# bayesml/BayesML

Measured on AMD Instinct MI355X. Metric: GMM-VB E+M samples/sec at K=64,D=128,N=1e7; 1/2/4/8-GPU scaling, higher is better.
Workload: dtype f64; 1 GPU; GMM-VB K=64 D=128 N=10000000 rows/GPU x 1 GPU, x stored f32, one VB iteration per step (c3 of BASELINE.json configs); classes=64, degree=128, rows_per_gpu=10000000, rows_total=10000000, x_storage=f32, parallelism=rows1, row_tiles=1

## Files before the change

### bayesml_amd/csrc/capi.hip

```cpp
#include "capi_internal.h"

namespace {
thread_local std::string g_err;
}

namespace gmmvb {
int fail(int code, const char* what, hipError_t e) {
    g_err = what;
    if (e != hipSuccess) {
        g_err += ": ";
        g_err += hipGetErrorString(e);
    }
    return code;
}
}

namespace {
KernelSizes kernel_sizes(int K, int D) {
    KernelSizes ks;
    ks.max_tiles = kMaxTiles;
    ks.t1_splits = GMMVB_T1_SPLITS;
    ks.sel_rows = kSelRows;
    ks.lse_rows = kLseRows;
    ks.scan_parts = kScanParts;
    ks.rec_slots = kRecSlots;
    ks.generic_rows = generic_rows(D);
    if (D > 32 * kMaxTiles) return ks;
    const int T = feature_tiles(D, kMaxTiles);
    ks.mstep_components_per_wg = mstep_components_per_wg(T, false);
    ks.slab_len = slab_len(T);
    ks.estep_image_doubles = estep_image_doubles(T);
    ks.estep_tri_image_doubles = estep_tri_image_doubles();
    ks.estep_bound_blocks = estep_bound_blocks(T);
    ks.estep_i8_image_bytes = estep_i8_image_bytes(D, 0);
    ks.estep_i8_bound_image_bytes = estep_i8_image_bytes(D, 1);
    ks.estep_i8_digit_row_bytes = estep_i8_digit_row_bytes(D);
    ks.proj_image_len = proj_image_len(K, D);
    ks.proj_const_len = proj_const_len(K);
    return ks;
}

struct Slots {
    void** at[kBufCount];
#define GMMVB_X(name) (void**)&ws->name,
    explicit Slots(gmmvb_workspace* ws) : at{GMMVB_WORKSPACE_BUFFERS(GMMVB_X)} {}
#undef GMMVB_X
};

struct HipAllocator {
    hipError_t err = hipSuccess;
    void* get(int64_t bytes, bool pinned) {
        void* p = nullptr;
        err = pinned ? hipHostMalloc(&p, (size_t)bytes, hipHostMallocDefault) : hipMalloc(&p, (size_t)bytes);
        return err == hipSuccess ? p : nullptr;
    }
    bool zero(void* p, int64_t bytes, bool pinned) {
        if (pinned) std::memset(p, 0, (size_t)bytes);
        else err = hipMemset(p, 0, (size_t)bytes);
        return err == hipSuccess;
    }
    void release(void* p, bool pinned) { (void)(pinned ? hipHostFree(p) : hipFree(p)); }
};

hipError_t init_workspace(gmmvb_workspace* ws) {
    hipError_t e = hipEventCreateWithFlags(&ws->ctr_ev, hipEventDisableTiming);
    if (ws->generic) {
        const int lds = (int)((size_t)ws->D * generic_rows(ws->D) * sizeof(double));
        if (e == hipSuccess) e = hipFuncSetAttribute((const void*)estep_generic_kernel<float>, hipFuncAttributeMaxDynamicSharedMemorySize, lds);
        if (e == hipSuccess) e = hipFuncSetAttribute((const void*)estep_generic_kernel<double>, hipFuncAttributeMaxDynamicSharedMemorySize, lds);
        return e;
    }
    ws->pt.init(ws->T, estep_bound_blocks(ws->T) ? (ws->D + 31) / 32 : 0);
    for (int i = 0; i < 6 && e == hipSuccess && ws->prune != 0; ++i) e = hipEventCreate(&ws->cal_ev[i]);
    return e;
}
}

extern "C" {

int gmmvb_abi_version(void) { return GMMVB_ABI_VERSION; }
const char* gmmvb_last_error(void) { return g_err.c_str(); }

int64_t gmmvb_stats_len(int K, int D) {
    if (K < 1 || D < 1) return -1;
    return (int64_t)K * (2 + (int64_t)D + (int64_t)D * D);
}

static int create_workspace(int K, int D, int x_dtype, int64_t max_rows, gmmvb_workspace* first, gmmvb_workspace** out) {
    if (!out) return fail(GMMVB_EINVAL, "out is null");
    *out = nullptr;
    if (K < 1 || D < 1 || max_rows < 1) return fail(GMMVB_EINVAL, "K, D and max_rows must be positive");
    if (x_dtype != GMMVB_F32 && x_dtype != GMMVB_F64) return fail(GMMVB_EINVAL, "x_dtype must be GMMVB_F32 or GMMVB_F64");
    int dev = 0;
    hipError_t e = hipGetDevice(&dev);
    if (e != hipSuccess) return fail(GMMVB_EHIP, "hipGetDevice", e);
    hipDeviceProp_t prop;
    e = hipGetDeviceProperties(&prop, dev);
    if (e != hipSuccess) return fail(GMMVB_EHIP, "hipGetDeviceProperties", e);

    gmmvb_workspace* ws = new (std::nothrow) gmmvb_workspace();
    gmmvb_scratch* group = first ? first->scratch : new (std::nothrow) gmmvb_scratch();
    if (!ws || !group) {
        delete ws;
        if (!first) delete group;
        return fail(GMMVB_ENOMEM, "host allocation failed");
    }
    ws->scratch = group;
    ++group->refs;
    const KernelSizes ks = kernel_sizes(K, D);
    const WorkspaceShape shape = make_shape(K, D, x_dtype, max_rows, prop.multiProcessorCount > 0 ? prop.multiProcessorCount : 256,
                                            WorkspaceOptions::read(std::getenv), ks);
    static_cast<WorkspaceShape&>(*ws) = shape;
    if (!first) group->npad = shape.npad;
    ws->buffers = buffer_plan(shape, ks, group->npad);
    HipAllocator hip;
    if (const BufferSpec* failed = allocate_all(ws->buffers, Slots(ws).at, group, hip, &ws->bytes)) {
        gmmvb_workspace_destroy(ws);
        return fail(failed->code, failed->what, hip.err);
    }
    e = init_workspace(ws);
    if (e != hipSuccess) {
        gmmvb_workspace_destroy(ws);
        return fail(GMMVB_EHIP, "workspace initialisation", e);
    }
    *out = ws;
    return GMMVB_OK;
}

int gmmvb_workspace_create(int K, int D, int x_dtype, int64_t max_rows, gmmvb_workspace** out) {
    return create_workspace(K, D, x_dtype, max_rows, nullptr, out);
}

int gmmvb_workspace_create_tile(gmmvb_workspace* first, int64_t max_rows, gmmvb_workspace** out) {
    if (!out) return fail(GMMVB_EINVAL, "out is null");
    *out = nullptr;
    if (!first || !first->scratch) return fail(GMMVB_EINVAL, "null argument");
    if (first->generic || first->hmm != nullptr)
        return fail(GMMVB_EUNSUPPORTED, "tile groups: mixture workspaces with c_degree <= 256 only (the HMM's time axis does not tile)");
    if (max_rows < 1 || max_rows > first->max_rows)
        return fail(GMMVB_EINVAL, "a further tile must not be larger than the group's first workspace");
    return create_workspace(first->K, first->D, first->x_dtype, max_rows, first, out);
}

int gmmvb_workspace_destroy(gmmvb_workspace* ws) {
    if (!ws) return GMMVB_OK;
    gmmvb_scratch* group = ws->scratch;
    if (group && group->owner == ws) group->owner = nullptr;
    HipAllocator hip;
    if (free_all(ws->buffers, Slots(ws).at, group, hip)) delete group;
    if (ws->pol_host) (void)hipHostFree(ws->pol_host);
    auto drop = [](hipEvent_t e) {
        if (e) (void)hipEventDestroy(e);
    };
    drop(ws->pol_ev);
    drop(ws->ctr_ev);
    for (hipEvent_t e : ws->ev) drop(e);
    for (hipEvent_t e : ws->span_ev) drop(e);
    for (hipEvent_t e : ws->cal_ev) drop(e);
    if (ws->hmm) hmm_state_destroy(ws->hmm);
    delete ws;
    return GMMVB_OK;
}

int64_t gmmvb_workspace_bytes(const gmmvb_workspace* ws) { return ws ? ws->bytes : -1; }

const char* gmmvb_last_launch_info(const gmmvb_workspace* ws) { return ws ? ws->info : ""; }

int gmmvb_pass_counts(const gmmvb_workspace* ws, int64_t* out ) {
    if (!ws || !out) return fail(GMMVB_EINVAL, "null argument");
    for (int i = 0; i < 8; ++i) out[i] = ws->passes[i];
    return GMMVB_OK;
}

int gmmvb_profile_enable(gmmvb_workspace* ws, int on) {
    if (!ws) return fail(GMMVB_EINVAL, "null argument");
    if (on && !ws->ev[0]) {
        for (auto& e : ws->ev) {
            hipError_t rc = hipEventCreate(&e);
            if (rc != hipSuccess) return fail(GMMVB_EHIP, "hipEventCreate", rc);
        }
        for (auto& e : ws->span_ev) {
            hipError_t rc = hipEventCreate(&e);
            if (rc != hipSuccess) return fail(GMMVB_EHIP, "hipEventCreate", rc);
        }
    }
    ws->prof = on != 0;
    ws->prof_light = on == 2;
    ws->span_open = false;
    ws->ev_e = ws->ev_m = false;
    ws->n_spans = 0;
    return GMMVB_OK;
}

const char* gmmvb_profile_span_name(int slot) { return (slot >= 0 && slot < kSpanSlots) ? kSpanNames[slot] : ""; }

int gmmvb_profile_spans(gmmvb_workspace* ws, float* ms , int* launches ) {
    if (!ws || !ms || !launches) return fail(GMMVB_EINVAL, "null argument");
    for (int i = 0; i < kSpanSlots; ++i) {
        ms[i] = 0.0f;
        launches[i] = 0;
    }
    for (int i = 0; i < ws->n_spans; ++i) {
        float t = 0.0f;
        hipError_t rc = hipEventSynchronize(ws->span_ev[2 * i + 1]);
        if (rc == hipSuccess) rc = hipEventElapsedTime(&t, ws->span_ev[2 * i], ws->span_ev[2 * i + 1]);
        if (rc != hipSuccess) return fail(GMMVB_EHIP, "event timing (span)", rc);
        ms[ws->span_slot[i]] += t;
        ++launches[ws->span_slot[i]];
    }
    return GMMVB_OK;
}

int gmmvb_profile_last_ms(gmmvb_workspace* ws, float* estep_ms, float* mstep_ms) {
    if (!ws || !estep_ms || !mstep_ms) return fail(GMMVB_EINVAL, "null argument");
    *estep_ms = *mstep_ms = -1.0f;
    if (ws->ev_e) {
        hipError_t rc = hipEventSynchronize(ws->ev[1]);
        if (rc == hipSuccess) rc = hipEventElapsedTime(estep_ms, ws->ev[0], ws->ev[1]);
        if (rc != hipSuccess) return fail(GMMVB_EHIP, "event timing (estep)", rc);
    }
    if (ws->ev_m) {
        hipError_t rc = hipEventSynchronize(ws->ev[3]);
        if (rc == hipSuccess) rc = hipEventElapsedTime(mstep_ms, ws->ev[2], ws->ev[3]);
        if (rc != hipSuccess) return fail(GMMVB_EHIP, "event timing (mstep)", rc);
    }
    return GMMVB_OK;
}

int gmmvb_set_pivot(gmmvb_workspace* ws, const double* pivot_dev, void* stream) {
    if (!ws || !pivot_dev) return fail(GMMVB_EINVAL, "null argument");
    hipError_t e = hipMemcpyAsync(ws->pivot, pivot_dev, (size_t)ws->D * sizeof(double), hipMemcpyDeviceToDevice,
                                  (hipStream_t)stream);
    if (e != hipSuccess) return fail(GMMVB_EHIP, "hipMemcpyAsync(pivot)", e);
    ws->xc_src = nullptr;
    ws->xq_src = nullptr;
    ++ws->pivot_gen;
    if (ws->lock_live) {
        ws->lock_live = false;
        ws->lock_reset = true;
    }
    return GMMVB_OK;
}

int gmmvb_wants_drift(const gmmvb_workspace* ws, int64_t n_rows) {
    if (!ws || ws->prune == 0 || ws->estep_variant != kEstepLds8 || ws->hmm != nullptr || !ws->rec_k) return 0;
    if (ws->opt_carry_off) return 0;
    if (ws->sharded) n_rows = ws->shard_rows / ws->shard_ranks;
    return (ws->prune == 2 || n_rows * (int64_t)ws->K >= (int64_t(1) << 23)) ? 1 : 0;
}

namespace {
__global__ void set_drift_kernel(const double* __restrict__ gamma, const double* __restrict__ delta, const double* __restrict__ big_gamma,
                                 const double* __restrict__ cvec, int K, double* __restrict__ drift) {
    const int k = blockIdx.x * blockDim.x + threadIdx.x;
    if (k >= K) return;
    drift[k] = gamma[k];
    drift[K + k] = delta[k];
    drift[2 * K + k] = cvec[k];
    drift[3 * K + k] = big_gamma[k];
}
}

int gmmvb_set_drift(gmmvb_workspace* ws, const double* gamma_dev, const double* delta_dev, const double* big_gamma_dev,
                    double typical_gamma, void* stream) {
    if (!ws || !gamma_dev || !delta_dev || !big_gamma_dev) return fail(GMMVB_EINVAL, "null argument");
    ws->typical_gamma = typical_gamma;
    hipStream_t st = (hipStream_t)stream;
    hipLaunchKernelGGL(set_drift_kernel, dim3((unsigned)((ws->K + 255) / 256)), dim3(256), 0, st, gamma_dev, delta_dev, big_gamma_dev,
                       ws->cvec, ws->K, ws->drift);
    const hipError_t e = hipGetLastError();
    if (e != hipSuccess) return fail(GMMVB_EHIP, "set_drift_kernel", e);
    ws->have_drift = ws->have_params && ws->params_used;
    return GMMVB_OK;
}

int gmmvb_debug_record(gmmvb_workspace* ws, int64_t row, double* out ) {
    if (!ws || !out || !ws->rec_k || row < 0 || row >= ws->npad) return fail(GMMVB_EINVAL, "bad argument");
    hipError_t e = hipDeviceSynchronize();
    auto get = [&e](void* dst, const void* src, size_t n) {
        if (e == hipSuccess) e = hipMemcpy(dst, src, n, hipMemcpyDeviceToHost);
    };
    for (int j = 0; j < kRecSlots; ++j) {
        unsigned short k = 0;
        float d = 0.0f;
        get(&k, ws->rec_k + (int64_t)j * ws->npad + row, sizeof(k));
        get(&d, ws->rec_d + (int64_t)j * ws->npad + row, sizeof(d));
        out[j] = k == kRecEmpty ? -1.0 : (double)k;
        out[8 + j] = d;
    }
    float B = 0.0f;
    unsigned char ex = 0, sel = 0, fl = 0;
    int kh = 0;
    get(&B, ws->rec_B + row, sizeof(B));
    get(&ex, ws->rec_exact + row, 1);
    get(&sel, ws->rec_sel + row, 1);
    get(&fl, ws->rec_flags + row, 1);
    get(&kh, ws->khat + row, sizeof(kh));
    get(out + 21, ws->lse + row, sizeof(double));
    out[16] = B;
    out[17] = ex;
    out[18] = sel;
    out[19] = fl;
    out[20] = kh;
    for (int w = 0; w < 4; ++w) {
        unsigned long long m = 0;
        if (w < (ws->K + 63) / 64) get(&m, ws->masks + (int64_t)w * ws->npad + row, sizeof(m));
        out[22 + w] = (double)m;
    }
    if (e != hipSuccess) return fail(GMMVB_EHIP, "reading a record back", e);
    return GMMVB_OK;
}

int64_t gmmvb_regroup_count(const gmmvb_workspace* ws) { return ws ? ws->sorts : -1; }

namespace {
__global__ void debug_all_rows_kernel(int* __restrict__ list, int* __restrict__ counts, int K, int k, int64_t n_rows) {
    const int64_t i = (int64_t)blockIdx.x * blockDim.x + threadIdx.x;
    if (i < n_rows) list[i] = (int)i;
    if (i < K) counts[i] = (int)(i == k ? n_rows : 0);
}
}

int gmmvb_debug_proof(gmmvb_workspace* ws, int k, int64_t n_rows, float* ub_dev, double* lb_dev, void* stream) {
    if (!ws || !ub_dev || !lb_dev || k < 0 || k >= ws->K) return fail(GMMVB_EINVAL, "bad argument");
    if (!ws->xq || !ws->img_i8b || ws->xq_src == nullptr || ws->xq_rows != n_rows || ws->xq_gen != ws->img_gen || !ws->have_params)
        return fail(GMMVB_ESTATE, "no digit planes for these rows: gmmvb_set_pivot, gmmvb_prepare_rows, gmmvb_set_params first");
    claim_scratch(ws);
    hipStream_t st = (hipStream_t)stream;
    ws->tmeta_valid = false;
    const unsigned grid = (unsigned)((std::max<int64_t>(n_rows, ws->K) + 255) / 256);
    hipLaunchKernelGGL(debug_all_rows_kernel, dim3(grid), dim3(256), 0, st, ws->lists + (int64_t)k * ws->npad, ws->counts, ws->K, k,
                       n_rows);
    hipLaunchKernelGGL(gather_plan_kernel, dim3(1), dim3(64), 0, st, ws->counts, ws->K, estep_i8_pairs_per_chunk(), ws->plan);
    hipError_t e = launch_estep_i8_proof(ws->D, ws->num_cu, st, ws->xq, ws->xqe, ws->img_i8b, ws->cvec, ws->K, ws->lists, ws->npad,
                                         ws->counts, ws->plan, ws->ub32, ws->lnrho, ws->npad);
    if (e == hipSuccess) e = hipMemcpyAsync(ub_dev, ws->ub32 + (int64_t)k * ws->npad, (size_t)n_rows * sizeof(float),
                                            hipMemcpyDeviceToDevice, st);
    if (e == hipSuccess) e = hipMemcpyAsync(lb_dev, ws->lnrho + (int64_t)k * ws->npad, (size_t)n_rows * sizeof(double),
                                            hipMemcpyDeviceToDevice, st);
    if (e != hipSuccess) return fail(GMMVB_EHIP, "proof kernel (diagnostic)", e);
    ws->e_state = 0;
    ws->lost_estep = false;
    ws->bounds_rows = 0;
    ws->rec_valid = ws->dense_valid = ws->rec_live = false;
    ws->active_lists = ws->blk_fresh = false;
    ws->lag.valid = false;
    if (ws->lock_live) {
        ws->lock_live = false;
        ws->lock_reset = true;
    }
    return GMMVB_OK;
}

int gmmvb_forget(gmmvb_workspace* ws) {
    if (!ws) return fail(GMMVB_EINVAL, "null argument");
    ws->forget = true;
    ws->have_drift = false;
    if (ws->lock_live) {
        ws->lock_live = false;
        ws->lock_reset = true;
    }
    return GMMVB_OK;
}

int gmmvb_set_params(gmmvb_workspace* ws, const double* c_dev, const double* m_dev, const double* u_dev,
                     void* stream) {
    if (!ws || !c_dev || !m_dev || !u_dev) return fail(GMMVB_EINVAL, "null argument");
    hipStream_t st = (hipStream_t)stream;
    hipError_t e = hipSuccess;
    if (ws->generic) {
        e = hipMemcpyAsync(ws->cvec, c_dev, (size_t)ws->K * sizeof(double), hipMemcpyDeviceToDevice, st);
        if (e != hipSuccess) return fail(GMMVB_EHIP, "hipMemcpyAsync(c)", e);
        e = hipMemcpyAsync(ws->gen_m, m_dev, (size_t)ws->K * ws->D * sizeof(double), hipMemcpyDeviceToDevice, st);
        if (e == hipSuccess)
            e = hipMemcpyAsync(ws->gen_u, u_dev, (size_t)ws->K * ws->D * ws->D * sizeof(double), hipMemcpyDeviceToDevice, st);
        if (e != hipSuccess) return fail(GMMVB_EHIP, "hipMemcpyAsync(m, u)", e);
        ws->have_params = true;
        ws->params_used = false;
        return GMMVB_OK;
    }
    if (ws->wide) {
        if (ws->pivot_i8) return fail(GMMVB_EUNSUPPORTED, "gmmvb_set_params: int8 images past D = 128");
        hipLaunchKernelGGL(pack_params_kernel, dim3(ws->K), dim3(256), 0, st, u_dev, m_dev, ws->K, ws->D, ws->T, ws->img_len, ws->img,
                           c_dev, ws->cvec, nullptr, nullptr);
        e = hipGetLastError();
        if (e != hipSuccess) return fail(GMMVB_EHIP, "pack_params_kernel", e);
    } else {
        e = launch_pack_images(u_dev, m_dev, c_dev, ws->pivot, ws->K, ws->D, ws->T, ws->img_len, ws->img, ws->cvec, ws->pivot_i8,
                               ws->pivot_i8 ? ws->img_i8 : nullptr, ws->pivot_i8 ? ws->img_i8b : nullptr, st);
        if (e != hipSuccess) return fail(GMMVB_EHIP, "pack_images_kernel", e);
        if (ws->pivot_i8) ws->img_gen = ws->pivot_gen;
    }
    if (ws->tri) {
        e = launch_pack_tri16(u_dev, m_dev, ws->K, ws->D, ws->tri, st);
        if (e != hipSuccess) return fail(GMMVB_EHIP, "pack_tri16_kernel", e);
    }
    ws->proj_table = false;
    if (ws->gimg && ws->opt_project != 0 && ws->sorted && ws->tile_ref_valid && ws->have_drift && ws->xq_gen == ws->pivot_gen &&
        !ws->opt_carry_off) {
        e = launch_proj_table(u_dev, m_dev, c_dev, ws->pivot, ws->K, ws->D, ws->gimg, ws->gconst, st);
        if (e != hipSuccess) return fail(GMMVB_EHIP, "proj_table_kernel", e);
        ws->proj_table = true;
    }
    ws->have_params = true;
    ws->params_used = false;
    return GMMVB_OK;
}

int fetch_counters(gmmvb_workspace* ws) {
    if (ws->ctr_pending) {
        hipError_t e = hipEventSynchronize(ws->ctr_ev);
        if (e != hipSuccess) return fail(GMMVB_EHIP, "waiting for the E-step counters", e);
        ws->lag.act = ws->ctr_host[0];
        if (ws->pend_mode == 0) {
            ws->lag.eval = (double)ws->pend_rows * ws->K;
            ws->lag.over = 0.0;
            ws->lag.settled = 0.0;
            ws->lag.listed = ws->lag.accum = ws->lag.act;
            ws->lag.exits = 0.0;
            ws->lag.cols = -1.0;
            ws->lag.left = -1.0;
            ws->lag.proof = 0.0;
            ws->lag.moved = 0.0;
        } else {
            ws->lag.proof = ws->ctr_host[7];
            ws->lag.exits = (ws->exit_host && ws->gather_exit) ? (double)ws->exit_host[0] : 0.0;
            ws->lag.cols = (ws->exit_host && ws->pend_lazy) ? (double)ws->exit_host[1] : -1.0;
            ws->lag.left = (ws->exit_host && ws->pend_proj) ? (double)ws->exit_host[2] : -1.0;
            ws->lag.settled = ws->ctr_host[4];
            ws->lag.listed = ws->ctr_host[5];
            ws->lag.accum = ws->ctr_host[6];
            ws->lag.eval = ws->ctr_host[1] + ((ws->pend_mode == 1 || ws->pend_mode == 3) ? ws->pend_round0 : 0.0);
            ws->lag.over = ws->ctr_host[2];
            ws->lag.moved = ws->ctr_host[3];
            if (!ws->sharded && ws->sorted && !ws->pend_first_sorted) ws->moved_since_sort += ws->lag.moved;
        }
        ws->lag.rows = (double)ws->pend_rows;
        ws->lag.mode = ws->pend_mode;
        ws->lag.valid = true;
        ws->ctr_pending = false;
    }
    return GMMVB_OK;
}

void poll_counters(gmmvb_workspace* ws) {
    if (ws->ctr_pending && hipEventQuery(ws->ctr_ev) == hipSuccess) (void)fetch_counters(ws);
}

namespace {
__global__ void policy_export_kernel(const double* __restrict__ ctr, const unsigned long long* __restrict__ exits, int mode,
                                     double rows, int K, double round0, int counted, int use_exits, double* __restrict__ out) {
    if (threadIdx.x != 0 || blockIdx.x != 0) return;
    const bool dense = mode == 0;
    const double act = counted ? ctr[0] : 0.0;
    out[0] = act;
    out[1] = dense ? rows * K : ctr[1] + ((mode == 1 || mode == 3) ? round0 : 0.0);
    out[2] = dense ? 0.0 : ctr[2];
    out[3] = dense ? 0.0 : ctr[3];
    out[4] = dense ? 0.0 : ctr[4];
    out[5] = dense ? act : ctr[5];
    out[6] = dense ? act : ctr[6];
    out[7] = dense ? 0.0 : ctr[7];
    out[8] = (dense || !use_exits || !exits) ? 0.0 : (double)*exits;
    out[9] = rows;
    out[10] = 1.0;
    out[11] = counted ? 1.0 : 0.0;
    out[12] = (double)mode;
    for (int i = 13; i < GMMVB_POLICY_LEN; ++i) out[i] = 0.0;
}
}

int gmmvb_set_shard(gmmvb_workspace* ws, int64_t global_rows, int n_ranks) {
    if (!ws || global_rows < 1 || n_ranks < 1) return fail(GMMVB_EINVAL, "bad argument");
    ws->sharded = n_ranks > 1;
    ws->shard_rows = global_rows;
    ws->shard_ranks = n_ranks;
    ws->pol.valid = false;
    if (ws->sharded && !ws->pol_host) {
        hipError_t e = hipHostMalloc((void**)&ws->pol_host, GMMVB_POLICY_LEN * sizeof(double), hipHostMallocDefault);
        if (e == hipSuccess) e = hipEventCreateWithFlags(&ws->pol_ev, hipEventDisableTiming);
        if (e != hipSuccess) return fail(GMMVB_EHIP, "policy buffers", e);
    }
    return GMMVB_OK;
}

int gmmvb_policy_export(gmmvb_workspace* ws, double* out_dev, void* stream) {
    if (!ws || !out_dev) return fail(GMMVB_EINVAL, "null argument");
    if (ws->e_state != 1) return fail(GMMVB_ESTATE, "no E-step output in the workspace");
    hipLaunchKernelGGL(policy_export_kernel, dim3(1), dim3(64), 0, (hipStream_t)stream, ws->ctr, ws->exit_ctr, ws->prev_pass,
                       (double)ws->e_rows, ws->K, ws->pend_round0, ws->exp_counted ? 1 : 0, ws->gather_exit ? 1 : 0, out_dev);
    hipError_t e = hipGetLastError();
    if (e != hipSuccess) return fail(GMMVB_EHIP, "policy export", e);
    return GMMVB_OK;
}

int gmmvb_policy_import(gmmvb_workspace* ws, const double* in_dev, void* stream) {
    if (!ws || !in_dev) return fail(GMMVB_EINVAL, "null argument");
    if (!ws->sharded) return GMMVB_OK;
    hipStream_t st = (hipStream_t)stream;
    hipError_t e = hipMemcpyAsync(ws->pol_host, in_dev, GMMVB_POLICY_LEN * sizeof(double), hipMemcpyDeviceToHost, st);
    if (e == hipSuccess) e = hipEventRecord(ws->pol_ev, st);
    if (e != hipSuccess) return fail(GMMVB_EHIP, "policy import", e);
    ws->pol_pending = true;
    ws->pol_mode = ws->prev_pass;
    ws->pol_first_sorted = ws->pend_first_sorted;
    return GMMVB_OK;
}

int take_policy(gmmvb_workspace* ws) {
    if (!ws->pol_pending) return GMMVB_OK;
    hipError_t e = hipEventSynchronize(ws->pol_ev);
    if (e != hipSuccess) return fail(GMMVB_EHIP, "waiting for the imported counters", e);
    const double* h = ws->pol_host;
    gmmvb_pass_counters& p = ws->pol;
    p.act = h[0];
    p.eval = h[1];
    p.over = h[2];
    p.moved = h[3];
    p.settled = h[4];
    p.listed = h[5];
    p.accum = h[6];
    p.proof = h[7];
    p.exits = h[8];
    p.rows = h[9];
    p.ranks = h[10];
    p.mode = h[10] >= 1.0 ? (int)(h[12] / h[10] + 0.5) : ws->pol_mode;
    p.valid = h[10] >= 1.0 && h[11] == h[10];
    if (p.valid && ws->sorted && !ws->pol_first_sorted) ws->moved_since_sort += p.moved;
    ws->pol_pending = false;
    return GMMVB_OK;
}

int gmmvb_last_sparsity(gmmvb_workspace* ws, void* stream, double* active_pairs, double* evaluated_pairs) {
    (void)stream;
    if (!ws || !active_pairs || !evaluated_pairs) return fail(GMMVB_EINVAL, "null argument");
    if (ws->e_state != 1 && !ws->lost_estep) return fail(GMMVB_ESTATE, "no E-step output in the workspace");
    int rc = fetch_counters(ws);
    if (rc) return rc;
    *evaluated_pairs = ws->lag.mode == 0 ? (double)ws->e_rows * ws->K : ws->lag.eval;
    *active_pairs = (ws->sparse && ws->act_rows == ws->e_rows) ? ws->lag.act : -1.0;
    return GMMVB_OK;
}

int gmmvb_last_work(gmmvb_workspace* ws, double* out) {
    if (!ws || !out) return fail(GMMVB_EINVAL, "null argument");
    if (ws->e_state != 1 && !ws->lost_estep) return fail(GMMVB_ESTATE, "no E-step output in the workspace");
    int rc = fetch_counters(ws);
    if (rc) return rc;
    const bool counted = ws->sparse && ws->act_rows == ws->e_rows;
    out[0] = counted ? ws->lag.act : -1.0;
    out[1] = ws->lag.mode == 0 ? (double)ws->e_rows * ws->K : ws->lag.eval;
    out[2] = counted ? ws->lag.accum : -1.0;
    out[3] = ws->lag.mode == 0 ? 0.0 : ws->lag.settled;
    out[4] = ws->lag.mode == 0 ? 0.0 : ws->lag.exits;
    out[5] = ws->lag.mode == 0 ? 0.0 : ws->lag.proof;
    out[6] = ws->lag.mode == 3 ? ws->lag.cols : -1.0;
    out[7] = ws->lag.mode == 3 ? ws->lag.left : -1.0;
    return GMMVB_OK;
}

int gmmvb_policy_calibrate(gmmvb_workspace* ws, int on) {
    if (!ws) return fail(GMMVB_EINVAL, "null argument");
    ws->opt_calibrate = on != 0;
    if (!on) {
        ws->pt.init(ws->T, estep_bound_blocks(ws->T) ? (ws->D + 31) / 32 : 0);
        for (double& p : ws->cal_pairs) p = 0.0;
    }
    return GMMVB_OK;
}

int gmmvb_policy_table(gmmvb_workspace* ws, double* out ) {
    if (!ws || !out) return fail(GMMVB_EINVAL, "null argument");
    cal_poll(ws);
    const gmmvb::PolicyTable& t = ws->pt;
    const double v[GMMVB_POLICY_TABLE_LEN] = {t.dense_e_ns, t.dense_m_ns, t.bound_ns, t.exact_ns, t.proof_ns, t.list_m_ns,
                                              t.lit_dense_e, t.lit_dense_m, t.lit_bound, t.prune_below(), t.dense_again_above(),
                                              t.list_m_below(), (double)(t.measured & 7), (double)((t.measured >> 3) & 7),
                                              ws->opt_calibrate ? 1.0 : 0.0, 0.0};
    for (int i = 0; i < GMMVB_POLICY_TABLE_LEN; ++i) out[i] = v[i];
    return GMMVB_OK;
}

int check_x(const gmmvb_workspace* ws, const void* x_dev, int64_t ldx, int64_t n_rows, bool* vec) {
    if (!ws || !x_dev) return fail(GMMVB_EINVAL, "null argument");
    if (n_rows < 1 || n_rows > ws->max_rows) return fail(GMMVB_EINVAL, "n_rows must be in [1, max_rows]");
    if (ldx < ws->D) return fail(GMMVB_EINVAL, "ldx must be >= D");
    const int64_t esz = ws->x_dtype == GMMVB_F64 ? 8 : 4;
    const int64_t valign = esz * (ws->T > 4 ? ws->T : 4);
    *vec = (ws->D % 16 == 0) && ((uintptr_t)x_dev % valign == 0) && ((ldx * esz) % valign == 0);
    return GMMVB_OK;
}

int gmmvb_prepare_rows(gmmvb_workspace* ws, const void* x_dev, int64_t ldx, int64_t n_rows, void* stream) {
    bool vec = false;
    int rc = check_x(ws, x_dev, ldx, n_rows, &vec);
    if (rc) return rc;
    claim_scratch(ws);
    ws->bounds_rows = 0;
    if (ws->lock_live) {
        ws->lock_live = false;
        ws->lock_reset = true;
    }
    ws->sorted = false;
    ws->tile_ref_valid = false;
    ws->rec_valid = false;
    ws->dense_valid = false;
    ws->lag.valid = false;
    if (!ws->xc) return GMMVB_OK;
    const int Dp = 16 * ws->T;
    const int64_t pad_rows = round_up(n_rows, 64) + 64;
    const int64_t total = pad_rows * Dp;
    const unsigned grid = (unsigned)((total + 255) / 256);
    hipStream_t st = (hipStream_t)stream;
    if (ws->x_dtype == GMMVB_F64)
        hipLaunchKernelGGL(center_rows_kernel<double>, dim3(grid), dim3(256), 0, st, (const double*)x_dev, ldx, n_rows,
                           pad_rows, ws->D, Dp, ws->pivot, ws->xc);
    else
        hipLaunchKernelGGL(center_rows_kernel<float>, dim3(grid), dim3(256), 0, st, (const float*)x_dev, ldx, n_rows,
                           pad_rows, ws->D, Dp, ws->pivot, ws->xc);
    hipError_t e = hipGetLastError();
    if (e != hipSuccess) return fail(GMMVB_EHIP, "center_rows launch", e);
    ws->xc_src = x_dev;
    ws->xc_rows = n_rows;
    ws->xc_ldx = ldx;
    ws->xc_stale = false;
    if (ws->xq) {
        e = launch_x_digits(x_dev, ws->x_dtype == GMMVB_F64, ldx, n_rows, ws->D, ws->pivot, ws->xq, ws->xqe, st);
        if (e != hipSuccess) return fail(GMMVB_EHIP, "x_digits launch", e);
        ws->xq_src = x_dev;
        ws->xq_rows = n_rows;
        ws->xq_ldx = ldx;
        ws->xq_gen = ws->pivot_gen;
    }
    return GMMVB_OK;
}

hipError_t recenter_rows(gmmvb_workspace* ws, int64_t n_rows, hipStream_t st) {
    const int Dp = 16 * ws->T;
    const int64_t pad_rows = round_up(n_rows, 64) + 64;
    const unsigned cg = (unsigned)((pad_rows * Dp + 255) / 256);
    const void* src = ws->sorted ? ws->xp : ws->xc_src;
    const int64_t ld = ws->sorted ? (int64_t)ws->D : ws->xc_ldx;
    if (ws->x_dtype == GMMVB_F64)
        hipLaunchKernelGGL(center_rows_kernel<double>, dim3(cg), dim3(256), 0, st, (const double*)src, ld, n_rows,
                           pad_rows, ws->D, Dp, ws->pivot, ws->xc);
    else
        hipLaunchKernelGGL(center_rows_kernel<float>, dim3(cg), dim3(256), 0, st, (const float*)src, ld, n_rows,
                           pad_rows, ws->D, Dp, ws->pivot, ws->xc);
    ws->xc_stale = false;
    return hipGetLastError();
}


}
```

### bayesml_amd/csrc/capi_estep.hip

```cpp
#include "capi_internal.h"

namespace {

struct Pass {
    gmmvb_workspace* ws;
    const void* x_dev;
    int64_t ldx, n_rows;
    hipStream_t st;
    int is64;
    bool vec;
    int sel_grid;
    double pairs;
    EstepArgs a{};
    EstepI8Args a8{};
    RecArrays rec{};
    bool i8 = false;
    bool prunable = false;
    bool prev_lists = false, can_project = false, own_known = false, tmeta_was_valid = false;
    int mode = kPassDense;
    bool settle = false, proof_capable = false;
    double skip_margin = -1.0;
    bool counted = false, proof_ran = false, tmeta_kept = false, projected = false, filtered = false, emission_to_hmm = false,
         sorted_now = false;
    bool phase_closed = false;
    const char* name = "";
    int rpw = 0;
    int64_t grid = 0;

    PassFacts facts();
    int apply(const PassFacts& f, const PassPlan& plan);
    int run_generic();
    int run_dense();
    int run_bound();
    int run_sweep();
    int run_sweep_over_lists();
    int run_sweep_from_best();
    int sweep_bounds(bool proof, bool own_round);
    int run_candidates();
    int finish(const char* latch_what);
};

hipError_t regroup_rows(gmmvb_workspace* ws, const void* x_dev, int64_t ldx, int64_t n_rows, hipStream_t st, bool keep_state,
                        bool margin_ok) {
    const int sel_grid = (int)((n_rows + kSelRows - 1) / kSelRows);
    const unsigned cgrid = (unsigned)((n_rows + 255) / 256);
    const int* key = ws->khat;
    const int* perm_in = ws->sorted ? ws->perm : nullptr;
    const bool by_margin = ws->opt_regroup_margin && margin_ok && ws->K >= kMarginBuckets;
    if (by_margin) {
        int* bucket = ws->perm_tmp;
        hipLaunchKernelGGL(margin_bucket_kernel, dim3(cgrid), dim3(256), 0, st, ws->lnrho, ws->npad, n_rows, ws->lse, ws->khat,
                           keep_state ? ws->lock : nullptr, bucket);
        hipLaunchKernelGGL(select_mask_kernel<3>, dim3(sel_grid), dim3(kSelRows), 0, st, ws->lnrho, ws->npad, n_rows,
                           kMarginBuckets, bucket, ws->masks, ws->blk);
        scan_and_fill(ws, st, ws->masks, ws->blk, sel_grid, n_rows, kMarginBuckets);
        int* key1 = reinterpret_cast<int*>(ws->rec_d);
        hipLaunchKernelGGL(perm_compose_kernel, dim3(cgrid, kMarginBuckets), dim3(256), 0, st, ws->lists, ws->npad, ws->counts,
                           ws->khat, key1);
        hipLaunchKernelGGL(perm_compose_kernel, dim3(cgrid, kMarginBuckets), dim3(256), 0, st, ws->lists, ws->npad, ws->counts,
                           perm_in, ws->perm_tmp);
        key = key1;
        perm_in = ws->perm_tmp;
    }
    hipLaunchKernelGGL(select_mask_kernel<3>, dim3(sel_grid), dim3(kSelRows), 0, st, ws->lnrho, ws->npad, n_rows, ws->K,
                       const_cast<int*>(key), ws->masks, ws->blk);
    scan_and_fill(ws, st, ws->masks, ws->blk, sel_grid, n_rows, ws->K);
    ws->tile_ref_valid = false;
    if (ws->tile_ref) {
        if (launch_proj_tile_ref(ws->counts, ws->K, sel_grid, ws->tile_ref, st) == hipSuccess) ws->tile_ref_valid = true;
    }
    if (by_margin) {
        hipLaunchKernelGGL(perm_compose_kernel, dim3(cgrid, ws->K), dim3(256), 0, st, ws->lists, ws->npad, ws->counts, perm_in,
                           ws->khat);
        int* new_perm = ws->khat;
        ws->khat = ws->perm_tmp;
        ws->perm_tmp = ws->perm;
        ws->perm = new_perm;
    } else {
        hipLaunchKernelGGL(perm_compose_kernel, dim3(cgrid, ws->K), dim3(256), 0, st, ws->lists, ws->npad, ws->counts, perm_in,
                           ws->perm_tmp);
        std::swap(ws->perm, ws->perm_tmp);
    }
    if (keep_state) {
        hipLaunchKernelGGL(regroup_state_kernel, dim3((unsigned)((n_rows + 255) / 256)), dim3(256), 0, st, ws->perm,
                           ws->sorted ? ws->iperm : nullptr, n_rows, ws->lock, ws->lcomp, ws->dlock, ws->rec_sel, ws->rec_flags,
                           ws->rthr);
        std::swap(ws->lock, ws->rec_sel);
        std::swap(ws->lcomp, ws->rec_flags);
        std::swap(ws->dlock, ws->rthr);
    }
    hipLaunchKernelGGL(perm_invert_kernel, dim3((unsigned)((n_rows + 255) / 256)), dim3(256), 0, st, ws->perm, n_rows, ws->iperm);
    const int64_t total = n_rows * ws->D;
    const unsigned pg = (unsigned)((total + 255) / 256);
    const int64_t esz = ws->x_dtype == GMMVB_F64 ? 8 : 4;
    if ((ws->D * esz) % 16 == 0 && (ldx * esz) % 16 == 0 && (uintptr_t)x_dev % 16 == 0) {
        const int p16 = (int)(ws->D * esz / 16);
        hipLaunchKernelGGL(permute_rows16_kernel, dim3((unsigned)((n_rows * p16 + 255) / 256)), dim3(256), 0, st,
                           (const uint4*)x_dev, ldx * esz / 16, n_rows, p16, ws->perm, (uint4*)ws->xp);
    } else if (ws->x_dtype == GMMVB_F64)
        hipLaunchKernelGGL(permute_rows_kernel<double>, dim3(pg), dim3(256), 0, st, (const double*)x_dev, ldx, n_rows, ws->D,
                           ws->perm, (double*)ws->xp);
    else
        hipLaunchKernelGGL(permute_rows_kernel<float>, dim3(pg), dim3(256), 0, st, (const float*)x_dev, ldx, n_rows, ws->D,
                           ws->perm, (float*)ws->xp);
    ws->xc_stale = ws->xc != nullptr;
    if (ws->xq && ws->xq_src == x_dev) {
        hipError_t eq = launch_x_digits(ws->xp, ws->x_dtype == GMMVB_F64, ws->D, n_rows, ws->D, ws->pivot, ws->xq, ws->xqe, st);
        if (eq != hipSuccess) return eq;
        ws->xq_gen = ws->pivot_gen;
    }
    ws->sorted = true;
    ++ws->sorts;
    return hipGetLastError();
}

hipError_t launch_bound_pass(gmmvb_workspace* ws, const EstepI8Args& a8, int is64, bool vec, hipStream_t st,
                             const char** name, int* rpw_out, int64_t* grid_out) {
    const int rpw = estep_i8_rows_per_wg();
    int64_t grid = (a8.n_rows + rpw - 1) / rpw;
    if (grid > (1 << 20)) grid = 1 << 20;
    *rpw_out = rpw;
    *grid_out = grid;
    EstepI8Args ab = a8;
    ab.img = ws->img_i8b;
    ab.khat = ws->khat;
    ab.ub = ws->ub32;
    return launch_estep_i8_bound(is64, vec, ws->bound.tb, (int)grid, st, ab, name);
}

hipError_t lists_and_gather(gmmvb_workspace* ws, const EstepArgs& a, int is64, bool vec, int sel_grid, hipStream_t st,
                            const float* thr = nullptr, const double* block_total = nullptr ) {
    if (thr) {
        hipError_t em = hipMemsetAsync(ws->exit_ctr, 0, sizeof(unsigned long long), st);
        if (em != hipSuccess) return em;
    }
    span_begin(ws, kSpanSelect, st);
    scan_and_fill(ws, st, ws->masks, ws->blk, sel_grid, a.n_rows, ws->K, block_total);
    hipLaunchKernelGGL(gather_plan_kernel, dim3(1), dim3(64), 0, st, ws->counts, ws->K,
                       estep_gather_rows_per_wg(ws->T, is64), ws->plan);
    hipError_t e = hipGetLastError();
    span_end(ws, st);
    if (e != hipSuccess) return e;
    span_begin(ws, kSpanGather, st);
    e = launch_estep_gather_dev(ws->T, is64, vec, 2 * ws->num_cu, st, a, ws->lists, ws->npad, ws->counts, ws->plan, thr,
                                thr ? ws->exit_ctr : nullptr, 0.0f);
    span_end(ws, st);
    ++ws->passes[7];
    return e;
}

}

extern "C" {


bool cal_wanted(gmmvb_workspace* ws, int what, double pairs) {
    return ws->opt_calibrate && ws->cal_ev[0] != nullptr && !((ws->pt.measured >> what) & 1) && ws->cal_pairs[what] == 0.0 &&
           pairs >= (double)(int64_t(1) << 23) && ws->hmm == nullptr;
}
void cal_mark(gmmvb_workspace* ws, int what, double pairs, hipStream_t st) {
    note_hip(ws, hipEventRecord(ws->cal_ev[2 * what + 1], st));
    ws->cal_pairs[what] = pairs;
}
void cal_poll(gmmvb_workspace* ws) {
    for (int what = 0; what < 3; ++what) {
        if (ws->cal_pairs[what] <= 0.0 || hipEventQuery(ws->cal_ev[2 * what + 1]) != hipSuccess) continue;
        float ms = 0.0f;
        if (hipEventElapsedTime(&ms, ws->cal_ev[2 * what], ws->cal_ev[2 * what + 1]) == hipSuccess) {
            double ns = (double)ms * 1e6 / ws->cal_pairs[what];
            if (what == 2) ns += 0.010 * tri_pairs(ws->T) / 36.0;
            const bool took = ws->pt.take(what, ns);
            if (ws->opt_debug)
                std::fprintf(stderr, "[gmmvb] policy table: %s %.4f ns per pair %s (prune below %.3f, dense again above %.3f, list M below %.3f)\n",
                             what == 0 ? "dense E" : (what == 1 ? "dense M" : "bound pass"), ns, took ? "taken" : "out of range: literal kept",
                             ws->pt.prune_below(), ws->pt.dense_again_above(), ws->pt.list_m_below());
            if (!took) ws->pt.measured |= 8 << what;
            ws->cal_pairs[what] = (took || ++ws->cal_tries[what] >= 3) ? -1.0 : 0.0;
        } else {
            ws->cal_pairs[what] = -1.0;
        }
    }
}

}

namespace {

hipError_t proof_round(gmmvb_workspace* ws, hipStream_t st, const int* blk_base, int sel_grid, int64_t n_rows, float* ub) {
    if (ws->opt_proof_blocked && ws->slabs &&
        estep_i8_proof_work_bytes(ws->K, n_rows) <= ws->scratch->bytes[kBuf_slabs])
        return launch_estep_i8_proof_blocked(ws->D, ws->num_cu, st, ws->xq, ws->xqe, ws->img_i8b, ws->cvec, ws->K, ws->lists,
                                             ws->npad, ws->counts, blk_base, sel_grid, ws->slabs, ub, ws->lnrho, ws->npad);
    hipLaunchKernelGGL(gather_plan_kernel, dim3(1), dim3(64), 0, st, ws->counts, ws->K, estep_i8_pairs_per_chunk(), ws->plan);
    return launch_estep_i8_proof(ws->D, ws->num_cu, st, ws->xq, ws->xqe, ws->img_i8b, ws->cvec, ws->K, ws->lists, ws->npad,
                                 ws->counts, ws->plan, ub, ws->lnrho, ws->npad);
}

int Pass::run_generic() {
    const int R = generic_rows(ws->D);
    const dim3 g((unsigned)((n_rows + R - 1) / R), (unsigned)ws->K);
    const size_t lds = (size_t)ws->D * R * sizeof(double);
    span_begin(ws, kSpanEstepMain, st);
    if (is64)
        hipLaunchKernelGGL(estep_generic_kernel<double>, g, dim3(64), lds, st, (const double*)x_dev, ldx, n_rows, ws->D,
                           ws->gen_u, ws->gen_m, ws->cvec, R, ws->lnrho, ws->npad);
    else
        hipLaunchKernelGGL(estep_generic_kernel<float>, g, dim3(64), lds, st, (const float*)x_dev, ldx, n_rows, ws->D,
                           ws->gen_u, ws->gen_m, ws->cvec, R, ws->lnrho, ws->npad);
    span_end(ws, st);
    if (phase_events(ws)) {
        note_hip(ws, hipEventRecord(ws->ev[1], st));
        ws->ev_e = true;
    }
    phase_closed = true;
    span_begin(ws, kSpanLse, st);
    hipLaunchKernelGGL(row_lse_kernel, dim3((unsigned)((n_rows + kLseRows - 1) / kLseRows)), dim3(256), 0, st, ws->lnrho,
                       ws->npad, n_rows, ws->K, ws->lse, nullptr, nullptr, 1);
    span_end(ws, st);
    hipError_t eg = hipGetLastError();
    if (eg != hipSuccess) return fail(GMMVB_EHIP, "estep_generic launch", eg);
    ++ws->passes[0];
    ws->rec_live = ws->rec_valid = false;
    ws->evaluated = pairs;
    std::snprintf(ws->info, sizeof(ws->info), "estep_generic_f64<D=%d> grid=%ux%ux64 rows/workgroup=%d", ws->D, g.x, g.y, R);
    name = nullptr;
    return GMMVB_OK;
}

int Pass::run_dense() {
    const bool valu16 = ws->estep_variant == kEstepValu16 && ws->tri != nullptr;
    emission_to_hmm = ws->T == 1 && !ws->wide && !i8 && !ws->sorted && hmm_fused_emission(ws->hmm);
    rpw = ws->wide ? estep_rows_rows_per_wg()
                     : (i8 ? estep_i8_rows_per_wg() : (valu16 ? estep_rows16_rows_per_wg() : estep_rows_per_wg(ws->estep_variant, ws->T, is64)));
    grid = (n_rows + rpw - 1) / rpw;
    if (grid > (1 << 20)) grid = 1 << 20;
    span_begin(ws, kSpanEstepMain, st);
    const bool cal_e = !ws->wide && !i8 && !emission_to_hmm && !valu16 && cal_wanted(ws, 0, pairs);
    if (cal_e) note_hip(ws, hipEventRecord(ws->cal_ev[0], st));
    hipError_t e = ws->wide ? launch_estep_rows(ws->T, is64, (int)grid, st, a, &name)
                            : (i8 ? launch_estep_i8(is64, vec, (int)grid, st, a8, &name)
                                  : (emission_to_hmm ? hmm_launch_emission16(ws->hmm, is64, vec, st, a, &name)
                                     : (valu16 ? launch_estep_rows16(is64, vec, (int)grid, st, a, ws->tri, &name)
                                            : launch_estep(ws->estep_variant, ws->T, is64, vec, (int)grid, st, a, &name))));
    if (cal_e) cal_mark(ws, 0, pairs, st);
    span_end(ws, st);
    if (e != hipSuccess) return fail(GMMVB_EHIP, "estep launch", e);
    ++ws->passes[0];
    const int lse_blocks = (int)((n_rows + kLseRows - 1) / kLseRows);
    const bool count_pairs = ws->sparse && ws->masks && ws->hmm == nullptr && n_rows * (int64_t)ws->K >= (int64_t(1) << 18);
    span_begin(ws, kSpanLse, st);
    if (count_pairs) {
        const int stride = lse_blocks >= 64 ? 16 : 1;
        const int sampled = (lse_blocks + stride - 1) / stride;
        hipLaunchKernelGGL(row_lse_kernel, dim3((unsigned)sampled), dim3(256), 0, st, ws->lnrho, ws->npad, n_rows, ws->K,
                           ws->lse, ws->dpart, nullptr, stride);
        hipLaunchKernelGGL(thr_kernel, dim3((unsigned)ws->K), dim3(256), 0, st, ws->dpart, nullptr, sampled, ws->K, ws->thr,
                           ws->ctr);
        hipLaunchKernelGGL(lse_mask_kernel, dim3((unsigned)sel_grid), dim3(kSelRows), 0, st, ws->lnrho, ws->npad, n_rows,
                           ws->K, ws->thr, ws->lse, ws->masks, ws->blk, ws->apart, ws->khat);
        hipLaunchKernelGGL(sum_parts_kernel, dim3(1), dim3(1024), 0, st, ws->apart, nullptr, nullptr, nullptr, nullptr, nullptr,
                           nullptr, nullptr, sel_grid, ws->ctr);
        if (prunable)
            hipLaunchKernelGGL(rec_build_kernel<false>, dim3((unsigned)((n_rows + 255) / 256)), dim3(256), 0, st, ws->lnrho,
                               ws->npad, n_rows, ws->K, ws->cvec, nullptr, rec, ws->ub32);
        e = hipGetLastError();
        if (e != hipSuccess) return fail(GMMVB_EHIP, "row_lse / lse_mask launch", e);
        counted = true;
        ws->rec_valid = prunable;
    } else if (ws->hmm != nullptr) {
        ws->lse_stale = true;
        ws->rec_valid = false;
    } else {
        hipLaunchKernelGGL(row_lse_kernel, dim3((unsigned)lse_blocks), dim3(256), 0, st, ws->lnrho, ws->npad, n_rows, ws->K,
                           ws->lse, nullptr, nullptr, 1);
        e = hipGetLastError();
        if (e != hipSuccess) return fail(GMMVB_EHIP, "row_lse launch", e);
        ws->rec_valid = false;
    }
    span_end(ws, st);
    ws->rec_live = false;
    ws->evaluated = pairs;
    return GMMVB_OK;
}

int Pass::run_bound() {
    span_begin(ws, kSpanEstepMain, st);
    const bool cal_b = ws->bound.tb == (ws->D + 31) / 32 && cal_wanted(ws, 2, pairs);
    if (cal_b) note_hip(ws, hipEventRecord(ws->cal_ev[4], st));
    hipError_t e = launch_bound_pass(ws, a8, is64, vec, st, &name, &rpw, &grid);
    if (cal_b) cal_mark(ws, 2, pairs, st);
    span_end(ws, st);
    if (e != hipSuccess) return fail(GMMVB_EHIP, "estep_bound launch", e);
    ++ws->passes[1];
    span_begin(ws, kSpanSelect, st);
    hipLaunchKernelGGL(select_mask_kernel<3>, dim3(sel_grid), dim3(kSelRows), 0, st, ws->lnrho, ws->npad, n_rows, ws->K, ws->khat,
                       ws->masks, ws->blk);
    span_end(ws, st);
    e = lists_and_gather(ws, a, is64, vec, sel_grid, st);
    if (e != hipSuccess) return fail(GMMVB_EHIP, "E-step best-component evaluation", e);
    span_begin(ws, kSpanSelect, st);
    hipLaunchKernelGGL(rec_build_kernel<true>, dim3((unsigned)((n_rows + 255) / 256)), dim3(256), 0, st, ws->lnrho, ws->npad,
                       n_rows, ws->K, ws->cvec, ws->khat, rec, ws->ub32);
    hipLaunchKernelGGL(rec_select_kernel, dim3(sel_grid), dim3(kSelRows), 0, st, rec, n_rows, ws->K, ws->cvec, ws->masks,
                       ws->npad, ws->blk, ws->epart, ws->opart, ws->rthr);
    if (proof_capable) {
        scan_and_fill(ws, st, ws->masks, ws->blk, sel_grid, n_rows, ws->K, ws->epart);
        span_end(ws, st);
        span_begin(ws, kSpanProof, st);
        e = proof_round(ws, st, ws->blk, sel_grid, n_rows, ws->ub32);
        span_end(ws, st);
        if (e != hipSuccess) return fail(GMMVB_EHIP, "proof round (bound pass)", e);
        span_begin(ws, kSpanSelect, st);
        hipLaunchKernelGGL(rec_prune_kernel, dim3(sel_grid), dim3(kSelRows), 0, st, rec, ws->masks, ws->npad, n_rows, ws->K,
                           ws->cvec, ws->ub32, ws->rthr, ws->blk, ws->epart, ws->ppart);
        proof_ran = true;
    }
    span_end(ws, st);
    return GMMVB_OK;
}

int Pass::sweep_bounds(bool proof, bool own_round) {
    unsigned char* lock = settle ? ws->lock : nullptr;
    unsigned long long* pmask = proof ? ws->rmask : nullptr;
    const int proof_all = ws->opt_proof_all ? 1 : 0, own_fresh = own_round ? 1 : 0;
    if (can_project && ws->opt_project == 2) {
        note_hip(ws, hipMemsetAsync(ws->exit_ctr + 2, 0, sizeof(unsigned long long), st));
        hipError_t e = launch_rec_project(sel_grid, st, project_args(ws, n_rows, lock, pmask, proof_all, own_fresh));
        if (e != hipSuccess) return fail(GMMVB_EHIP, "rec_project launch", e);
        name = "estep_sweep_projected";
        projected = true;
    } else if (ws->tmeta) {
        note_hip(ws, hipMemsetAsync(ws->exit_ctr + 1, 0, sizeof(unsigned long long), st));
        dispatch_mask_words(ws->K, [&](auto wc) {
            hipLaunchKernelGGL((rec_sweep_kernel<true, true, decltype(wc)::value>), dim3(sel_grid), dim3(kSelRows), 0, st, ws->ub32,
                               ws->lnrho, ws->npad, n_rows, ws->K, ws->drift, ws->cvec, ws->khat, rec, ws->masks, ws->blk,
                               ws->epart, ws->opart, lock, ws->dlock, ws->rthr, ws->lcomp, pmask, ws->rblk, proof_all, own_fresh,
                               ws->tmeta, tmeta_was_valid ? 0 : 1, ws->exit_ctr + 1, ws->ppart);
        });
        tmeta_kept = true;
    } else {
        hipLaunchKernelGGL(rec_sweep_kernel<true>, dim3(sel_grid), dim3(kSelRows), 0, st, ws->ub32, ws->lnrho, ws->npad, n_rows,
                           ws->K, ws->drift, ws->cvec, ws->khat, rec, ws->masks, ws->blk, ws->epart, ws->opart, lock, ws->dlock,
                           ws->rthr, ws->lcomp, pmask, ws->rblk, proof_all, own_fresh, nullptr, 0, nullptr, ws->ppart);
    }
    return GMMVB_OK;
}

int Pass::run_sweep_over_lists() {
    span_begin(ws, kSpanSelect, st);
    if (!ws->active_lists)
        scan_and_fill(ws, st, ws->masks, ws->blk, sel_grid, n_rows, ws->K, ws->prev_pass != 0 ? ws->gpart : nullptr);
    hipLaunchKernelGGL(gather_plan_kernel, dim3(1), dim3(64), 0, st, ws->counts, ws->K, estep_gather_rows_per_wg(ws->T, is64),
                       ws->plan);
    span_end(ws, st);
    span_begin(ws, kSpanGather, st);
    hipError_t e = launch_estep_gather_dev(ws->T, is64, vec, 2 * ws->num_cu, st, a, ws->lists, ws->npad, ws->counts, ws->plan);
    span_end(ws, st);
    ++ws->passes[7];
    if (e != hipSuccess) return fail(GMMVB_EHIP, "E-step active-pair evaluation", e);
    const bool proof = proof_capable && (ws->skip_used || ws->opt_proof_all);
    const bool own_round = proof && ws->skip_used && !(ws->typical_gamma >= ws->pt.own_round_below);
    if (own_round) {
        span_begin(ws, kSpanSelect, st);
        hipLaunchKernelGGL(settled_mask_kernel, dim3(sel_grid), dim3(kSelRows), 0, st, ws->lock, ws->masks, ws->lcomp, ws->npad,
                           n_rows, ws->K, ws->rmask, ws->rblk, ws->drift, ws->spart);
        scan_and_fill(ws, st, ws->rmask, ws->rblk, sel_grid, n_rows, ws->K, ws->spart);
        span_end(ws, st);
        span_begin(ws, kSpanProof, st);
        e = proof_round(ws, st, ws->rblk, sel_grid, n_rows, nullptr);
        span_end(ws, st);
        if (e != hipSuccess) return fail(GMMVB_EHIP, "proof round (settled rows' own pairs)", e);
    }
    span_begin(ws, kSpanSelect, st);
    int rc = sweep_bounds(proof, own_round);
    if (rc) return rc;
    if (proof && can_project && !projected) {
        note_hip(ws, hipMemsetAsync(ws->exit_ctr + 2, 0, sizeof(unsigned long long), st));
        e = launch_proj_filter(sel_grid, st, project_args(ws, n_rows, ws->lock, ws->rmask, 0, 0));
        if (e != hipSuccess) return fail(GMMVB_EHIP, "proj_filter launch", e);
        filtered = true;
    }
    if (proof) {
        scan_and_fill(ws, st, ws->rmask, ws->rblk, sel_grid, n_rows, ws->K, projected ? nullptr : ws->ppart);
        span_end(ws, st);
        span_begin(ws, kSpanProof, st);
        e = proof_round(ws, st, ws->rblk, sel_grid, n_rows, ws->ub32);
        span_end(ws, st);
        if (e != hipSuccess) return fail(GMMVB_EHIP, "proof round", e);
        span_begin(ws, kSpanSelect, st);
        hipLaunchKernelGGL(rec_proof_decide_kernel, dim3(sel_grid), dim3(kSelRows), 0, st, rec, ws->rmask, ws->masks, ws->npad,
                           n_rows, ws->K, ws->cvec, ws->ub32, ws->lnrho, ws->lcomp, ws->dlock, ws->rthr, ws->blk, ws->epart,
                           ws->ppart, own_round ? ws->spart : nullptr);
        proof_ran = true;
    }
    span_end(ws, st);
    return GMMVB_OK;
}

int Pass::run_sweep_from_best() {
    span_begin(ws, kSpanSelect, st);
    hipLaunchKernelGGL(select_mask_kernel<3>, dim3(sel_grid), dim3(kSelRows), 0, st, ws->lnrho, ws->npad, n_rows, ws->K, ws->khat,
                       ws->masks, ws->blk);
    span_end(ws, st);
    hipError_t e = lists_and_gather(ws, a, is64, vec, sel_grid, st);
    if (e != hipSuccess) return fail(GMMVB_EHIP, "E-step best-component evaluation", e);
    span_begin(ws, kSpanSelect, st);
    hipLaunchKernelGGL(rec_sweep_kernel<false>, dim3(sel_grid), dim3(kSelRows), 0, st, ws->ub32, ws->lnrho, ws->npad, n_rows, ws->K,
                       ws->drift, ws->cvec, ws->khat, rec, ws->masks, ws->blk, ws->epart, ws->opart,
                       settle ? ws->lock : nullptr, ws->dlock, ws->rthr, ws->lcomp, nullptr, nullptr, 0, 0, nullptr, 0);
    span_end(ws, st);
    return GMMVB_OK;
}

int Pass::run_sweep() {
    rpw = kSelRows;
    grid = sel_grid;
    name = "estep_sweep_bounds";
    ++ws->passes[4];
    ++ws->sweeps;
    const int rc = prev_lists ? run_sweep_over_lists() : run_sweep_from_best();
    if (rc) return rc;
    ws->sweep_prev = prev_lists;
    return GMMVB_OK;
}

int Pass::run_candidates() {
    hipError_t e = lists_and_gather(ws, a, is64, vec, sel_grid, st, ws->gather_exit ? ws->rthr : nullptr, ws->epart);
    if (e != hipSuccess) return fail(GMMVB_EHIP, "E-step candidate evaluation", e);
    span_begin(ws, kSpanLse, st);
    hipLaunchKernelGGL(rec_finish_kernel, dim3(sel_grid), dim3(kSelRows), 0, st, rec, ws->lnrho, ws->npad, n_rows, ws->K,
                       ws->cvec, ws->lse, ws->khat, ws->masks, ws->blk, ws->apart, ws->mpart, ws->ub32,
                       settle ? ws->lock : nullptr, ws->dlock, skip_margin, settle ? ws->dmask : nullptr,
                       settle ? ws->dblk : nullptr, ws->mmask, ws->mblk, ws->spart, ws->gpart, ws->qpart, ws->rthr, ws->lcomp);
    if (!proof_ran) note_hip(ws, hipMemsetAsync(ws->ctr + 7, 0, sizeof(double), st));
    hipLaunchKernelGGL(sum_parts_kernel, dim3(proof_ran ? 8 : 7), dim3(1024), 0, st, ws->apart, ws->epart, ws->opart, ws->mpart,
                       ws->spart, ws->gpart, ws->qpart, ws->ppart, sel_grid, ws->ctr);
    e = hipGetLastError();
    span_end(ws, st);
    if (e != hipSuccess) return fail(GMMVB_EHIP, "rec_finish launch", e);
    counted = true;
    ws->rec_valid = true;
    ws->rec_live = true;
    ws->evaluated = -1.0;
    if (settle) {
        ws->lock_live = true;
        ws->delta_pending = true;
    }
    return GMMVB_OK;
}

int Pass::finish(const char* latch_what) {
    ws->tmeta_valid = tmeta_kept;
    ws->pend_lazy = tmeta_kept;
    ws->pend_proj = projected || filtered;
    if (!phase_closed && phase_events(ws)) {
        note_hip(ws, hipEventRecord(ws->ev[1], st));
        ws->ev_e = true;
    }
    if (counted) {
        hipError_t e = hipMemcpyAsync(ws->ctr_host, ws->ctr, 8 * sizeof(double), hipMemcpyDeviceToHost, st);
        if (e == hipSuccess && ws->exit_ctr && mode != kPassDense)
            e = hipMemcpyAsync(ws->exit_host, ws->exit_ctr, 3 * sizeof(unsigned long long), hipMemcpyDeviceToHost, st);
        if (e == hipSuccess) e = hipEventRecord(ws->ctr_ev, st);
        if (e != hipSuccess) return fail(GMMVB_EHIP, "E-step counters", e);
        ws->ctr_pending = true;
        ws->pend_mode = mode;
        ws->pend_rows = n_rows;
        ws->pend_first_sorted = sorted_now;
        ws->pend_round0 = (mode == kPassSweep && ws->sweep_prev && own_known) ? ws->lag.listed : (double)n_rows;
        ws->act_rows = n_rows;
    } else {
        ws->ctr_pending = false;
        ws->lag.valid = false;
        ws->act_rows = 0;
    }
    ws->exp_counted = counted;
    ws->pol.valid = false;
    ws->act_host = -1.0;
    ws->active_lists = false;
    ws->mlists_done = ws->mlists_lost = false;
    if (skip_margin >= 0.0) ws->skip_used = true;
    ws->blk_fresh = counted;
    ws->e_state = emission_to_hmm ? 4 : 1;
    ws->hmm_no_lnrho = emission_to_hmm;
    ws->lost_estep = false;
    ws->e_rows = n_rows;
    ws->params_used = true;
    ws->have_drift = false;
    ws->bounds_rows = n_rows;
    ws->bounds_x = x_dev;
    ws->bounds_ldx = ldx;
    ws->prev_pass = mode;
    ws->dense_valid = !projected;
    if (mode == kPassDense || mode == kPassBound) ws->sweeps = 0;
    if (name)
        std::snprintf(ws->info, sizeof(ws->info), "%s grid=%lldx%d rows/workgroup=%d", name, (long long)grid,
                      (i8 || mode != kPassDense) ? 512 : estep_threads(ws->estep_variant), rpw);
    return take_hip(ws, latch_what);
}

PassFacts Pass::facts() {
    PassFacts f;
    f.L = ws->sharded ? ws->pol : ws->lag;
    f.prune = ws->prune;
    f.xc_of_x = xc_is_of(ws, x_dev, ldx, n_rows);
    f.has_xc = ws->xc != nullptr;
    f.can_prune = ws->prune != 0 && ws->estep_variant == kEstepLds8 && ws->hmm == nullptr && ws->rec_k != nullptr && f.has_xc &&
                  f.xc_of_x;
    const int64_t size_rows = ws->sharded ? ws->shard_rows / ws->shard_ranks : n_rows;
    f.big = ws->prune == 2 || size_rows * (int64_t)ws->K >= (int64_t(1) << 23);
    f.same_rows = ws->bounds_rows == n_rows && ws->bounds_x == x_dev && ws->bounds_ldx == ldx;
    f.known = f.L.valid && (ws->sharded || (f.L.rows == (double)n_rows && !ws->ctr_pending));
    own_known = ws->lag.valid && ws->lag.rows == (double)n_rows && !ws->ctr_pending;
    f.after_estep = ws->e_state == 1 || ws->lost_estep;
    f.prev_lists = (ws->active_lists || ws->blk_fresh) && f.after_estep && ws->act_rows == n_rows && f.same_rows;
    f.xq_of_x = xq_is_of(ws, x_dev, ldx, n_rows);
    f.can_project = ws->proj_table && ws->gimg != nullptr && ws->sorted && ws->tile_ref_valid && f.prev_lists && f.xq_of_x &&
                    ws->xq_gen == ws->pivot_gen && ws->lock != nullptr;
    f.forget = ws->forget;
    f.have_drift = ws->have_drift;
    f.opt_carry_off = ws->opt_carry_off;
    f.dense_valid = ws->dense_valid;
    f.opt_project = ws->opt_project;
    f.typical_gamma = ws->typical_gamma;
    f.bound_fail_act = ws->bound_fail_act;
    f.bound_tb = ws->bound.tb;
    f.T = ws->T, f.K = ws->K, f.D = ws->D;
    f.n_rows = n_rows;
    f.sort_rows = ws->sort_rows, f.has_xp = ws->xp != nullptr, f.sorted = ws->sorted;
    f.sorts = ws->sorts;
    f.moved_since_sort = ws->moved_since_sort;
    f.hmm = ws->hmm != nullptr;
    f.has_lock = ws->lock != nullptr, f.lock_reset = ws->lock_reset, f.lock_live = ws->lock_live;
    f.delta_pending = ws->delta_pending, f.cache_on = ws->cache_on, f.sparse = ws->sparse, f.has_masks = ws->masks != nullptr;
    f.opt_proof = ws->opt_proof, f.has_bound_images = ws->img_i8b != nullptr, f.xq_current = ws->xq_gen == ws->img_gen;
    f.settle_margin = ws->settle_margin;
    prunable = f.can_prune && f.big;
    prev_lists = f.prev_lists;
    can_project = f.can_project;
    return f;
}

int Pass::apply(const PassFacts& f, const PassPlan& plan) {
    if (plan.spare_set) ws->spare_last = plan.spare_last;
    if (plan.fell_back) ++ws->passes[3];
    ws->bound_fail_act = plan.bound_fail_act;
    ws->forget = false;
    if (ws->lock) {
        if (plan.reset_cache) {
            hipError_t e = hipMemsetAsync(ws->lock, 0, (size_t)ws->npad, st);
            if (e == hipSuccess) e = hipMemsetAsync(ws->cache, 0, (size_t)gmmvb_stats_len(ws->K, ws->D) * sizeof(double), st);
            if (e != hipSuccess) return fail(GMMVB_EHIP, "resetting the cache of single-component rows", e);
            ws->lock_live = false;
            ws->skip_used = false;
        }
        ws->lock_reset = false;
        ws->delta_pending = false;
    }
    ws->settled_fresh = false;
    mode = plan.mode;
    settle = plan.settle;
    proof_capable = plan.proof_capable;
    skip_margin = plan.skip_margin;
    if (ws->opt_debug) {
        const gmmvb_pass_counters& L = f.L;
        const double rows_l = f.rows_l();
        std::fprintf(stderr, "[gmmvb] estep: mode=%d known=%d lag(mode=%d act=%.3g eval=%.3g over=%.3g settled=%.3g listed=%.3g) gamma=%.3f rec_valid=%d drift=%d settle=%d\n",
                     plan.mode, (int)f.known, L.mode, L.act / rows_l, L.eval / rows_l, L.over / rows_l, L.settled / rows_l,
                     L.listed / rows_l, ws->typical_gamma, (int)ws->rec_valid, (int)ws->have_drift, (int)plan.settle);
    }
    const bool wants_drift = gmmvb_wants_drift(ws, n_rows) != 0;
    ws->bound.choose(plan.mode, ws->img_i8b != nullptr, f.L, f.known, wants_drift && ws->have_drift, wants_drift, ws->pt, ws->T,
                     ws->D, ws->K);
    return GMMVB_OK;
}

}

extern "C" {

int gmmvb_estep(gmmvb_workspace* ws, const void* x_dev, int64_t ldx, int64_t n_rows, void* stream) {
    bool vec = false;
    int rc = check_x(ws, x_dev, ldx, n_rows, &vec);
    if (rc) return rc;
    if (!ws->have_params) return fail(GMMVB_ESTATE, "gmmvb_set_params has not been called");
    claim_scratch(ws);
    hipStream_t st = (hipStream_t)stream;
    Pass p{ws, x_dev, ldx, n_rows, st, ws->x_dtype == GMMVB_F64, vec, (int)((n_rows + kSelRows - 1) / kSelRows),
           (double)n_rows * ws->K};
    if (ws->generic) {
        if (phase_events(ws)) note_hip(ws, hipEventRecord(ws->ev[0], st));
        ws->n_spans = 0;
        rc = p.run_generic();
        return rc ? rc : p.finish("event record inside the E-step");
    }
    p.i8 = ws->estep_variant == kEstepI8;
    p.a = EstepArgs{x_dev, ldx, n_rows, ws->D, ws->img, ws->cvec, ws->K, ws->lnrho, ws->npad};
    p.a8 = EstepI8Args{x_dev, ldx, n_rows, ws->D, ws->img_i8, ws->pivot_i8, ws->cvec, ws->K, ws->lnrho, ws->npad};
    if (ws->sorted && ws->xc_src != x_dev) ws->sorted = false;

    if (ws->sharded) {
        rc = take_policy(ws);
        if (rc) return rc;
    }
    poll_counters(ws);
    cal_poll(ws);
    const PassFacts facts = p.facts();
    const PassPlan plan = choose_pass(ws->pt, facts);
    rc = p.apply(facts, plan);
    if (rc) return rc;

    if (phase_events(ws)) note_hip(ws, hipEventRecord(ws->ev[0], st));
    ws->n_spans = 0;
    if (plan.regroup) {
        span_begin(ws, kSpanSelect, st);
        hipError_t e = regroup_rows(ws, x_dev, ldx, n_rows, st, ws->lock_live, ws->e_state == 1 && !ws->lse_stale);
        span_end(ws, st);
        if (e != hipSuccess) return fail(GMMVB_EHIP, "regrouping the rows", e);
        ws->moved_since_sort = 0.0;
        p.sorted_now = true;
    }
    if (ws->sorted) {
        p.a.x = p.a8.x = ws->xp;
        p.a.ldx = p.a8.ldx = ws->D;
        p.vec = ws->D % 16 == 0;
    }
    p.rec = RecArrays{ws->rec_k, ws->rec_d, ws->rec_B, ws->rec_exact, ws->rec_sel, ws->rec_flags, ws->npad};
    ws->lse_stale = false;
    p.tmeta_was_valid = ws->tmeta_valid;
    ws->tmeta_valid = false;
    if (p.mode == kPassDense) {
        rc = p.run_dense();
    } else {
        rc = p.mode == kPassBound ? p.run_bound() : p.run_sweep();
        if (rc == GMMVB_OK) rc = p.run_candidates();
    }
    return rc ? rc : p.finish("event record / counter reset inside the E-step");
}

}
```

### bayesml_amd/csrc/capi_internal.h

```cpp
#pragma once
#include "workspace.h"

#include <cstdio>
#include <algorithm>
#include <cstdlib>
#include <cstring>
#include <new>
#include <string>
#include <type_traits>

#include "aux_kernels.h"
#include "generic.h"
#include "launch.h"
#include "records.h"

using namespace gmmvb;

#ifndef GMMVB_T1_SPLITS
#define GMMVB_T1_SPLITS 24
#endif

template <int W = 1, typename F>
static inline void dispatch_mask_words(int K, F&& f) {
    if constexpr (W < 4) {
        if ((K + 63) / 64 == W) return f(std::integral_constant<int, W>{});
        return dispatch_mask_words<W + 1>(K, f);
    } else {
        return f(std::integral_constant<int, 4>{});
    }
}

extern "C" {

enum { kSpanEstepMain = 0, kSpanSelect = 1, kSpanGather = 2, kSpanLse = 3, kSpanLists = 4, kSpanMstepMain = 5,
       kSpanReduce = 6, kSpanProof = 7, kSpanSlots = 8 };
static const char* const kSpanNames[kSpanSlots] = {"estep_main", "estep_select", "estep_gather", "estep_lse_mask",
                                                   "mstep_lists", "mstep_main", "mstep_reduce", "estep_proof"};
static inline void note_hip(gmmvb_workspace* ws, hipError_t e) {
    if (e != hipSuccess && ws->hip_err == hipSuccess) ws->hip_err = e;
}
static inline int take_hip(gmmvb_workspace* ws, const char* what) {
    if (ws->hip_err == hipSuccess) return GMMVB_OK;
    const hipError_t e = ws->hip_err;
    ws->hip_err = hipSuccess;
    return fail(GMMVB_EHIP, what, e);
}
static inline bool span_kept(const gmmvb_workspace* ws, int slot) {
    return !ws->prof_light || slot == kSpanEstepMain || slot == kSpanGather || slot == kSpanMstepMain;
}
static inline void span_begin(gmmvb_workspace* ws, int slot, hipStream_t st) {
    ws->span_open = false;
    if (!ws->prof || ws->n_spans >= gmmvb_workspace::kMaxSpans || !span_kept(ws, slot)) return;
    ws->span_slot[ws->n_spans] = slot;
    ws->span_open = true;
    note_hip(ws, hipEventRecord(ws->span_ev[2 * ws->n_spans], st));
}
static inline void span_end(gmmvb_workspace* ws, hipStream_t st) {
    if (!ws->span_open) return;
    ws->span_open = false;
    note_hip(ws, hipEventRecord(ws->span_ev[2 * ws->n_spans + 1], st));
    ++ws->n_spans;
}
static inline bool phase_events(const gmmvb_workspace* ws) { return ws->prof && !ws->prof_light; }

static inline bool xc_is_of(const gmmvb_workspace* ws, const void* x_dev, int64_t ldx, int64_t n_rows) {
    return ws->xc_src == x_dev && ws->xc_rows == n_rows && ws->xc_ldx == ldx;
}
static inline bool xq_is_of(const gmmvb_workspace* ws, const void* x_dev, int64_t ldx, int64_t n_rows) {
    return ws->xq != nullptr && ws->xq_src == x_dev && ws->xq_rows == n_rows && ws->xq_ldx == ldx;
}
static inline void scan_and_fill(gmmvb_workspace* ws, hipStream_t st, const unsigned long long* masks, int* blk, int nblk,
                                 int64_t n_rows, int K, const double* block_total = nullptr, unsigned char* lock = nullptr,
                                 const unsigned char* lcomp = nullptr) {
    launch_scan_counts(st, blk, nblk, K, ws->counts, ws->scan_parts);
    hipLaunchKernelGGL(fill_lists_kernel, dim3(nblk), dim3(kSelRows), 0, st, masks, ws->npad, n_rows, K, blk, ws->lists, ws->npad,
                       lock, lcomp, block_total);
}
static inline ProjectArgs project_args(const gmmvb_workspace* ws, int64_t n_rows, unsigned char* lock, unsigned long long* pmask,
                                       int proof_all, int own_fresh) {
    return ProjectArgs{ws->xq, ws->xqe, ws->gimg, ws->gconst, ws->tile_ref, ws->lnrho, ws->npad, n_rows, ws->K, ws->D, ws->drift,
                       ws->cvec, ws->rec_k, ws->rec_d, ws->rec_B, ws->rec_exact, ws->rec_sel, ws->rec_flags, ws->masks, ws->blk,
                       ws->epart, ws->opart, lock, ws->dlock, ws->rthr, ws->lcomp, pmask, ws->rblk, proof_all, own_fresh,
                       ws->exit_ctr + 2};
}

static inline void yield_scratch(gmmvb_workspace* w) {
    w->lost_estep = w->e_state == 1;
    w->e_state = 0;
    w->active_lists = false;
    if (w->mlists_done) w->mlists_lost = true;
    w->mlists_done = false;
    w->rec_live = false;
    w->settled_fresh = false;
    if (w->xc_src) w->xc_stale = true;
}
static inline void claim_scratch(gmmvb_workspace* ws) {
    gmmvb_scratch* s = ws->scratch;
    if (!s || s->owner == ws) return;
    if (s->owner) yield_scratch(s->owner);
    s->owner = ws;
}
int fetch_counters(gmmvb_workspace* ws);
void poll_counters(gmmvb_workspace* ws);
int take_policy(gmmvb_workspace* ws);
int check_x(const gmmvb_workspace* ws, const void* x_dev, int64_t ldx, int64_t n_rows, bool* vec);
hipError_t recenter_rows(gmmvb_workspace* ws, int64_t n_rows, hipStream_t st);
bool cal_wanted(gmmvb_workspace* ws, int what, double pairs);
void cal_mark(gmmvb_workspace* ws, int what, double pairs, hipStream_t st);
void cal_poll(gmmvb_workspace* ws);

}
```

### bayesml_amd/csrc/capi_mstep.hip

```cpp
#include "capi_internal.h"

extern "C" {

int gmmvb_load_responsibilities(gmmvb_workspace* ws, const double* r_dev, int64_t n_rows, void* stream) {
    if (!ws || !r_dev) return fail(GMMVB_EINVAL, "null argument");
    if (n_rows < 1 || n_rows > ws->max_rows) return fail(GMMVB_EINVAL, "n_rows must be in [1, max_rows]");
    claim_scratch(ws);
    const int tb = 256;
    hipLaunchKernelGGL(load_r_kernel, dim3((unsigned)((n_rows + tb - 1) / tb)), dim3(tb), 0, (hipStream_t)stream,
                       r_dev, n_rows, ws->K, ws->lnrho, ws->npad, ws->lse, ws->sorted ? ws->iperm : nullptr);
    hipError_t e = hipGetLastError();
    if (e != hipSuccess) return fail(GMMVB_EHIP, "load_r launch", e);
    ws->e_state = 2;
    ws->lost_estep = false;
    ws->e_rows = n_rows;
    ws->n_spans = 0;
    ws->bounds_rows = 0;
    if (ws->lock_live) {
        ws->lock_live = false;
        ws->lock_reset = true;
    }

    ws->rec_valid = false;
    ws->dense_valid = false;
    ws->rec_live = false;
    ws->act_rows = 0;
    return GMMVB_OK;
}

int gmmvb_mstep(gmmvb_workspace* ws, const void* x_dev, int64_t ldx, int64_t n_rows, double* stats_dev,
                void* stream) {
    bool vec = false;
    int rc = check_x(ws, x_dev, ldx, n_rows, &vec);
    if (rc) return rc;
    if (!stats_dev) return fail(GMMVB_EINVAL, "stats_dev is null");
    if (ws->e_state == 0 || ws->e_state == 4 || ws->e_rows != n_rows)
        return fail(GMMVB_ESTATE, "no responsibilities for these rows: call gmmvb_estep or gmmvb_load_responsibilities first");
    hipStream_t st = (hipStream_t)stream;
    if (ws->lse_stale && ws->e_state == 1) {
        hipLaunchKernelGGL(row_lse_kernel, dim3((unsigned)((n_rows + kLseRows - 1) / kLseRows)), dim3(256), 0, st, ws->lnrho,
                           ws->npad, n_rows, ws->K, ws->lse, nullptr, nullptr, 1);
        ws->lse_stale = false;
    }
    if (ws->generic) {
        const int direct = ws->e_state == 2 ? 1 : (ws->e_state == 3 ? 2 : 0);
        if (ws->e_state == 3 && hmm_ensure_gamma_cm(ws->hmm, st) != hipSuccess) return fail(GMMVB_EHIP, "gamma transpose launch");
        const double* lr = ws->e_state == 3 ? hmm_gamma_cm(ws->hmm) : ws->lnrho;
        const double* aux = ws->e_state == 3 && !ws->hmm_skip_h ? ws->lnrho : nullptr;
        int S = ws->gen_S;
        const int64_t rps = round_up((n_rows + S - 1) / S, 64);
        S = (int)((n_rows + rps - 1) / rps);
        const int tiles = tri_pairs(ws->T);
        if (phase_events(ws)) note_hip(ws, hipEventRecord(ws->ev[2], st));
        span_begin(ws, kSpanMstepMain, st);
        if (ws->x_dtype == GMMVB_F64) {
            hipLaunchKernelGGL(mstep_generic_first_kernel<double>, dim3(ws->K, S), dim3(256), 0, st, (const double*)x_dev, ldx, n_rows,
                               ws->D, ws->pivot, lr, ws->lse, aux, ws->npad, ws->K, rps, direct, ws->gen_first);
            hipLaunchKernelGGL(mstep_generic_second_kernel<double>, dim3(tiles, ws->K, S), dim3(256), 0, st, (const double*)x_dev, ldx,
                               n_rows, ws->D, ws->pivot, lr, ws->lse, aux, ws->npad, ws->K, rps, direct, ws->T, ws->gen_second);
        } else {
            hipLaunchKernelGGL(mstep_generic_first_kernel<float>, dim3(ws->K, S), dim3(256), 0, st, (const float*)x_dev, ldx, n_rows,
                               ws->D, ws->pivot, lr, ws->lse, aux, ws->npad, ws->K, rps, direct, ws->gen_first);
            hipLaunchKernelGGL(mstep_generic_second_kernel<float>, dim3(tiles, ws->K, S), dim3(256), 0, st, (const float*)x_dev, ldx,
                               n_rows, ws->D, ws->pivot, lr, ws->lse, aux, ws->npad, ws->K, rps, direct, ws->T, ws->gen_second);
        }
        span_end(ws, st);
        if (phase_events(ws)) {
            note_hip(ws, hipEventRecord(ws->ev[3], st));
            ws->ev_m = true;
        }
        span_begin(ws, kSpanReduce, st);
        const int64_t elems = ws->D + 2 + (int64_t)tiles * 256;
        hipLaunchKernelGGL(reduce_generic_kernel, dim3((unsigned)((elems + 255) / 256), ws->K), dim3(256), 0, st, ws->gen_first,
                           ws->gen_second, S, ws->K, ws->D, ws->T, stats_dev);
        span_end(ws, st);
        hipError_t eg = hipGetLastError();
        if (eg != hipSuccess) return fail(GMMVB_EHIP, "mstep_generic launch", eg);
        ++ws->passes[5];
        const size_t used = std::strlen(ws->info);
        std::snprintf(ws->info + used, sizeof(ws->info) - used, " | mstep_generic_f64<D=%d> tiles=%d splits=%d", ws->D, tiles, S);
        return take_hip(ws, "event record inside the M-step");
    }
    int64_t S = ws->S_cap;
    const int64_t groups = (n_rows + 63) / 64;
    if (S > groups) S = groups;
    int64_t rows_per_split = round_up((n_rows + S - 1) / S, 64);
    if (ws->split_rows && rows_per_split > ws->split_rows) rows_per_split = ws->split_rows;
    S = (n_rows + rows_per_split - 1) / rows_per_split;
    bool pre = ws->xc && xc_is_of(ws, x_dev, ldx, n_rows);
    if (ws->wide && !pre && ws->xc) {
        rc = gmmvb_prepare_rows(ws, x_dev, ldx, n_rows, stream);
        if (rc) return rc;
        pre = true;
    }
    const int kpw = mstep_components_per_wg(ws->T, pre);
    const int KG = (ws->K + kpw - 1) / kpw;
    int64_t grid = 8 * ((S + 7) / 8) * KG;
    MstepArgs a{x_dev, ldx, n_rows, ws->D, ws->pivot, ws->lnrho, ws->lse, nullptr, ws->npad, ws->K, KG, (int)S,
                rows_per_split, ws->e_state == 2 ? 1 : 0, ws->slabs};
    const bool hmm_small = ws->e_state == 3 && ws->T == 1 && pre;
    if (ws->e_state == 3) {
        if (!hmm_small && hmm_ensure_gamma_cm(ws->hmm, st) != hipSuccess) return fail(GMMVB_EHIP, "gamma transpose launch");
        a.lnrho = hmm_gamma_cm(ws->hmm);
        a.aux = (ws->hmm_no_lnrho || ws->hmm_skip_h) ? nullptr : ws->lnrho;
        a.direct_r = 2;
    }
    if (pre) {
        a.x = ws->xc;
        a.ldx = 16 * ws->T;
        a.D = 16 * ws->T;
    } else if (ws->sorted) {
        return fail(GMMVB_ESTATE, "the workspace's rows are regrouped for another sample matrix: call gmmvb_prepare_rows first");
    }
    const char* name = "";
    hipError_t e;
    bool sparse = ws->sparse && ws->masks && pre && ws->e_state == 1 && ws->act_rows == n_rows;
    if (sparse) {
        const double pairs = (double)n_rows * ws->K;
        if (ws->rec_live) {
        } else {
            rc = fetch_counters(ws);
            if (rc) return rc;
            sparse = ws->lag.valid && ws->lag.act <= ws->pt.list_m_below() * pairs;
        }
    }
    if (sparse && ws->K > 256) sparse = false;
    if (ws->rec_live && ws->e_state == 1 && !sparse)
        return fail(GMMVB_ESTATE, "a pruned E-step needs the list M-step over the matrix of the E-step (gmmvb_prepare_rows)");
    if (ws->lock_live && !sparse)
        return fail(GMMVB_ESTATE, "settled rows need the list M-step over the matrix of the E-step (gmmvb_prepare_rows)");
    if (sparse) {
        const int nblk = (int)((n_rows + kSelRows - 1) / kSelRows);
        if (phase_events(ws)) note_hip(ws, hipEventRecord(ws->ev[2], st));
        const int cap_chunks0 = (int)std::min<int64_t>((int64_t)ws->S_cap * ws->K, 1 << 30);
#ifndef GMMVB_MLIST_RMIN
#define GMMVB_MLIST_RMIN 1024
#endif
        const int r_min0 = GMMVB_MLIST_RMIN;
        MstepListArgs la0{ws->xc, ws->lnrho, ws->lse, ws->lists, ws->npad, ws->counts, ws->plan_m, cap_chunks0, r_min0,
                          ws->npad, ws->K, ws->slabs};
        static const bool list_xc = dev_env("GMMVB_MLIST_XC") && dev_env("GMMVB_MLIST_XC")[0] == '1';
        if (!list_xc && ws->x_dtype == GMMVB_F32 && ws->D == 16 * ws->T && (ws->T == 2 || ws->T == 4 || ws->T == 8)) {
            if (ws->sorted) {
                la0.x32 = (const float*)ws->xp;
                la0.ldx = ws->D;
            } else if (vec) {
                la0.x32 = (const float*)x_dev;
                la0.ldx = ldx;
            }
            la0.n_rows = n_rows;
            la0.D = ws->D;
            la0.pivot = ws->pivot;
        }
        if (!la0.x32 && ws->xc_stale) {
            e = recenter_rows(ws, n_rows, st);
            if (e != hipSuccess) return fail(GMMVB_EHIP, "center_rows launch", e);
        }
        int64_t lgrid = (cap_chunks0 + kpw - 1) / kpw;
        {
            const int64_t most = (n_rows * (int64_t)ws->K + r_min0 - 1) / r_min0 + ws->K;
            if ((most + kpw - 1) / kpw < lgrid) lgrid = (most + kpw - 1) / kpw;
        }
        const int elems0 = tri_pairs(ws->T) * 256 + 16 * ws->T + 2;
        if (ws->lock_live && ws->delta_pending) {
            span_begin(ws, kSpanLists, st);
            scan_and_fill(ws, st, ws->dmask, ws->dblk, nblk, n_rows, ws->K, ws->e_state == 1 ? ws->qpart : nullptr, ws->lock,
                          ws->lcomp);
            span_end(ws, st);
            MstepListArgs ld = la0;
            ld.direct_r = 3;
            int64_t dgrid = ((n_rows + r_min0 - 1) / r_min0 + ws->K + kpw - 1) / kpw;
            if (dgrid > lgrid) dgrid = lgrid;
            const char* dname = "";
            span_begin(ws, kSpanMstepMain, st);
            e = launch_mstep_list(ws->T, (int)dgrid, st, ld, &dname);
            span_end(ws, st);
            if (e != hipSuccess) return fail(GMMVB_EHIP, "settled-row delta launch", e);
            span_begin(ws, kSpanReduce, st);
            hipLaunchKernelGGL(reduce_chunks_kernel, dim3((elems0 + 255) / 256, ws->K), dim3(256), 0, st, ws->slabs, ws->plan_m,
                               ws->K, ws->D, ws->T, ws->cache, 1, nullptr);
            span_end(ws, st);
            ws->delta_pending = false;
            ws->active_lists = false;
            ws->mlists_done = false;
        }
        if (ws->lock_live) {
            if (!ws->mlists_done) {
                if (ws->mlists_lost)
                    return fail(GMMVB_ESTATE, "the M-step's lists were used by a read-out of settled rows: call gmmvb_estep again");
                span_begin(ws, kSpanLists, st);
                scan_and_fill(ws, st, ws->mmask, ws->mblk, nblk, n_rows, ws->K, ws->e_state == 1 ? ws->qpart : nullptr);
                e = hipGetLastError();
                span_end(ws, st);
                if (e != hipSuccess) return fail(GMMVB_EHIP, "active-sample lists", e);
                ws->mlists_done = true;
                ws->active_lists = false;
            }
        } else if (!ws->active_lists) {
            span_begin(ws, kSpanLists, st);
            scan_and_fill(ws, st, ws->masks, ws->blk, nblk, n_rows, ws->K);
            e = hipGetLastError();
            span_end(ws, st);
            if (e != hipSuccess) return fail(GMMVB_EHIP, "active-sample lists", e);
            ws->active_lists = true;
            ws->blk_fresh = false;
        }
        grid = lgrid;
        S = 0;
        rows_per_split = r_min0;
        const MstepListArgs& la = la0;
        span_begin(ws, kSpanMstepMain, st);
        e = launch_mstep_list(ws->T, (int)grid, st, la, &name);
        span_end(ws, st);
        ++ws->passes[6];
    } else {
        ++ws->passes[5];
        if (phase_events(ws)) note_hip(ws, hipEventRecord(ws->ev[2], st));
        if (pre && ws->xc_stale) {
            e = recenter_rows(ws, n_rows, st);
            if (e != hipSuccess) return fail(GMMVB_EHIP, "center_rows launch", e);
        }
        span_begin(ws, kSpanMstepMain, st);
        if (ws->T == 1 && pre) {
            constexpr int kSmallCw = 8;
            const int per_wg = 4 * kSmallCw;
            const int KGW = (ws->K + per_wg - 1) / per_wg;
            grid = 8 * ((S + 7) / 8) * KGW;
            if (hmm_small)
                e = launch_hmm_mstep_small((int)grid, st, a, KGW, hmm_gamma_tm(ws->hmm), hmm_padded_states(ws->hmm),
                                           !ws->opt_hmm_mstep_dense, &name);
            else
                e = launch_mstep_small((int)grid, st, a, KGW, kSmallCw, &name);
        } else {
            const bool cal = a.direct_r == 0 && cal_wanted(ws, 1, (double)n_rows * ws->K);
            if (cal) note_hip(ws, hipEventRecord(ws->cal_ev[2], st));
            e = launch_mstep(ws->T, ws->x_dtype == GMMVB_F64, vec, pre, (int)grid, st, a, &name);
            if (cal) cal_mark(ws, 1, (double)n_rows * ws->K, st);
        }
        span_end(ws, st);
    }
    if (e != hipSuccess) return fail(GMMVB_EHIP, "mstep launch", e);
    if (phase_events(ws)) {
        note_hip(ws, hipEventRecord(ws->ev[3], st));
        ws->ev_m = true;
    }
    const int elems = tri_pairs(ws->T) * 256 + 16 * ws->T + 2;
    span_begin(ws, kSpanReduce, st);
    if (sparse)
        hipLaunchKernelGGL(reduce_chunks_kernel, dim3((elems + 255) / 256, ws->K), dim3(256), 0, st, ws->slabs, ws->plan_m,
                           ws->K, ws->D, ws->T, stats_dev, 0, ws->lock_live ? ws->cache : nullptr);
    else
        hipLaunchKernelGGL(reduce_stats_kernel, dim3((elems + 255) / 256, ws->K), dim3(256), 0, st, ws->slabs, (int)S,
                           ws->K, ws->D, ws->T, stats_dev);
    span_end(ws, st);
    e = hipGetLastError();
    if (e != hipSuccess) return fail(GMMVB_EHIP, "reduce_stats launch", e);
    const size_t used = std::strlen(ws->info);
    std::snprintf(ws->info + used, sizeof(ws->info) - used, " | %s grid=%lldx%d splits=%lld rows/split=%lld", name,
                  (long long)grid, mstep_threads(ws->T, pre), (long long)S, (long long)rows_per_split);
    return take_hip(ws, "event record inside the M-step");
}

int gmmvb_estep_mstep(gmmvb_workspace* ws, const void* x_dev, int64_t ldx, int64_t n_rows, double* stats_dev,
                      void* stream) {
    int rc = gmmvb_estep(ws, x_dev, ldx, n_rows, stream);
    if (rc) return rc;
    return gmmvb_mstep(ws, x_dev, ldx, n_rows, stats_dev, stream);
}

}
```

### bayesml_amd/csrc/records.h

```cpp
#pragma once
#include <type_traits>
#include "aux_kernels.h"

namespace gmmvb {

__device__ __forceinline__ void rec_insert(float (&ds)[kRecSlots], unsigned short (&ks)[kRecSlots], float (&vs)[kRecSlots],
                                           float& rest, float cd, unsigned short ck, float cv) {
    if (!(cd < ds[kRecSlots - 1])) {
        if (ck != kRecEmpty && !(ck & kRecListed)) rest = (cv > rest || cv != cv) ? cv : rest;
        return;
    }
#pragma unroll
    for (int j = 0; j < kRecSlots; ++j) {
        const bool lt = cd < ds[j];
        const float td = lt ? ds[j] : cd, tv = lt ? vs[j] : cv;
        const unsigned short tk = lt ? ks[j] : ck;
        ds[j] = lt ? cd : ds[j];
        vs[j] = lt ? cv : vs[j];
        ks[j] = lt ? ck : ks[j];
        cd = td;
        cv = tv;
        ck = tk;
    }
    if (ck != kRecEmpty && !(ck & kRecListed)) rest = (cv > rest || cv != cv) ? cv : rest;
}

template <bool GIVEN>
__global__ __launch_bounds__(256) void rec_build_kernel(const double* __restrict__ lnrho, int64_t npad, int64_t n_rows,
                                                        int K, const double* __restrict__ cvec,
                                                        const int* __restrict__ khat, RecArrays rec,
                                                        float* __restrict__ ub32 ) {
    const int64_t n = (int64_t)blockIdx.x * 256 + threadIdx.x;
    if (n >= n_rows) return;
    float ds[kRecSlots], vs[kRecSlots];
    unsigned short ks[kRecSlots];
#pragma unroll
    for (int j = 0; j < kRecSlots; ++j) {
        ds[j] = __builtin_huge_valf();
        vs[j] = -__builtin_huge_valf();
        ks[j] = kRecEmpty;
    }
    float rest = -__builtin_huge_valf();
    const int kb = GIVEN ? khat[n] : -1;
    for (int k0 = 0; k0 < K; k0 += 8) {
        double pre[8];
#pragma unroll
        for (int q = 0; q < 8; ++q) {
            if (k0 + q >= K) pre[q] = 0.0;
            else if (GIVEN) pre[q] = (double)ub32[(int64_t)(k0 + q) * npad + n];
            else pre[q] = lnrho[(int64_t)(k0 + q) * npad + n];
        }
#pragma unroll
        for (int q = 0; q < 8; ++q) {
            const int k = k0 + q;
            if (k >= K) break;
            const double v = pre[q];
            if (!GIVEN) ub32[(int64_t)k * npad + n] = f32_up(v);
            if (GIVEN && k == kb) continue;
            rec_insert(ds, ks, vs, rest, f32_down(dist_of(cvec[k], v)), (unsigned short)k, f32_up(v));
        }
    }
    unsigned ex = 0;
    if (GIVEN) {
        const int at = kRecSlots - 1;
        if (ks[at] != kRecEmpty) rest = (vs[at] > rest || vs[at] != vs[at]) ? vs[at] : rest;
        ks[at] = (unsigned short)kb;
        const double vb = lnrho[(int64_t)kb * npad + n];
        ds[at] = f32_down(dist_of(cvec[kb], vb));
        ub32[(int64_t)kb * npad + n] = f32_up(vb);
        ex = 1u << at;
    } else {
#pragma unroll
        for (int j = 0; j < kRecSlots; ++j) ex |= (ks[j] != kRecEmpty) ? (1u << j) : 0u;
    }
#pragma unroll
    for (int j = 0; j < kRecSlots; ++j) {
        rec.k[(int64_t)j * rec.npad + n] = ks[j];
        rec.d[(int64_t)j * rec.npad + n] = ds[j];
    }
    rec.B[n] = rest;
    rec.exact[n] = (unsigned char)ex;
    rec.sel[n] = 0;
    rec.flags[n] = 0;
}

static __global__ __launch_bounds__(kSelRows) void rec_select_kernel(RecArrays rec, int64_t n_rows, int K,
                                                              const double* __restrict__ cvec,
                                                              unsigned long long* __restrict__ masks, int64_t npad,
                                                              int* __restrict__ blk_cnt, double* __restrict__ epart,
                                                              double* __restrict__ opart,
                                                              float* __restrict__ rthr ) {
    __shared__ int wcnt[4][256];
    __shared__ double sc[256];
    __shared__ int wsum[2][4];
    const int tid = threadIdx.x, wave = tid >> 6;
    const int W = (K + 63) / 64;
    for (int k = tid & 63; k < K; k += 64) wcnt[wave][k] = 0;
    for (int k = tid; k < K; k += kSelRows) sc[k] = cvec[k];
    __syncthreads();
    const int64_t n = (int64_t)blockIdx.x * kSelRows + tid;
    const bool valid = n < n_rows;
    unsigned long long mk[4] = {0ull, 0ull, 0ull, 0ull};
    int listed = 0, over_i = 0;
    if (valid) {
        const unsigned ex = rec.exact[n];
        const double ninf = -__builtin_huge_val();
        double lb = ninf;
        double ub[kRecSlots];
        unsigned short kk[kRecSlots];
#pragma unroll
        for (int j = 0; j < kRecSlots; ++j) {
            const unsigned short k = rec.k[(int64_t)j * rec.npad + n];
            kk[j] = k;
            ub[j] = ninf;
            if (k == kRecEmpty) continue;
            const double d = (double)rec.d[(int64_t)j * rec.npad + n];
            const float yf = f32_down(d * (1.0 - 1e-12));
            const double c = sc[k];
            ub[j] = c - 0.5 * (double)yf * (double)yf * (1.0 - 1e-12) + 1e-12 * fabs(c);
            if ((ex >> j) & 1u) {
                const double du = d * (1.0 + 2.4e-7) * (1.0 + 1e-12);
                const double l = c - 0.5 * du * du * (1.0 + 1e-12) - 1e-12 * fabs(c);
                lb = l > lb ? l : lb;
            }
        }
        const double thr = lb - kRelNats;
        unsigned sel = 0;
#pragma unroll
        for (int j = 0; j < kRecSlots; ++j) {
            if (kk[j] == kRecEmpty || ((ex >> j) & 1u)) continue;
            if (!(ub[j] < thr)) {
                sel |= 1u << j;
                mk[kk[j] >> 6] |= 1ull << (kk[j] & 63);
                ++listed;
            }
        }
        const double B = (double)rec.B[n];
        bool over = !(lb > ninf);
        int extra = 0;
        if (!over && (B > ninf || B != B) && !(B < thr)) {
            unsigned long long inslot[4] = {0ull, 0ull, 0ull, 0ull};
#pragma unroll
            for (int j = 0; j < kRecSlots; ++j)
                if (kk[j] != kRecEmpty) inslot[kk[j] >> 6] |= 1ull << (kk[j] & 63);
            for (int k = 0; k < K; ++k) {
                if ((inslot[k >> 6] >> (k & 63)) & 1ull) continue;
                mk[k >> 6] |= 1ull << (k & 63);
                ++extra;
            }
            rec.B[n] = -__builtin_huge_valf();
            over = extra > 24;
        }
        listed += extra;
        if (over) {
            for (int w = 0; w < W; ++w) mk[w] = (K - 64 * w >= 64) ? ~0ull : ((1ull << (K - 64 * w)) - 1ull);
            listed = K;
            over_i = 1;
            sel = 0;
        }
        rec.sel[n] = (unsigned char)sel;
        rec.flags[n] = (unsigned char)(over ? 1 : (extra > 0 ? 2 : 0));
        rthr[n] = (over || !(thr > ninf)) ? -__builtin_huge_valf() : f32_down(thr);
        for (int w = 0; w < W; ++w) masks[(int64_t)w * npad + n] = mk[w];
    }
    for (int w = 0; w < W; ++w) count_word(mk[w], w, wave, wcnt);
#pragma unroll
    for (int o = 32; o > 0; o >>= 1) {
        listed += __shfl_xor(listed, o);
        over_i += __shfl_xor(over_i, o);
    }
    if ((tid & 63) == 0) {
        wsum[0][wave] = listed;
        wsum[1][wave] = over_i;
    }
    __syncthreads();
    for (int k = tid; k < K; k += kSelRows)
        blk_cnt[blk_at(k, blockIdx.x, K)] = wcnt[0][k] + wcnt[1][k] + wcnt[2][k] + wcnt[3][k];
    if (tid == 0) {
        epart[blockIdx.x] = (double)(wsum[0][0] + wsum[0][1] + wsum[0][2] + wsum[0][3]);
        opart[blockIdx.x] = (double)(wsum[1][0] + wsum[1][1] + wsum[1][2] + wsum[1][3]);
    }
}


__device__ __forceinline__ float sweep_carry(float old, float4 p) {
    const float qd = p.w - old;
    const float sq = __builtin_amdgcn_sqrtf(qd + qd);
    const float t = fmaxf(fmaf(p.x, sq, -p.y), 0.0f);
    const float w = fminf(t * t * 0.4999995f, 3.0e38f);
    const float r = p.z - w;
    return fmaf(fabsf(r), 2.4e-7f, r);
}

__device__ __forceinline__ float max_f32_raw(float a, float b) {
    float r;
    asm("v_max_f32 %0, %1, %2" : "=v"(r) : "v"(a), "v"(b));
    return r;
}

__device__ __forceinline__ float wave_max_f32(float v) {
    asm volatile(
        "s_nop 1\n\t"
        "v_max_f32_dpp %0, %0, %0 quad_perm:[1,0,3,2] row_mask:0xf bank_mask:0xf\n\t"
        "s_nop 1\n\t"
        "v_max_f32_dpp %0, %0, %0 quad_perm:[2,3,0,1] row_mask:0xf bank_mask:0xf\n\t"
        "s_nop 1\n\t"
        "v_max_f32_dpp %0, %0, %0 row_half_mirror row_mask:0xf bank_mask:0xf\n\t"
        "s_nop 1\n\t"
        "v_max_f32_dpp %0, %0, %0 row_mirror row_mask:0xf bank_mask:0xf\n\t"
        "s_nop 1"
        : "+v"(v));
    const float a = __builtin_bit_cast(float, __builtin_amdgcn_readlane(__builtin_bit_cast(int, v), 0));
    const float b = __builtin_bit_cast(float, __builtin_amdgcn_readlane(__builtin_bit_cast(int, v), 16));
    const float c = __builtin_bit_cast(float, __builtin_amdgcn_readlane(__builtin_bit_cast(int, v), 32));
    const float d = __builtin_bit_cast(float, __builtin_amdgcn_readlane(__builtin_bit_cast(int, v), 48));
    return max_f32_raw(max_f32_raw(a, b), max_f32_raw(c, d));
}

template <bool PREV, bool LAZY = false, int WC = 0>
__global__ __launch_bounds__(kSelRows, (LAZY && WC >= 3 ? 5 : 1)) void rec_sweep_kernel(float* __restrict__ ub, const double* __restrict__ u, int64_t npad,
                                                             int64_t n_rows, int K,
                                                             const double* __restrict__ drift,
                                                             const double* __restrict__ c_new,
                                                             const int* __restrict__ khat, RecArrays rec,
                                                             unsigned long long* __restrict__ masks,
                                                             int* __restrict__ blk_cnt, double* __restrict__ epart,
                                                             double* __restrict__ opart,
                                                             unsigned char* __restrict__ lock ,
                                                             float* __restrict__ dlock,
                                                             float* __restrict__ rthr ,
                                                             const unsigned char* __restrict__ lcomp ,
                                                             unsigned long long* __restrict__ pmask ,
                                                             int* __restrict__ pblk,
                                                             int proof_all ,
                                                             int own_fresh ,
                                                             float4* __restrict__ tmeta = nullptr ,
                                                             int tmeta_reset = 0 ,
                                                             unsigned long long* __restrict__ col_ctr = nullptr ,
                                                             double* __restrict__ ppre = nullptr ) {
    static_assert(!LAZY || PREV, "the lazy sweep is a form of the PREV sweep");
    __shared__ int wcnt[4][256];
    __shared__ int pcnt[4][256];
    __shared__ float4 sp[256];
    __shared__ float2 sq[256];
    __shared__ double sc[256];
    __shared__ unsigned char sfirst[256];
    __shared__ float s_delta[256];
    __shared__ int wsum[3][4];
    __shared__ unsigned char s_force[LAZY ? 256 : 1];
    __shared__ float s_thr[LAZY ? 4 : 1];
    __shared__ unsigned long long s_open[LAZY ? 4 : 1];
    __shared__ unsigned long long s_redo[LAZY ? 4 : 1];
    __shared__ unsigned long long s_keep[LAZY ? 4 : 1];
    __shared__ unsigned long long s_any[LAZY ? 4 : 1][4];
    __shared__ float s_red[LAZY ? 4 : 1][LAZY ? 256 : 1];
    __shared__ float s_skip[LAZY ? 4 : 1];
    const int tid = threadIdx.x, wave = tid >> 6, lane = tid & 63;
    const int W = WC > 0 ? WC : (K + 63) / 64;
    const int64_t n = (int64_t)blockIdx.x * kSelRows + tid;
    const bool valid = n < n_rows;
    unsigned long long fresh[4] = {0ull, 0ull, 0ull, 0ull};
    unsigned lk_pre = 0u;
    int kset_pre = 0;
    float dl_pre = 0.0f;
    double lb_pre = 0.0;
    float4 meta_pre = make_float4(0.0f, 0.0f, 0.0f, 0.0f);
    if (valid && PREV) {
        for (int w = 0; w < W; ++w) fresh[w] = masks[(int64_t)w * npad + n];
        if (lock != nullptr) {
            lk_pre = lock[n];
            kset_pre = lcomp[n];
            dl_pre = dlock[n];
            if (own_fresh && lk_pre == 1u) lb_pre = u[(int64_t)kset_pre * npad + n];
        }
    }
    if constexpr (LAZY)
        if (tid < K && !tmeta_reset) meta_pre = tmeta[(int64_t)blockIdx.x * K + tid];
    for (int k = lane; k < K; k += 64) wcnt[wave][k] = pcnt[wave][k] = 0;
    float4 step = make_float4(0.0f, 0.0f, 0.0f, 0.0f);
    for (int k = tid; k < K; k += kSelRows) {
        sfirst[k] = (own_fresh && own_first(drift[3 * K + k], drift[K + k])) ? 1 : 0;
        const double g = drift[k] * (1.0 - 1e-6);
        step = make_float4(g > 0.0 ? f32_down(g) : 0.0f, f32_up(drift[K + k]), f32_up(c_new[k]), f32_down(drift[2 * K + k]));
        if constexpr (!LAZY) sp[k] = step;
        s_delta[k] = step.y;
        sq[k] = make_float2(f32_up(drift[3 * K + k] * (1.0 + 1e-6)), f32_down(c_new[k]));
        sc[k] = c_new[k];
        if constexpr (LAZY) s_force[k] = 0;
    }
    const double ninf = -__builtin_huge_val();
    double vb = ninf;
    if (valid && PREV) {
        for (int w = 0; w < W; ++w) {
            unsigned long long m = fresh[w];
            while (m) {
                const int b = __builtin_ctzll(m);
                m &= m - 1;
                const double v = u[(int64_t)(64 * w + b) * npad + n];
                vb = (v > vb || v != v) ? v : vb;
            }
        }
    }
    __syncthreads();
    unsigned long long mk[4] = {0ull, 0ull, 0ull, 0ull};
    unsigned long long pm[4] = {0ull, 0ull, 0ull, 0ull};
    int listed = 0, over_i = 0;
    unsigned long long nocand[4] = {0ull, 0ull, 0ull, 0ull};
    bool by_bound = false, over = false;
    int kset = -1;
    float d_set = 0.0f, thr_f = __builtin_huge_valf();
    if (valid) {
        const int kb = PREV ? -1 : khat[n];
        if constexpr (!PREV) {
            fresh[kb >> 6] = 1ull << (kb & 63);
            vb = u[(int64_t)kb * npad + n];
        }
        const double thr = vb - kRelNats;
        by_bound = PREV && lock != nullptr && lk_pre == 1u && (fresh[0] | fresh[1] | fresh[2] | fresh[3]) == 0ull;
        float thr_set = 0.0f;
        if (by_bound) {
            kset = kset_pre;
            float dn;
            if (sfirst[kset]) {
                const double lbn = lb_pre;
                dn = f32_up(dist_of(sc[kset], lbn) * (1.0 + 1e-9));
            } else {
                dn = fmaf(sq[kset].x, dl_pre, s_delta[kset]) * (1.0f + 2.4e-7f);
            }
            const float lb = sq[kset].y - dn * dn * 0.5000005f;
            d_set = dn;
            thr_set = (lb - fabsf(lb) * 2.4e-7f) - ((float)kRelevanceNats + 0.2f);
        }
        over = !by_bound && !(thr > ninf);
        thr_f = by_bound ? thr_set : (over ? -__builtin_huge_valf() : f32_down(thr));
        if (over) fresh[0] = fresh[1] = fresh[2] = fresh[3] = 0ull;
        rthr[n] = thr_f;
#pragma unroll
        for (int w = 0; w < 4; ++w) nocand[w] = fresh[w];
        if (by_bound) nocand[kset >> 6] |= 1ull << (kset & 63);
    }
    float4 meta = make_float4(0.0f, 0.0f, 0.0f, 0.0f), comp = meta;
    bool col_open = false, col_forced = false, col_redo = false, col_keep = false;
    float col_bound = 0.0f;
    if constexpr (LAZY) {
        if (valid) {
            for (int w = 0; w < W; ++w) {
                unsigned long long m = nocand[w];
                while (m) {
                    const int b = __builtin_ctzll(m);
                    m &= m - 1;
                    s_force[64 * w + b] = 1;
                }
            }
        }
        float tmin = thr_f == thr_f ? thr_f : -__builtin_huge_valf();
#pragma unroll
        for (int o = 32; o > 0; o >>= 1) tmin = fminf(tmin, __shfl_xor(tmin, o));
        if (lane == 0) s_thr[wave] = tmin;
        __syncthreads();
        const float tile_thr = fminf(fminf(s_thr[0], s_thr[1]), fminf(s_thr[2], s_thr[3]));
        float skip = -__builtin_huge_valf();
        if (tid < K) {
            const int k = tid;
            meta = tmeta_reset ? make_float4(__builtin_huge_valf(), 1.0f, 0.0f, step.w) : meta_pre;
            comp = make_float4(f32_down((double)meta.y * (double)step.x),
                               f32_up(((double)step.x * (double)meta.z + (double)step.y) * (1.0 + 1e-15)), step.z, meta.w);
            col_bound = sweep_carry(meta.x, comp);
            col_forced = s_force[k] != 0;
            const bool unknown = !(meta.x < __builtin_huge_valf());
            col_open = col_forced || unknown || !(col_bound < tile_thr);
            col_redo = col_open && unknown && !col_forced;
            col_keep = col_open && !unknown && !col_forced;
            sp[k] = comp;
            if (!col_open) {
                tmeta[(int64_t)blockIdx.x * K + k] = make_float4(meta.x, comp.x, comp.y, meta.w);
                skip = col_bound;
            }
        }
        const unsigned long long ob = __builtin_amdgcn_ballot_w64(col_open), rb = __builtin_amdgcn_ballot_w64(col_redo);
        const unsigned long long kb2 = __builtin_amdgcn_ballot_w64(col_keep);
#pragma unroll
        for (int o = 32; o > 0; o >>= 1) skip = fmaxf(skip, __shfl_xor(skip, o));
        if (lane == 0) {
            s_open[wave] = ob;
            s_redo[wave] = rb;
            s_keep[wave] = kb2;
            s_skip[wave] = skip;
            if (col_ctr && ob) atomicAdd(col_ctr, (unsigned long long)__builtin_popcountll(ob));
        }
        __syncthreads();
    }
    unsigned long long anyw[4] = {0ull, 0ull, 0ull, 0ull};
    float mine[4] = {-__builtin_huge_valf(), -__builtin_huge_valf(), -__builtin_huge_valf(), -__builtin_huge_valf()};
    bool stays = false;
    {
        unsigned s[kRecSlots + 1];
#pragma unroll
        for (int j = 0; j <= kRecSlots; ++j) s[j] = 0xFFFFFFFFu;
        float restmax = -__builtin_huge_valf();
        const bool near = npad < (int64_t(1) << 29);
        const unsigned off = (unsigned)(near ? (valid ? n : 0) : 0) * 4u;
        const int64_t nn = valid ? n : 0;
        unsigned long long red_w = 0ull, keep_w = 0ull;
        float mine_w = -__builtin_huge_valf();
        const bool need_chain = !LAZY || __builtin_amdgcn_ballot_w64(valid && !by_bound) != 0ull;
        auto pair = [&](auto ch, int k, int bit, float old, unsigned long long fw, unsigned long long nw, unsigned long long& mw,
                        unsigned long long& aw) {
            constexpr bool CH = decltype(ch)::value;
            const float ubn = sweep_carry(old, sp[k]);
            char* base = (char*)(ub + (int64_t)k * npad + (near ? 0 : nn));
            const unsigned long long b1 = 1ull << bit;
            if (valid && !(LAZY && (keep_w & b1) != 0ull)) *(float*)(base + off) = ubn;
            const bool isf = (fw & b1) != 0ull;
            const bool cand = valid && !(ubn < thr_f) && (nw & b1) == 0ull;
            mw |= cand ? b1 : 0ull;
            restmax = max_f32_raw(restmax, (cand || isf) ? -__builtin_huge_valf() : ubn);
            if constexpr (CH) sweep_chain(s, (isf || !valid) ? 0xFFFFFFFFu : sweep_key(ubn, (unsigned)k));
            if constexpr (LAZY) {
                aw |= __builtin_amdgcn_ballot_w64(cand) != 0ull ? b1 : 0ull;
                if (red_w & b1) {
                    const float m = wave_max_f32(valid ? ubn : -__builtin_huge_valf());
                    mine_w = lane == bit ? m : mine_w;
                }
            }
        };
        auto old_of = [&](int k) {
            const char* base = (const char*)(ub + (int64_t)k * npad + (near ? 0 : nn));
            return *(const float*)(base + off);
        };
        for (int w = 0; w < W; ++w) {
            const unsigned long long fw = w == 0 ? fresh[0] : (w == 1 ? fresh[1] : (w == 2 ? fresh[2] : fresh[3]));
            const unsigned long long nw = w == 0 ? nocand[0] : (w == 1 ? nocand[1] : (w == 2 ? nocand[2] : nocand[3]));
            unsigned long long mw = 0ull, aw = 0ull;
            if constexpr (LAZY) {
                const unsigned long long o0 = s_open[w];
                unsigned long long ow = ((unsigned long long)(unsigned)__builtin_amdgcn_readfirstlane((int)(o0 >> 32)) << 32) |
                                        (unsigned)__builtin_amdgcn_readfirstlane((int)o0);
                const unsigned long long r0 = s_redo[w];
                red_w = ((unsigned long long)(unsigned)__builtin_amdgcn_readfirstlane((int)(r0 >> 32)) << 32) |
                        (unsigned)__builtin_amdgcn_readfirstlane((int)r0);
                const unsigned long long q0 = s_keep[w];
                keep_w = ((unsigned long long)(unsigned)__builtin_amdgcn_readfirstlane((int)(q0 >> 32)) << 32) |
                         (unsigned)__builtin_amdgcn_readfirstlane((int)q0);
                mine_w = -__builtin_huge_valf();
                auto columns = [&](auto ch) {
                    while (ow) {
                        int kq[8];
#pragma unroll
                        for (int q = 0; q < 8; ++q) {
                            kq[q] = ow ? __builtin_ctzll(ow) : -1;
                            ow &= ow - 1;
                        }
                        float pre[8];
#pragma unroll
                        for (int q = 0; q < 8; ++q)
                            if (kq[q] >= 0) pre[q] = old_of(64 * w + kq[q]);
#pragma unroll
                        for (int q = 0; q < 8; ++q)
                            if (kq[q] >= 0) pair(ch, 64 * w + kq[q], kq[q], pre[q], fw, nw, mw, aw);
                    }
                };
                if (need_chain) columns(std::true_type{});
                else columns(std::false_type{});
                if (w == 0) mine[0] = mine_w;
                else if (w == 1) mine[1] = mine_w;
                else if (w == 2) mine[2] = mine_w;
                else mine[3] = mine_w;
            } else {
                if (valid) {
                    const int kend = K < 64 * w + 64 ? K : 64 * w + 64;
                    int k0 = 64 * w;
                    for (; k0 + 8 <= kend; k0 += 8) {
                        float pre[8];
#pragma unroll
                        for (int q = 0; q < 8; ++q) pre[q] = old_of(k0 + q);
#pragma unroll
                        for (int q = 0; q < 8; ++q) pair(std::true_type{}, k0 + q, k0 + q - 64 * w, pre[q], fw, nw, mw, aw);
                    }
                    for (; k0 < kend; ++k0) pair(std::true_type{}, k0, k0 - 64 * w, old_of(k0), fw, nw, mw, aw);
                }
            }
            if (w == 0) { mk[0] = mw; anyw[0] = aw; }
            else if (w == 1) { mk[1] = mw; anyw[1] = aw; }
            else if (w == 2) { mk[2] = mw; anyw[2] = aw; }
            else { mk[3] = mw; anyw[3] = aw; }
        }
        if (valid) {
        bool proof_row = false, proof_cand = false;
        if (pmask != nullptr && proof_all && !by_bound && !over && (mk[0] | mk[1] | mk[2] | mk[3]) != 0ull) {
#pragma unroll
            for (int w = 0; w < 4; ++w) {
                pm[w] = mk[w];
                mk[w] = 0ull;
            }
            proof_cand = true;
        }
        if (by_bound) {
            stays = (mk[0] | mk[1] | mk[2] | mk[3]) == 0ull;
            if (stays) {
                dlock[n] = d_set;
            } else if (pmask != nullptr) {
#pragma unroll
                for (int w = 0; w < 4; ++w) {
                    pm[w] = mk[w];
                    mk[w] = 0ull;
                }
                if (!sfirst[kset]) pm[kset >> 6] |= 1ull << (kset & 63);
                proof_row = true;
                dlock[n] = d_set;
            } else {
                mk[kset >> 6] |= 1ull << (kset & 63);
                rthr[n] = -__builtin_huge_valf();
            }
        }
        unsigned sel = 0, ex = 0;
        int in_slots = 0;
        if (!(LAZY && stays)) {
        if (LAZY && by_bound) {
#pragma unroll
            for (int j = 0; j <= kRecSlots; ++j) s[j] = 0xFFFFFFFFu;
        }
        for (int w = 0; w < W; ++w) {
            unsigned long long m = fresh[w];
            while (m) {
                const int b = __builtin_ctzll(m);
                m &= m - 1;
                const int k = 64 * w + b;
                const float fu = f32_up(u[(int64_t)k * npad + n]);
                ub[(int64_t)k * npad + n] = fu;
                sweep_chain(s, PREV ? sweep_key(fu, (unsigned)k) : (unsigned)k);
            }
        }
        float ds[kRecSlots];
        unsigned short ks[kRecSlots];
        unsigned long long in_slot[4] = {0ull, 0ull, 0ull, 0ull};
#pragma unroll
        for (int j = 0; j < kRecSlots; ++j) {
            ks[j] = kRecEmpty;
            ds[j] = __builtin_huge_valf();
            if (s[j] == 0xFFFFFFFFu) continue;
            const int k = (int)(s[j] & 0xFFu);
            ks[j] = (unsigned short)k;
            const unsigned long long bit = 1ull << (k & 63);
            const int kw = WC == 1 ? 0 : (k >> 6);
            if (fresh[kw] & bit) {
                in_slot[kw] |= bit;
                ex |= 1u << j;
                ds[j] = f32_down(dist_of(sc[k], PREV ? u[(int64_t)k * npad + n] : vb));
            } else {
                ds[j] = dist_lower_f32(sc[k], (double)sweep_key_bound(s[j]));
                if (mk[kw] & bit) {
                    sel |= 1u << j;
                    ++in_slots;
                }
            }
        }
        for (int w = 0; w < W; ++w) {
            mk[w] |= fresh[w] & ~in_slot[w];
            listed += __builtin_popcountll(mk[w]);
        }
        float rest = -__builtin_huge_valf();
        if (s[kRecSlots] != 0xFFFFFFFFu) {
            const int k9 = (int)(s[kRecSlots] & 0xFFu);
            rest = ((mk[k9 >> 6] >> (k9 & 63)) & 1ull) ? restmax : sweep_key_bound(s[kRecSlots]);
        }
        if constexpr (LAZY) {
            if (by_bound) rest = restmax;
            rest = fmaxf(rest, fmaxf(fmaxf(s_skip[0], s_skip[1]), fmaxf(s_skip[2], s_skip[3])));
        }
        {
#pragma unroll
            for (int j = 0; j < kRecSlots; ++j) {
                rec.k[(int64_t)j * rec.npad + n] = ks[j];
                rec.d[(int64_t)j * rec.npad + n] = ds[j];
            }
            rec.B[n] = rest;
            rec.exact[n] = (unsigned char)(over ? 0 : ex);
            rec.sel[n] = (unsigned char)(over ? 0 : sel);
        }
        }
        rec.flags[n] = (unsigned char)(stays ? 4 : (proof_row ? 8 : (over ? 1 : ((listed > in_slots ? 2 : 0) | (proof_cand ? 16 : 0)))));
        over_i = over ? 1 : 0;
        for (int w = 0; w < W; ++w) {
            masks[(int64_t)w * npad + n] = mk[w];
            if (pmask) pmask[(int64_t)w * npad + n] = pm[w];
        }
        }
    }
    int plisted = 0;
    for (int w = 0; w < W; ++w) {
        count_word(mk[w], w, wave, wcnt);
        if (pmask) count_word(pm[w], w, wave, pcnt);
        plisted += __builtin_popcountll(pm[w]);
    }
#pragma unroll
    for (int o = 32; o > 0; o >>= 1) {
        listed += __shfl_xor(listed, o);
        over_i += __shfl_xor(over_i, o);
        plisted += __shfl_xor(plisted, o);
    }
    if (lane == 0) {
        wsum[0][wave] = listed;
        wsum[1][wave] = over_i;
        wsum[2][wave] = plisted;
    }
    if constexpr (LAZY) {
        if (lane == 0)
            for (int w = 0; w < 4; ++w) s_any[wave][w] = anyw[w];
        for (int w = 0; w < W; ++w) s_red[wave][64 * w + lane] = w == 0 ? mine[0] : (w == 1 ? mine[1] : (w == 2 ? mine[2] : mine[3]));
    }
    __syncthreads();
    if constexpr (LAZY) {
        for (int w = 0; w < W; ++w) {
            unsigned long long fix = s_keep[w] & (s_any[0][w] | s_any[1][w] | s_any[2][w] | s_any[3][w]);
            while (fix) {
                const int b = __builtin_ctzll(fix);
                fix &= fix - 1;
                const int k = 64 * w + b;
                if (valid) {
                    float* e = ub + (int64_t)k * npad + n;
                    *e = sweep_carry(*e, sp[k]);
                }
            }
        }
        if (tid < K && col_open) {
            const int k = tid, w = k >> 6;
            const bool any = (((s_any[0][w] | s_any[1][w] | s_any[2][w] | s_any[3][w]) >> (k & 63)) & 1ull) != 0ull;
            if (col_keep && !any) {
                tmeta[(int64_t)blockIdx.x * K + k] = make_float4(meta.x, comp.x, comp.y, meta.w);
            } else {
                float tub = col_bound;
                if (col_redo) tub = fmaxf(fmaxf(s_red[0][k], s_red[1][k]), fmaxf(s_red[2][k], s_red[3][k]));
                if (col_forced || any) tub = __builtin_huge_valf();
                tmeta[(int64_t)blockIdx.x * K + k] = make_float4(tub, 1.0f, 0.0f, sq[k].y);
            }
        }
    }
    for (int k = tid; k < K; k += kSelRows) {
        blk_cnt[blk_at(k, blockIdx.x, K)] = wcnt[0][k] + wcnt[1][k] + wcnt[2][k] + wcnt[3][k];
        if (pmask) pblk[blk_at(k, blockIdx.x, K)] = pcnt[0][k] + pcnt[1][k] + pcnt[2][k] + pcnt[3][k];
    }
    if (tid == 0) {
        epart[blockIdx.x] = (double)(wsum[0][0] + wsum[0][1] + wsum[0][2] + wsum[0][3]);
        opart[blockIdx.x] = (double)(wsum[1][0] + wsum[1][1] + wsum[1][2] + wsum[1][3]);
        if (ppre) ppre[blockIdx.x] = (double)(wsum[2][0] + wsum[2][1] + wsum[2][2] + wsum[2][3]);
    }
}

static __global__ __launch_bounds__(kSelRows) void rec_proof_decide_kernel(RecArrays rec, const unsigned long long* __restrict__ pmask,
                                                                    unsigned long long* __restrict__ masks, int64_t npad,
                                                                    int64_t n_rows, int K, const double* __restrict__ cvec,
                                                                    const float* __restrict__ ub32, const double* __restrict__ lb,
                                                                    const unsigned char* __restrict__ lcomp,
                                                                    float* __restrict__ dlock, float* __restrict__ rthr,
                                                                    int* __restrict__ blk_cnt, double* __restrict__ epart,
                                                                    double* __restrict__ ppart,
                                                                    const double* __restrict__ own_part ) {
    __shared__ int wcnt[4][256];
    __shared__ int wsum[2][4];
    const int tid = threadIdx.x, wave = tid >> 6;
    const int W = (K + 63) / 64;
    for (int k = tid & 63; k < K; k += 64) wcnt[wave][k] = 0;
    const int64_t n = (int64_t)blockIdx.x * kSelRows + tid;
    const bool valid = n < n_rows;
    unsigned long long mk[4] = {0ull, 0ull, 0ull, 0ull}, old[4] = {0ull, 0ull, 0ull, 0ull};
    int listed = 0, proved = 0;
    const unsigned fl0 = valid ? rec.flags[n] : 0u;
    if (valid && ((fl0 & 16u) || fl0 == 8u)) {
        for (int w = 0; w < W; ++w) old[w] = mk[w] = masks[(int64_t)w * npad + n];
        if (fl0 & 16u) {
            const double thr = (double)rthr[n];
            unsigned sel = rec.sel[n];
            int in_slots = __builtin_popcount(sel), total = 0;
            unsigned long long kept[4] = {0ull, 0ull, 0ull, 0ull};
            for (int w = 0; w < W; ++w) {
                unsigned long long m = pmask[(int64_t)w * npad + n];
                proved += __builtin_popcountll(m);
                while (m) {
                    int b[4];
                    float uf[4];
#pragma unroll
                    for (int q = 0; q < 4; ++q) {
                        b[q] = m ? __builtin_ctzll(m) : -1;
                        m &= m - 1;
                    }
#pragma unroll
                    for (int q = 0; q < 4; ++q) uf[q] = b[q] >= 0 ? ub32[(int64_t)(64 * w + b[q]) * npad + n] : 0.0f;
#pragma unroll
                    for (int q = 0; q < 4; ++q)
                        if (b[q] >= 0 && !((double)uf[q] < thr)) kept[w] |= 1ull << b[q];
                }
            }
            unsigned long long done[4] = {0ull, 0ull, 0ull, 0ull};
            for (int w = 0; w < W; ++w) done[w] = pmask[(int64_t)w * npad + n] & ~kept[w];
#pragma unroll
            for (int j = 0; j < kRecSlots; ++j) {
                const unsigned short k = rec.k[(int64_t)j * rec.npad + n];
                if (k == kRecEmpty) continue;
                if (((kept[k >> 6] >> (k & 63)) & 1ull) && !((sel >> j) & 1u)) {
                    sel |= 1u << j;
                    ++in_slots;
                } else if ((done[k >> 6] >> (k & 63)) & 1ull) {
                    rec.d[(int64_t)j * rec.npad + n] = dist_lower_f32(cvec[k], (double)ub32[(int64_t)k * npad + n]);
                    done[k >> 6] &= ~(1ull << (k & 63));
                }
            }
            float done_max = -__builtin_huge_valf();
            for (int w = 0; w < W; ++w) {
                unsigned long long m = done[w];
                while (m) {
                    const int b = __builtin_ctzll(m);
                    m &= m - 1;
                    done_max = fmaxf(done_max, ub32[(int64_t)(64 * w + b) * npad + n]);
                }
            }
            if (done_max > rec.B[n]) rec.B[n] = done_max;
            for (int w = 0; w < W; ++w) {
                mk[w] |= kept[w];
                total += __builtin_popcountll(mk[w]);
                masks[(int64_t)w * npad + n] = mk[w];
            }
            rec.sel[n] = (unsigned char)sel;
            rec.flags[n] = (unsigned char)(total > in_slots ? 2 : 0);
        }
        if (fl0 == 8u) {
            const int kset = lcomp[n];
            const double l = lb[(int64_t)kset * npad + n];
            const double thr = l - kRelNats;
            unsigned long long kept[4] = {0ull, 0ull, 0ull, 0ull};
            bool any = false;
            float done_max = -__builtin_huge_valf();
            for (int w = 0; w < W; ++w) {
                unsigned long long m = pmask[(int64_t)w * npad + n];
                proved += __builtin_popcountll(m);
                if ((kset >> 6) == w) m &= ~(1ull << (kset & 63));
                while (m) {
                    int b[4];
                    float uf[4];
#pragma unroll
                    for (int q = 0; q < 4; ++q) {
                        b[q] = m ? __builtin_ctzll(m) : -1;
                        m &= m - 1;
                    }
#pragma unroll
                    for (int q = 0; q < 4; ++q) uf[q] = b[q] >= 0 ? ub32[(int64_t)(64 * w + b[q]) * npad + n] : 0.0f;
#pragma unroll
                    for (int q = 0; q < 4; ++q) {
                        if (b[q] < 0) continue;
                        if (!((double)uf[q] < thr)) {
                            kept[w] |= 1ull << b[q];
                            any = true;
                        } else {
                            done_max = fmaxf(done_max, uf[q]);
                        }
                    }
                }
            }
            if (!any && l > -__builtin_huge_val()) {
                rec.flags[n] = 4;
                dlock[n] = f32_up(dist_of(cvec[kset], l) * (1.0 + 1e-9));
            } else {
                kept[kset >> 6] |= 1ull << (kset & 63);
                unsigned sel = 0;
                int in_slots = 0, total = 0;
#pragma unroll
                for (int j = 0; j < kRecSlots; ++j) {
                    const unsigned short k = rec.k[(int64_t)j * rec.npad + n];
                    if (k != kRecEmpty && ((kept[k >> 6] >> (k & 63)) & 1ull)) {
                        sel |= 1u << j;
                        ++in_slots;
                    }
                }
                for (int w = 0; w < W; ++w) {
                    mk[w] = kept[w];
                    total += __builtin_popcountll(kept[w]);
                    masks[(int64_t)w * npad + n] = kept[w];
                }
                rec.sel[n] = (unsigned char)sel;
                rec.exact[n] = 0;
                rec.flags[n] = (unsigned char)(total > in_slots ? 2 : 0);
                const float Bn = rec.B[n];
                if (done_max > Bn) rec.B[n] = done_max;
                rthr[n] = -__builtin_huge_valf();
            }
        }
        for (int w = 0; w < W; ++w) {
            mk[w] &= ~old[w];
            listed += __builtin_popcountll(mk[w]);
        }
    }
    for (int w = 0; w < W; ++w) count_word(mk[w], w, wave, wcnt);
#pragma unroll
    for (int o = 32; o > 0; o >>= 1) {
        listed += __shfl_xor(listed, o);
        proved += __shfl_xor(proved, o);
    }
    if ((tid & 63) == 0) {
        wsum[0][wave] = listed;
        wsum[1][wave] = proved;
    }
    __syncthreads();
    const int joined = wsum[0][0] + wsum[0][1] + wsum[0][2] + wsum[0][3];
    if (joined != 0)
        for (int k = tid; k < K; k += kSelRows) {
            const int c = wcnt[0][k] + wcnt[1][k] + wcnt[2][k] + wcnt[3][k];
            if (c != 0) blk_cnt[blk_at(k, blockIdx.x, K)] += c;
        }
    if (tid == 0) {
        if (joined != 0) epart[blockIdx.x] += (double)joined;
        ppart[blockIdx.x] = (double)(wsum[1][0] + wsum[1][1] + wsum[1][2] + wsum[1][3]) + (own_part ? own_part[blockIdx.x] : 0.0);
    }
}

static __global__ __launch_bounds__(kSelRows) void rec_prune_kernel(RecArrays rec, unsigned long long* __restrict__ masks, int64_t npad,
                                                             int64_t n_rows, int K, const double* __restrict__ cvec,
                                                             const float* __restrict__ ub32, const float* __restrict__ rthr,
                                                             int* __restrict__ blk_cnt, double* __restrict__ epart,
                                                             double* __restrict__ ppart) {
    __shared__ int wcnt[4][256];
    __shared__ int wsum[2][4];
    const int tid = threadIdx.x, wave = tid >> 6;
    const int W = (K + 63) / 64;
    for (int k = tid & 63; k < K; k += 64) wcnt[wave][k] = 0;
    const int64_t n = (int64_t)blockIdx.x * kSelRows + tid;
    const bool valid = n < n_rows;
    unsigned long long mk[4] = {0ull, 0ull, 0ull, 0ull};
    int listed = 0, proved = 0;
    if (valid) {
        for (int w = 0; w < W; ++w) mk[w] = masks[(int64_t)w * npad + n];
        const unsigned fl = rec.flags[n];
        if (fl != 1u && (mk[0] | mk[1] | mk[2] | mk[3]) != 0ull) {
            const double thr = (double)rthr[n];
            unsigned long long inslot[4] = {0ull, 0ull, 0ull, 0ull};
            unsigned sel = rec.sel[n];
            float rest = rec.B[n];
            bool changed = false;
#pragma unroll
            for (int j = 0; j < kRecSlots; ++j) {
                const unsigned short k = rec.k[(int64_t)j * rec.npad + n];
                if (k == kRecEmpty) continue;
                inslot[k >> 6] |= 1ull << (k & 63);
                if (!((sel >> j) & 1u)) continue;
                const float u = ub32[(int64_t)k * npad + n];
                if ((double)u < thr) {
                    sel &= ~(1u << j);
                    mk[k >> 6] &= ~(1ull << (k & 63));
                    rec.d[(int64_t)j * rec.npad + n] = dist_lower_f32(cvec[k], (double)u);
                    changed = true;
                }
                ++proved;
            }
            int extra = 0;
            for (int w = 0; w < W; ++w) {
                unsigned long long m = mk[w] & ~inslot[w];
                while (m) {
                    const int b = __builtin_ctzll(m);
                    m &= m - 1;
                    const float u = ub32[(int64_t)(64 * w + b) * npad + n];
                    ++proved;
                    if ((double)u < thr) {
                        mk[w] &= ~(1ull << b);
                        rest = (u > rest) ? u : rest;
                        changed = true;
                    } else {
                        ++extra;
                    }
                }
            }
            if (changed) {
                for (int w = 0; w < W; ++w) masks[(int64_t)w * npad + n] = mk[w];
                rec.sel[n] = (unsigned char)sel;
                rec.B[n] = rest;
                rec.flags[n] = (unsigned char)(extra > 0 ? 2 : 0);
            }
        }
        for (int w = 0; w < W; ++w) listed += __builtin_popcountll(mk[w]);
    }
    for (int w = 0; w < W; ++w) count_word(mk[w], w, wave, wcnt);
#pragma unroll
    for (int o = 32; o > 0; o >>= 1) {
        listed += __shfl_xor(listed, o);
        proved += __shfl_xor(proved, o);
    }
    if ((tid & 63) == 0) {
        wsum[0][wave] = listed;
        wsum[1][wave] = proved;
    }
    __syncthreads();
    for (int k = tid; k < K; k += kSelRows)
        blk_cnt[blk_at(k, blockIdx.x, K)] = wcnt[0][k] + wcnt[1][k] + wcnt[2][k] + wcnt[3][k];
    if (tid == 0) {
        epart[blockIdx.x] = (double)(wsum[0][0] + wsum[0][1] + wsum[0][2] + wsum[0][3]);
        ppart[blockIdx.x] = (double)(wsum[1][0] + wsum[1][1] + wsum[1][2] + wsum[1][3]);
    }
}

static __global__ void gather_plan_kernel(const int* __restrict__ counts, int K, int per_wg, int* __restrict__ first) {
    __shared__ int sc[1025];
    if (blockIdx.x != 0) return;
    if (K > 1024) {
        if (threadIdx.x != 0) return;
        int total = 0;
        for (int k = 0; k < K; ++k) {
            first[k] = total;
            total += (counts[k] + per_wg - 1) / per_wg;
        }
        first[K] = total;
        return;
    }
    for (int k = threadIdx.x; k < K; k += blockDim.x) sc[k] = (counts[k] + per_wg - 1) / per_wg;
    __syncthreads();
    if (threadIdx.x == 0) {
        int total = 0;
        for (int k = 0; k < K; ++k) {
            const int c = sc[k];
            sc[k] = total;
            total += c;
        }
        sc[K] = total;
    }
    __syncthreads();
    for (int k = threadIdx.x; k <= K; k += blockDim.x) first[k] = sc[k];
}

static __global__ __launch_bounds__(kSelRows) void rec_finish_kernel(RecArrays rec, const double* __restrict__ lnrho, int64_t npad,
                                                              int64_t n_rows, int K, const double* __restrict__ cvec,
                                                              double* __restrict__ lse, int* __restrict__ khat,
                                                              unsigned long long* __restrict__ masks,
                                                              int* __restrict__ blk_cnt, double* __restrict__ apart,
                                                              double* __restrict__ mpart ,
                                                              float* __restrict__ ub32 ,
                                                              unsigned char* __restrict__ lock ,
                                                              float* __restrict__ dlock, double settle_margin ,
                                                              unsigned long long* __restrict__ dmask, int* __restrict__ dblk,
                                                              unsigned long long* __restrict__ mmask, int* __restrict__ mblk,
                                                              double* __restrict__ spart, double* __restrict__ gpart,
                                                              double* __restrict__ qpart ,
                                                              const float* __restrict__ rthr ,
                                                              unsigned char* __restrict__ lcomp ) {
    __shared__ int wcnt[4][256];
    __shared__ int dcnt[4][256];
    __shared__ int mcnt[4][256];
    __shared__ int wact[4], wmov[4], wset[4], wlist[4], wacc[4];
    const int tid = threadIdx.x, wave = tid >> 6;
    const int W = (K + 63) / 64;
    for (int k = tid & 63; k < K; k += 64) wcnt[wave][k] = dcnt[wave][k] = mcnt[wave][k] = 0;
    const int64_t n = (int64_t)blockIdx.x * kSelRows + tid;
    const bool valid = n < n_rows;
    unsigned long long mk[4] = {0ull, 0ull, 0ull, 0ull};
    unsigned long long dm[4] = {0ull, 0ull, 0ull, 0ull};
    int active = 0, settled_i = 0;
    const int khat_before = valid ? khat[n] : 0;
    const unsigned fl = valid ? rec.flags[n] : 0u;
    double row_l = 0.0, row_best = 0.0, row_second = __builtin_huge_val();
    int row_arg = -1;
    const double thr_row = valid ? (double)rthr[n] : 0.0;
    if (valid && fl == 4u) {
        active = 1;
        settled_i = 1;
    } else if (valid && fl == 2u) {
        const unsigned live = (unsigned)rec.sel[n] | (unsigned)rec.exact[n];
        float ds[kRecSlots], vs[kRecSlots];
        unsigned short ks[kRecSlots];
#pragma unroll
        for (int j = 0; j < kRecSlots; ++j) {
            ds[j] = __builtin_huge_valf();
            vs[j] = -__builtin_huge_valf();
            ks[j] = kRecEmpty;
        }
        float rest = rec.B[n];
        unsigned long long cand[4] = {0ull, 0ull, 0ull, 0ull}, ev[4] = {0ull, 0ull, 0ull, 0ull};
        for (int w = 0; w < W; ++w) cand[w] = masks[(int64_t)w * npad + n];
        double mx = -__builtin_huge_val(), ssum = 0.0;
        int arg = 0x7fffffff;
        bool nan = false;
        auto take_exact = [&](int k) {
            const double x = lnrho[(int64_t)k * npad + n];
            ub32[(int64_t)k * npad + n] = f32_up(x);
            ev[k >> 6] |= 1ull << (k & 63);
            nan = nan || x != x;
            if (x > mx) {
                ssum = fma(ssum, exp(mx - x), 1.0);
                arg = k;
                mx = x;
            } else {
                if (x == mx && k < arg) arg = k;
                ssum += exp(x - mx);
            }
            rec_insert(ds, ks, vs, rest, f32_down(dist_of(cvec[k], x)),
                       (unsigned short)(k | (x < thr_row ? 0 : kRecExactBit)), f32_up(x));
        };
#pragma unroll
        for (int j = 0; j < kRecSlots; ++j) {
            const unsigned short k = rec.k[(int64_t)j * rec.npad + n];
            if (k == kRecEmpty) continue;
            cand[k >> 6] &= ~(1ull << (k & 63));
            if ((live >> j) & 1u) {
                take_exact(k);
            } else {
                const float d = rec.d[(int64_t)j * rec.npad + n];
                rec_insert(ds, ks, vs, rest, d, k, f32_up(cvec[k] - 0.5 * (double)d * (double)d));
            }
        }
        for (int w = 0; w < W; ++w) {
            unsigned long long m = cand[w];
            while (m) {
                const int b = __builtin_ctzll(m);
                m &= m - 1;
                take_exact(64 * w + b);
            }
        }
        double l = mx + log(ssum);
        if (nan) l = __builtin_nan("");
        lse[n] = l;
        khat[n] = arg == 0x7fffffff ? 0 : arg;
        unsigned ex = 0;
#pragma unroll
        for (int j = 0; j < kRecSlots; ++j) {
            const bool e1 = ks[j] != kRecEmpty && (ks[j] & kRecExactBit);
            rec.k[(int64_t)j * rec.npad + n] = ks[j] == kRecEmpty ? kRecEmpty : (unsigned short)(ks[j] & kRecCompMask);
            rec.d[(int64_t)j * rec.npad + n] = ds[j];
            ex |= e1 ? (1u << j) : 0u;
        }
        rec.B[n] = rest;
        rec.exact[n] = (unsigned char)ex;
        for (int w = 0; w < W; ++w) {
            unsigned long long m = ev[w];
            while (m) {
                const int b = __builtin_ctzll(m);
                m &= m - 1;
                const double t = lnrho[(int64_t)(64 * w + b) * npad + n] - l;
                if (!(t < -kRelNats)) {
                    mk[w] |= 1ull << b;
                    ++active;
                }
            }
        }
        if (!nan) {
            float sec = rest;
#pragma unroll
            for (int j = 0; j < kRecSlots; ++j)
                if (ks[j] != kRecEmpty && (int)(ks[j] & kRecCompMask) != arg) sec = (vs[j] > sec || vs[j] != vs[j]) ? vs[j] : sec;
            row_l = l;
            row_best = mx;
            row_arg = arg == 0x7fffffff ? -1 : arg;
            row_second = (double)sec;
        }
    } else if (valid && fl == 0u) {
        unsigned live = (unsigned)rec.sel[n] | (unsigned)rec.exact[n];
        unsigned bounds_only = 0;
        double v[kRecSlots];
        unsigned short kk[kRecSlots];
        double mx = -__builtin_huge_val();
        int arg = 0x7fffffff;
        bool nan = false;
#pragma unroll
        for (int j = 0; j < kRecSlots; ++j) kk[j] = rec.k[(int64_t)j * rec.npad + n];
#pragma unroll
        for (int j = 0; j < kRecSlots; ++j)
            v[j] = ((live >> j) & 1u) ? lnrho[(int64_t)kk[j] * npad + n] : 0.0;
#pragma unroll
        for (int j = 0; j < kRecSlots; ++j) {
            if (!((live >> j) & 1u)) continue;
            const double x = v[j];
            ub32[(int64_t)kk[j] * npad + n] = f32_up(x);
            rec.d[(int64_t)j * rec.npad + n] = f32_down(dist_of(cvec[kk[j]], x));
            if (x < thr_row) bounds_only |= 1u << j;
            nan = nan || x != x;
            if (x > mx || (x == mx && (int)kk[j] < arg)) {
                mx = x;
                arg = kk[j];
            }
        }
        double s = 0.0;
#pragma unroll
        for (int j = 0; j < kRecSlots; ++j)
            if ((live >> j) & 1u) s += exp(v[j] - mx);
        double l = mx + log(s);
        if (nan) {
            l = __builtin_nan("");
            arg = arg == 0x7fffffff ? 0 : arg;
        }
        lse[n] = l;
        khat[n] = arg == 0x7fffffff ? 0 : arg;
        rec.exact[n] = (unsigned char)(live & ~bounds_only);
#pragma unroll
        for (int j = 0; j < kRecSlots; ++j) {
            if (!((live >> j) & 1u)) continue;
            if (!(v[j] - l < -kRelNats)) {
                mk[kk[j] >> 6] |= 1ull << (kk[j] & 63);
                ++active;
            }
        }
        if (!nan) {
            row_l = l;
            row_best = mx;
            row_arg = arg == 0x7fffffff ? -1 : arg;
        }
        if (!nan && active == 1 && settle_margin >= 0.0 && lock != nullptr) {
            double sec = (double)rec.B[n];
#pragma unroll
            for (int j = 0; j < kRecSlots; ++j) {
                if (kk[j] == kRecEmpty || (int)kk[j] == arg) continue;
                double o = v[j];
                if (!((live >> j) & 1u)) {
                    const double d = (double)rec.d[(int64_t)j * rec.npad + n];
                    o = cvec[kk[j]] - 0.5 * d * d * (1.0 - 1e-6);
                }
                sec = (o > sec || o != o) ? o : sec;
            }
            row_second = sec;
        }
    } else if (valid) {
        float ds[kRecSlots], vs[kRecSlots];
        unsigned short ks[kRecSlots];
#pragma unroll
        for (int j = 0; j < kRecSlots; ++j) {
            ds[j] = __builtin_huge_valf();
            vs[j] = -__builtin_huge_valf();
            ks[j] = kRecEmpty;
        }
        float rest = -__builtin_huge_valf();
        double mx = lnrho[n], s = 1.0;
        int arg = 0;
        ub32[n] = f32_up(mx);
        rec_insert(ds, ks, vs, rest, f32_down(dist_of(cvec[0], mx)), 0, f32_up(mx));
        for (int k = 1; k < K; ++k) {
            const double x = lnrho[(int64_t)k * npad + n];
            ub32[(int64_t)k * npad + n] = f32_up(x);
            rec_insert(ds, ks, vs, rest, f32_down(dist_of(cvec[k], x)), (unsigned short)k, f32_up(x));
            if (x > mx) {
                s = fma(s, exp(mx - x), 1.0);
                mx = x;
                arg = k;
            } else {
                s += exp(x - mx);
            }
        }
        const double l = mx + log(s);
        lse[n] = l;
        khat[n] = arg;
        row_l = l;
        row_best = mx;
        row_arg = (l == l) ? arg : -1;
        unsigned ex = 0;
#pragma unroll
        for (int j = 0; j < kRecSlots; ++j) {
            rec.k[(int64_t)j * rec.npad + n] = ks[j];
            rec.d[(int64_t)j * rec.npad + n] = ds[j];
            ex |= (ks[j] != kRecEmpty) ? (1u << j) : 0u;
        }
        rec.B[n] = rest;
        rec.exact[n] = (unsigned char)ex;
        rec.sel[n] = (unsigned char)ex;
        for (int k = 0; k < K; ++k) {
            const double t = lnrho[(int64_t)k * npad + n] - l;
            if (!(t < -kRelNats)) {
                mk[k >> 6] |= 1ull << (k & 63);
                ++active;
            }
        }
    }
    unsigned long long mm[4] = {mk[0], mk[1], mk[2], mk[3]};
    int in_lists = 0, m_pairs = 0;
    if (valid && lock != nullptr && fl != 4u) {
        const unsigned lk = lock[n];
        const bool single = row_arg >= 0 && active == 1;
        if (lk == 1u) {
            const int was = lcomp[n];
            if (!(single && row_arg == was)) {
                dm[was >> 6] |= 1ull << (was & 63);
                if (single) dm[row_arg >> 6] |= 1ull << (row_arg & 63);
                lock[n] = single ? 4 : 2;
            }
        } else if (single) {
            dm[row_arg >> 6] |= 1ull << (row_arg & 63);
            lock[n] = 3;
        }
        if (single) {
            lcomp[n] = (unsigned char)row_arg;
            mm[row_arg >> 6] &= ~(1ull << (row_arg & 63));
            if (settle_margin >= 1e300 || (settle_margin >= 0.0 && row_second < row_l - kRelNats - settle_margin)) {
                dlock[n] = f32_up(dist_of(cvec[row_arg], row_best) * (1.0 + 1e-9));
                mk[row_arg >> 6] &= ~(1ull << (row_arg & 63));
            }
        }
    }
    if (valid) {
        for (int w = 0; w < W; ++w) {
            masks[(int64_t)w * npad + n] = mk[w];
            in_lists += __builtin_popcountll(mk[w]);
            m_pairs += __builtin_popcountll(mm[w]) + __builtin_popcountll(dm[w]);
            if (dmask) {
                dmask[(int64_t)w * npad + n] = dm[w];
                mmask[(int64_t)w * npad + n] = mm[w];
            }
        }
    }
    for (int w = 0; w < W; ++w) {
        count_word<false>(mk[w], w, wave, wcnt);
        if (dmask) {
            count_word<false>(dm[w], w, wave, dcnt);
            count_word<false>(mm[w], w, wave, mcnt);
        }
    }
    int moved = (valid && khat[n] != khat_before) ? 1 : 0;
#pragma unroll
    for (int o = 32; o > 0; o >>= 1) {
        active += __shfl_xor(active, o);
        moved += __shfl_xor(moved, o);
        settled_i += __shfl_xor(settled_i, o);
        in_lists += __shfl_xor(in_lists, o);
        m_pairs += __shfl_xor(m_pairs, o);
    }
    if ((tid & 63) == 0) {
        wact[wave] = active;
        wmov[wave] = moved;
        wset[wave] = settled_i;
        wlist[wave] = in_lists;
        wacc[wave] = m_pairs;
    }
    __syncthreads();
    for (int k = tid; k < K; k += kSelRows) {
        blk_cnt[blk_at(k, blockIdx.x, K)] = wcnt[0][k] + wcnt[1][k] + wcnt[2][k] + wcnt[3][k];
        if (dblk) {
            dblk[blk_at(k, blockIdx.x, K)] = dcnt[0][k] + dcnt[1][k] + dcnt[2][k] + dcnt[3][k];
            mblk[blk_at(k, blockIdx.x, K)] = mcnt[0][k] + mcnt[1][k] + mcnt[2][k] + mcnt[3][k];
        }
    }
    if (tid == 0) {
        apart[blockIdx.x] = (double)(wact[0] + wact[1] + wact[2] + wact[3]);
        mpart[blockIdx.x] = (double)(wmov[0] + wmov[1] + wmov[2] + wmov[3]);
        spart[blockIdx.x] = (double)(wset[0] + wset[1] + wset[2] + wset[3]);
        gpart[blockIdx.x] = (double)(wlist[0] + wlist[1] + wlist[2] + wlist[3]);
        qpart[blockIdx.x] = (double)(wacc[0] + wacc[1] + wacc[2] + wacc[3]);
    }
}

static __global__ __launch_bounds__(1024) void sum_parts_kernel(const double* __restrict__ apart, const double* __restrict__ epart,
                                                         const double* __restrict__ opart, const double* __restrict__ mpart,
                                                         const double* __restrict__ spart, const double* __restrict__ gpart,
                                                         const double* __restrict__ qpart, const double* __restrict__ ppart,
                                                         int blocks, double* __restrict__ ctr) {
    __shared__ double part[16];
    const double* src = blockIdx.x == 0 ? apart : (blockIdx.x == 1 ? epart : (blockIdx.x == 2 ? opart :
                        (blockIdx.x == 3 ? mpart : (blockIdx.x == 4 ? spart : (blockIdx.x == 5 ? gpart :
                        (blockIdx.x == 6 ? qpart : ppart))))));
    if (!src) return;
    double a = 0.0;
    for (int b = threadIdx.x; b < blocks; b += 1024) a += src[b];
#pragma unroll
    for (int o = 32; o > 0; o >>= 1) a += __shfl_xor(a, o);
    if ((threadIdx.x & 63) == 0) part[threadIdx.x >> 6] = a;
    __syncthreads();
    if (threadIdx.x == 0) {
        double t = 0.0;
        for (int i = 0; i < 16; ++i) t += part[i];
        ctr[blockIdx.x] = t;
    }
}

__device__ __forceinline__ bool row_settled(const unsigned char* __restrict__ lock,
                                            const unsigned long long* __restrict__ emask, int64_t npad, int W, int64_t n) {
    if (lock[n] != 1) return false;
    unsigned long long any = 0ull;
    for (int w = 0; w < W; ++w) any |= emask[(int64_t)w * npad + n];
    return any == 0ull;
}

static __global__ __launch_bounds__(kSelRows) void settled_mask_kernel(const unsigned char* __restrict__ lock,
                                                                const unsigned long long* __restrict__ emask,
                                                                const unsigned char* __restrict__ lcomp, int64_t npad, int64_t n_rows,
                                                                int K, unsigned long long* __restrict__ masks,
                                                                int* __restrict__ blk_cnt,
                                                                const double* __restrict__ drift = nullptr ,
                                                                double* __restrict__ listed_part = nullptr ) {
    __shared__ int wcnt[4][256];
    const int64_t n = (int64_t)blockIdx.x * kSelRows + threadIdx.x;
    const bool valid = n < n_rows;
    const int W = (K + 63) / 64;
    const int wave = threadIdx.x >> 6;
    for (int k = threadIdx.x & 63; k < K; k += 64) wcnt[wave][k] = 0;
    const int64_t nn = valid ? n : 0;
    const unsigned lk = lock[nn];
    const int lc = (int)lcomp[nn];
    unsigned long long any = 0ull;
    for (int w = 0; w < W; ++w) any |= emask[(int64_t)w * npad + nn];
    int kh = (valid && lk == 1u && any == 0ull) ? lc : -1;
    if (kh >= 0 && drift != nullptr && !own_first(drift[3 * K + kh], drift[K + kh])) kh = -1;
    for (int w = 0; w < W; ++w) {
        const unsigned long long mk = (kh >= 0 && (kh >> 6) == w) ? 1ull << (kh & 63) : 0ull;
        if (valid) masks[(int64_t)w * npad + n] = mk;
        count_word(mk, w, wave, wcnt);
    }
    __syncthreads();
    int tot = 0;
    for (int k = threadIdx.x; k < K; k += kSelRows) {
        const int c = wcnt[0][k] + wcnt[1][k] + wcnt[2][k] + wcnt[3][k];
        blk_cnt[blk_at(k, blockIdx.x, K)] = c;
        tot += c;
    }
    if (listed_part) {
        __shared__ int wtot[4];
#pragma unroll
        for (int o = 32; o > 0; o >>= 1) tot += __shfl_xor(tot, o);
        if ((threadIdx.x & 63) == 0) wtot[wave] = tot;
        __syncthreads();
        if (threadIdx.x == 0) listed_part[blockIdx.x] = (double)(wtot[0] + wtot[1] + wtot[2] + wtot[3]);
    }
}

static __global__ void settled_lse_kernel(const unsigned char* __restrict__ lock, const unsigned long long* __restrict__ emask,
                                   const unsigned char* __restrict__ lcomp, const double* __restrict__ lnrho, int64_t npad,
                                   int64_t n_rows, int K, double* __restrict__ lse) {
    const int64_t n = (int64_t)blockIdx.x * blockDim.x + threadIdx.x;
    if (n < n_rows && row_settled(lock, emask, npad, (K + 63) / 64, n)) lse[n] = lnrho[(int64_t)lcomp[n] * npad + n];
}

static __global__ void rec_readout_kernel(RecArrays rec, const unsigned long long* __restrict__ masks,
                                   const double* __restrict__ lnrho, const double* __restrict__ lse,
                                   const double* __restrict__ cvec, int64_t npad, int64_t row0, int64_t n_rows, int K,
                                   int mode, double* __restrict__ out, const int* __restrict__ iperm,
                                   const unsigned char* __restrict__ lock, const unsigned char* __restrict__ lcomp) {
    const int64_t e = (int64_t)blockIdx.x * blockDim.x + threadIdx.x;
    if (e >= n_rows * K) return;
    const int64_t n = iperm ? iperm[row0 + e / K] : row0 + e / K;
    const int k = (int)(e % K);
    bool exact = ((masks[(int64_t)(k >> 6) * npad + n] >> (k & 63)) & 1ull) != 0 || (rec.flags[n] & 1) != 0;
    if (lock && (lock[n] == 1 || lock[n] >= 3) && (int)lcomp[n] == k) exact = true;
    if (mode == 1) {
        out[e] = exact ? exp(lnrho[(int64_t)k * npad + n] - lse[n]) : 0.0;
        return;
    }
    const bool no_record = rec.flags[n] == 4;
    double ub = no_record ? __builtin_huge_val() : (double)rec.B[n];
    if (!exact && !no_record) {
        const unsigned live = rec.exact[n];
#pragma unroll
        for (int j = 0; j < kRecSlots; ++j) {
            if (rec.k[(int64_t)j * rec.npad + n] == k) {
                exact = (live >> j) & 1u;
                const double d = (double)rec.d[(int64_t)j * rec.npad + n];
                ub = cvec[k] - 0.5 * d * d;
            }
        }
    }
    if (!exact) {
        const double cap = lse[n] - kRelNats;
        ub = cap < ub ? cap : ub;
    }
    out[e] = exact ? lnrho[(int64_t)k * npad + n] : ub;
}

}
```

### bayesml_amd/csrc/workspace.h

```cpp
#pragma once
#include "../../include/gmmvb.h"

#include <hip/hip_runtime.h>
#include <stdint.h>

#include <cstdlib>

#include "pass_plan.h"
#include "workspace_plan.h"

struct gmmvb_hmm_state;
struct gmmvb_workspace;

struct gmmvb_scratch : gmmvb::Scratch {
    gmmvb_workspace* owner = nullptr;
};

struct gmmvb_workspace : gmmvb::WorkspaceShape {
    gmmvb_scratch* scratch = nullptr;
    bool lost_estep = false;
    double* lnrho = nullptr;
    double* lse = nullptr;
    double* img = nullptr;
    double* tri = nullptr;
    unsigned char* img_i8 = nullptr;
    double* pivot_i8 = nullptr;
    unsigned char* img_i8b = nullptr;
    gmmvb::BoundLevel bound;
    double* drift = nullptr;
    bool have_drift = false;
    double typical_gamma = -1.0;
    bool params_used = false;
    int64_t bounds_rows = 0;
    const void* bounds_x = nullptr;
    int64_t bounds_ldx = 0;
    int prev_pass = 0;
    unsigned short* rec_k = nullptr;
    float* rec_d = nullptr;
    float* rec_B = nullptr;
    unsigned char* rec_exact = nullptr, *rec_sel = nullptr, *rec_flags = nullptr;
    bool rec_valid = false;
    bool rec_live = false;
    float* ub32 = nullptr;
    bool dense_valid = false;
    int sweeps = 0;
    int* plan = nullptr;
    int* plan_m = nullptr;
    double* epart = nullptr;
    double* opart = nullptr;
    double* mpart = nullptr;
    double moved_since_sort = 0.0;
    bool pend_first_sorted = false;
    double* ctr = nullptr;
    double* ctr_host = nullptr;
    hipEvent_t ctr_ev = nullptr;
    bool ctr_pending = false;
    int pend_mode = 0;
    int64_t pend_rows = 0;
    double pend_round0 = 0.0;
    bool sweep_prev = false;
    gmmvb_pass_counters lag, pol;
    gmmvb::PolicyTable pt;
    hipEvent_t cal_ev[6] = {nullptr, nullptr, nullptr, nullptr, nullptr, nullptr};
    double cal_pairs[3] = {0.0, 0.0, 0.0};
    int cal_tries[3] = {0, 0, 0};
    bool sharded = false;
    int64_t shard_rows = 0;
    int shard_ranks = 1;
    double* pol_host = nullptr;
    hipEvent_t pol_ev = nullptr;
    bool pol_pending = false;
    int pol_mode = 0;
    bool pol_first_sorted = false;
    bool exp_counted = false;
    bool forget = false;
    double spare_last = -1.0;
    double bound_fail_act = -1.0;
    double* cvec = nullptr;
    double* pivot = nullptr;
    double* dpart = nullptr;
    double* thr = nullptr;
    double* apart = nullptr;
    int64_t act_rows = 0;
    double act_host = -1.0;
    double evaluated = 0.0;
    int* lists = nullptr;
    bool active_lists = false;
    bool blk_fresh = false;
    int* khat = nullptr;
    int* counts = nullptr;
    int* blk = nullptr;
    int* scan_parts = nullptr;
    unsigned long long* masks = nullptr;
    double* slabs = nullptr;
    unsigned char* lock = nullptr;
    unsigned char* lcomp = nullptr;
    float* dlock = nullptr;
    float* rthr = nullptr;
    unsigned long long* exit_ctr = nullptr;
    unsigned long long* exit_host = nullptr;
    bool pend_lazy = false;
    unsigned long long* dmask = nullptr;
    int* dblk = nullptr;
    unsigned long long* mmask = nullptr;
    int* mblk = nullptr;
    double* cache = nullptr;
    double* spart = nullptr, *gpart = nullptr, *qpart = nullptr;
    unsigned long long* rmask = nullptr;
    int* rblk = nullptr;
    bool lock_live = false;
    bool delta_pending = false;
    bool mlists_done = false;
    bool mlists_lost = false;
    bool skip_used = false;
    bool lock_reset = false;
    bool settled_fresh = false;
    unsigned char* xq = nullptr;
    signed char* xqe = nullptr;
    const void* xq_src = nullptr;
    int64_t xq_rows = 0, xq_ldx = 0;
    int pivot_gen = 0, xq_gen = -1, img_gen = -2;
    unsigned char* gimg = nullptr;
    void* gconst = nullptr;
    int* tile_ref = nullptr;
    bool proj_table = false;
    bool tile_ref_valid = false;
    bool pend_proj = false;
    float4* tmeta = nullptr;
    bool tmeta_valid = false;
    double* ppart = nullptr;
    void* xp = nullptr;
    int* perm = nullptr, *iperm = nullptr, *perm_tmp = nullptr;
    bool sorted = false;
    int64_t sorts = 0;
    double* xc = nullptr;
    const void* xc_src = nullptr;
    int64_t xc_rows = 0, xc_ldx = 0;
    bool xc_stale = false;
    double* gen_u = nullptr;
    double* gen_m = nullptr;
    double* gen_first = nullptr;
    double* gen_second = nullptr;
    gmmvb::BufferPlan buffers;
    int64_t bytes = 0;
    bool have_params = false;
    int e_state = 0;
    int64_t e_rows = 0;
    char info[512] = {0};
    hipError_t hip_err = hipSuccess;
    int64_t passes[8] = {0, 0, 0, 0, 0, 0, 0, 0};
    bool prof = false;
    bool prof_light = false;
    bool span_open = false;
    hipEvent_t ev[4] = {nullptr, nullptr, nullptr, nullptr};
    bool ev_e = false, ev_m = false;
    static constexpr int kMaxSpans = 24;
    int n_spans = 0;
    int span_slot[kMaxSpans] = {0};
    hipEvent_t span_ev[2 * kMaxSpans] = {nullptr};
    gmmvb_hmm_state* hmm = nullptr;
    bool hmm_skip_h = false;
    bool hmm_no_lnrho = false;
    bool lse_stale = false;
};

namespace gmmvb {
inline const char* dev_env(const char* name) { return dev_switch(std::getenv, name); }
int fail(int code, const char* what, hipError_t e = hipSuccess);
void hmm_state_destroy(gmmvb_hmm_state* h);
const double* hmm_gamma_cm(const gmmvb_hmm_state* h);
const double* hmm_gamma_tm(const gmmvb_hmm_state* h);
int hmm_padded_states(const gmmvb_hmm_state* h);
bool hmm_fused_emission(const gmmvb_hmm_state* h);
hipError_t hmm_ensure_gamma_cm(gmmvb_hmm_state* h, hipStream_t st);
}
```

### bayesml_amd/csrc/workspace_plan.h

```cpp
#pragma once
#include <stdint.h>

#include <algorithm>
#include <cstdlib>
#include <cstring>
#include <vector>

#include "../../include/gmmvb.h"

namespace gmmvb {

enum EstepVariant { kEstepLds = 0, kEstepDirect = 1, kEstepLds8 = 2, kEstepI8 = 3, kEstepValu16 = 4 };
inline int64_t round_up(int64_t v, int64_t m) { return (v + m - 1) / m * m; }

inline bool not_zero(const char* v) { return !(v && std::strcmp(v, "0") == 0); }
inline bool is(const char* v, const char* word) { return v && std::strcmp(v, word) == 0; }
template <typename Lookup>
inline const char* dev_switch(Lookup&& lookup, const char* name) {
    const char* on = lookup("GMMVB_DEBUG");
    return (on && on[0] != '\0' && on[0] != '0') ? lookup(name) : nullptr;
}

struct WorkspaceOptions {
    bool sparse = true;
    int prune = 1;
    int variant_asked = -1;
    bool sort_rows = true;
    double settle_margin = 1e300;
    bool opt_proof = true;
    bool opt_proof_all = true;
    bool opt_proof_blocked = true;
    bool opt_lazy = true;
    int opt_project = 0;
    bool opt_regroup_margin = true;
    bool gather_exit = true;
    bool cache_on = true;
    bool opt_carry_off = false;
    bool opt_hmm_mstep_dense = false;
    bool opt_calibrate = true;
    bool opt_debug = false;

    template <typename Lookup>
    static WorkspaceOptions read(Lookup&& lookup) {
        auto dev = [&lookup](const char* name) { return dev_switch(lookup, name); };
        WorkspaceOptions o;
        o.sparse = not_zero(lookup("GMMVB_MSTEP_SPARSE"));
        o.prune = is(lookup("GMMVB_ESTEP_PRUNE"), "0") ? 0 : (is(lookup("GMMVB_ESTEP_PRUNE"), "force") ? 2 : 1);
        const char* variant = dev("GMMVB_ESTEP_VARIANT");
        o.variant_asked = is(variant, "lds8") ? kEstepLds8 : is(variant, "direct") ? kEstepDirect : is(variant, "lds4") ? kEstepLds
                          : is(variant, "i8") ? kEstepI8 : -1;
        o.sort_rows = not_zero(dev("GMMVB_SORT_ROWS"));
        if (const char* v = dev("GMMVB_SETTLE_MARGIN")) o.settle_margin = std::atof(v);
        o.opt_proof = not_zero(dev("GMMVB_PROOF"));
        o.opt_proof_all = !is(dev("GMMVB_PROOF"), "settled");
        o.opt_proof_blocked = not_zero(dev("GMMVB_PROOF_BLOCKED"));
        o.opt_lazy = not_zero(dev("GMMVB_SWEEP_LAZY"));
        o.opt_project = is(dev("GMMVB_PROJECT"), "filter") ? 1 : (is(dev("GMMVB_PROJECT"), "only") ? 2 : 0);
        o.opt_regroup_margin = not_zero(dev("GMMVB_REGROUP_MARGIN"));
        o.gather_exit = not_zero(dev("GMMVB_GATHER_EXIT"));
        o.cache_on = not_zero(dev("GMMVB_MSTEP_CACHE"));
        o.opt_carry_off = dev("GMMVB_ESTEP_CARRY_OFF") != nullptr;
        o.opt_hmm_mstep_dense = dev("GMMVB_HMM_MSTEP_DENSE") != nullptr;
        o.opt_calibrate = not_zero(dev("GMMVB_POLICY_CALIBRATE"));
        o.opt_debug = lookup("GMMVB_DEBUG") && lookup("GMMVB_DEBUG")[0] == '2';
        return o;
    }
};

struct KernelSizes {
    int max_tiles = 0, t1_splits = 0, sel_rows = 0, lse_rows = 0, scan_parts = 0, rec_slots = 0;
    int mstep_components_per_wg = 0;
    int slab_len = 0, estep_image_doubles = 0, estep_tri_image_doubles = 0, estep_bound_blocks = 0;
    int estep_i8_image_bytes = 0, estep_i8_bound_image_bytes = 0;
    int64_t estep_i8_digit_row_bytes = 0, proj_image_len = 0, proj_const_len = 0;
    int generic_rows = 0;
};

inline bool wide_features(int D, int max_tiles) { return D > 16 * max_tiles && D <= 32 * max_tiles; }
inline int feature_tiles(int D, int max_tiles) {
    const int T = (D + 15) / 16;
    return wide_features(D, max_tiles) ? 2 * ((T + 1) / 2) : T;
}

struct WorkspaceShape : WorkspaceOptions {
    int K = 0, D = 0, x_dtype = 0, num_cu = 0, T = 0;
    int64_t max_rows = 0, npad = 0;
    bool wide = false;
    bool generic = false;
    int KG = 0, S_cap = 0, img_len = 0, estep_variant = 0, gen_S = 1, img_i8_len = 0, img_i8b_len = 0;
    int64_t split_rows = 0, xc_len = 0;
    bool has_lists = false;
};

inline WorkspaceShape make_shape(int K, int D, int x_dtype, int64_t max_rows, int num_cu, const WorkspaceOptions& opt,
                                 const KernelSizes& ks) {
    WorkspaceShape s;
    s.K = K;
    s.D = D;
    s.x_dtype = x_dtype;
    s.max_rows = max_rows;
    s.num_cu = num_cu;
    s.T = feature_tiles(D, ks.max_tiles);
    s.wide = wide_features(D, ks.max_tiles);
    s.generic = D > 32 * ks.max_tiles;
    s.npad = round_up(max_rows, 64);
    if (s.generic) {
        s.sparse = s.sort_rows = s.cache_on = false;
        s.prune = 0;
        s.gen_S = (int)std::min<int64_t>(64, std::max<int64_t>(1, max_rows / 16384));
        return s;
    }
    static_cast<WorkspaceOptions&>(s) = opt;
    s.KG = (K + ks.mstep_components_per_wg - 1) / ks.mstep_components_per_wg;
    s.S_cap = std::max(8, (int)round_up(((int64_t)(s.T == 1 ? ks.t1_splits : 4) * num_cu + s.KG - 1) / s.KG, 8));
    s.split_rows = round_up(std::max<int64_t>(64, (16 << 20) / (16 * s.T * 8)), 64);
    s.S_cap = (int)std::max<int64_t>(s.S_cap, round_up((max_rows + s.split_rows - 1) / s.split_rows, 8));
    s.img_len = ks.estep_image_doubles;
    s.estep_variant = s.T == 1 ? kEstepValu16 : kEstepLds8;
    if (!s.wide && opt.variant_asked >= 0) s.estep_variant = opt.variant_asked;
    if (max_rows > 2000000000 || s.wide || K == 1) s.sparse = false;
    if (max_rows > 2000000000) s.sort_rows = false;
    if (!s.sparse || ks.estep_bound_blocks == 0 || K > 256) s.prune = 0;
    s.xc_len = (K == 1 && !s.wide) ? 0 : (s.npad + 64) * 16 * (int64_t)s.T;
    s.has_lists = s.sparse && K <= 256;
    if (s.estep_variant == kEstepI8) s.img_i8_len = ks.estep_i8_image_bytes;
    if (s.prune != 0) s.img_i8b_len = ks.estep_i8_bound_image_bytes;
    return s;
}

#define GMMVB_WORKSPACE_BUFFERS(X)                                                                                             \
    X(tri) X(img_i8) X(img_i8b) X(pivot_i8) X(lnrho) X(lse) X(img) X(cvec) X(pivot) X(slabs) X(xc) X(dpart) X(thr) X(apart)     \
    X(ctr) X(drift) X(lists) X(khat) X(counts) X(plan) X(plan_m) X(blk) X(scan_parts) X(masks) X(lock) X(lcomp) X(dlock)       \
    X(rthr) X(exit_ctr) X(exit_host) X(dmask) X(dblk) X(mmask) X(rmask) X(rblk) X(mblk) X(cache) X(spart) X(gpart) X(qpart)    \
    X(epart) X(opart) X(mpart) X(ppart) X(xq) X(xqe) X(gimg) X(gconst) X(tile_ref) X(rec_k) X(rec_d) X(rec_B) X(rec_exact)    \
    X(rec_sel) X(rec_flags) X(ub32) X(tmeta) X(xp) X(perm) X(iperm) X(perm_tmp) X(gen_u) X(gen_m) X(gen_first) X(gen_second)  \
    X(ctr_host)
#define GMMVB_X(name) kBuf_##name,
enum BufferId { GMMVB_WORKSPACE_BUFFERS(GMMVB_X) kBufCount };
#undef GMMVB_X
#define GMMVB_X(name) #name,
inline const char* buffer_name(int id) {
    static const char* const names[kBufCount] = {GMMVB_WORKSPACE_BUFFERS(GMMVB_X)};
    return names[id];
}
#undef GMMVB_X

enum : unsigned {
    kZeroed = 1,
    kZeroedLast = 8,
    kPinned = 2,
    kScratch = 4,
};
struct BufferSpec {
    int id;
    int64_t bytes;
    unsigned flags;
    int code;
    const char* what;
    bool counted() const { return (flags & kPinned) == 0; }
};

struct BufferPlan : std::vector<BufferSpec> {
    int code = GMMVB_ENOMEM;
    const char* what = "";
    void group(int c, const char* w) { code = c, what = w; }
    void add(int id, int64_t bytes, unsigned flags = 0) {
        if (bytes > 0) push_back(BufferSpec{id, bytes, flags, code, what});
    }
    int64_t counted_bytes() const {
        int64_t sum = 0;
        for (const BufferSpec& b : *this) sum += b.counted() ? b.bytes : 0;
        return sum;
    }
};

inline BufferPlan buffer_plan(const WorkspaceShape& s, const KernelSizes& ks, int64_t group_npad = 0) {
    const int64_t K = s.K, D = s.D, np = s.npad, f64 = 8, i32 = 4;
    BufferPlan p;
    if (s.generic) {
        p.group(GMMVB_ENOMEM, "hipMalloc (workspace)");
        p.add(kBuf_lnrho, K * np * f64, kScratch);
        p.add(kBuf_lse, np * f64);
        p.add(kBuf_cvec, K * f64);
        p.add(kBuf_pivot, D * f64, kZeroedLast);
        p.add(kBuf_gen_u, K * D * D * f64);
        p.add(kBuf_gen_m, K * D * f64);
        p.add(kBuf_gen_first, s.gen_S * K * (D + 2) * f64);
        p.add(kBuf_gen_second, s.gen_S * K * (s.T * (s.T + 1) / 2) * 256 * f64);
        p.add(kBuf_ctr, 8 * f64, kZeroedLast);
        p.group(GMMVB_EHIP, "workspace initialisation");
        p.add(kBuf_ctr_host, 8 * f64, kPinned);
        return p;
    }
    const int64_t blocks = (np + ks.sel_rows - 1) / ks.sel_rows, words = (K + 63) / 64;
    p.group(GMMVB_ENOMEM, "hipMalloc (packed triangular images)");
    if (s.estep_variant == kEstepValu16) p.add(kBuf_tri, K * ks.estep_tri_image_doubles * f64);
    p.group(GMMVB_ENOMEM, "hipMalloc (int8 images)");
    p.add(kBuf_img_i8, K * s.img_i8_len);
    p.add(kBuf_img_i8b, K * s.img_i8b_len);
    if (s.img_i8_len || s.img_i8b_len) p.add(kBuf_pivot_i8, D * f64);
    p.group(GMMVB_ENOMEM, "hipMalloc (workspace)");
    p.add(kBuf_lnrho, K * np * f64, kScratch);
    p.add(kBuf_lse, np * f64);
    p.add(kBuf_img, K * s.img_len * f64);
    p.add(kBuf_cvec, K * f64);
    p.add(kBuf_pivot, D * f64, kZeroedLast);
    p.add(kBuf_slabs, s.S_cap * K * ks.slab_len * f64, kScratch);
    p.add(kBuf_xc, s.xc_len * f64, kScratch);
    p.add(kBuf_dpart, (np + ks.lse_rows - 1) / ks.lse_rows * K * f64);
    p.add(kBuf_thr, K * f64);
    p.add(kBuf_apart, blocks * f64);
    p.add(kBuf_ctr, 8 * f64, kZeroedLast);
    p.add(kBuf_drift, 4 * K * f64);
    if (s.has_lists) {
        p.group(GMMVB_ENOMEM, "hipMalloc (sample lists / records)");
        p.add(kBuf_lists, K * (group_npad ? group_npad : np) * i32, kScratch);
        p.add(kBuf_khat, np * i32);
        p.add(kBuf_counts, K * i32);
        p.add(kBuf_plan, (K + 1) * i32);
        p.add(kBuf_plan_m, (K + 2) * i32);
        p.add(kBuf_blk, blocks * K * i32);
        p.add(kBuf_scan_parts, K * ks.scan_parts * i32);
        p.add(kBuf_masks, words * np * 8);
        p.add(kBuf_lock, np, kZeroed);
        p.add(kBuf_lcomp, np);
        p.add(kBuf_dlock, np * 4);
        p.add(kBuf_rthr, np * 4);
        p.add(kBuf_exit_ctr, 4 * 8, kZeroed);
        p.add(kBuf_exit_host, 4 * 8, kPinned | kZeroed);
        p.add(kBuf_dmask, words * np * 8);
        p.add(kBuf_dblk, blocks * K * i32);
        p.add(kBuf_mmask, words * np * 8);
        p.add(kBuf_rmask, words * np * 8);
        p.add(kBuf_rblk, blocks * K * i32);
        p.add(kBuf_mblk, blocks * K * i32);
        p.add(kBuf_cache, K * (2 + D + D * D) * f64, kZeroed);
        for (int id : {kBuf_spart, kBuf_gpart, kBuf_qpart, kBuf_epart, kBuf_opart, kBuf_mpart}) p.add(id, blocks * f64);
        p.add(kBuf_ppart, blocks * f64, kZeroed);
        if (s.prune != 0 && s.opt_proof && s.cache_on) {
            p.add(kBuf_xq, np * ks.estep_i8_digit_row_bytes);
            p.add(kBuf_xqe, np);
            if (s.opt_project != 0 && s.sort_rows && K <= ks.sel_rows && D > 32 && D <= 128) {
                p.add(kBuf_gimg, ks.proj_image_len, kZeroed);
                p.add(kBuf_gconst, ks.proj_const_len * 16);
                p.add(kBuf_tile_ref, blocks * i32);
            }
        }
        p.add(kBuf_rec_k, ks.rec_slots * np * 2);
        p.add(kBuf_rec_d, ks.rec_slots * np * 4);
        p.add(kBuf_rec_B, np * 4);
        for (int id : {kBuf_rec_exact, kBuf_rec_sel, kBuf_rec_flags}) p.add(id, np);
        p.add(kBuf_ub32, K * np * 4);
        if (s.opt_lazy && K <= ks.sel_rows) p.add(kBuf_tmeta, blocks * K * 16);
        if (s.sort_rows) {
            p.add(kBuf_xp, s.max_rows * D * (s.x_dtype == GMMVB_F64 ? 8 : 4));
            for (int id : {kBuf_perm, kBuf_iperm, kBuf_perm_tmp}) p.add(id, np * i32);
        }
    }
    p.group(GMMVB_EHIP, "workspace initialisation");
    p.add(kBuf_ctr_host, 8 * f64, kPinned);
    return p;
}

struct Scratch {
    void* buf[kBufCount] = {};
    int64_t bytes[kBufCount] = {};
    int64_t npad = 0;
    int refs = 0;
};
using BufferSlots = void** const*;

template <typename Allocator>
const BufferSpec* allocate_all(const BufferPlan& plan, BufferSlots slots, Scratch* group, Allocator& a, int64_t* counted) {
    static const BufferSpec too_large{-1, 0, 0, GMMVB_EINVAL, "a further tile must not be larger than the group's first workspace"};
    for (const BufferSpec& b : plan)
        if ((b.flags & kScratch) && group->buf[b.id] && b.bytes > group->bytes[b.id]) return &too_large;
    for (const BufferSpec& b : plan) {
        void*& p = *slots[b.id];
        if ((b.flags & kScratch) && group->buf[b.id]) {
            p = group->buf[b.id];
            continue;
        }
        p = a.get(b.bytes, (b.flags & kPinned) != 0);
        if (!p) return &b;
        if (b.flags & kScratch) {
            group->buf[b.id] = p;
            group->bytes[b.id] = b.bytes;
        }
        if (b.counted()) *counted += b.bytes;
        if ((b.flags & kZeroed) && !a.zero(p, b.bytes, (b.flags & kPinned) != 0)) return &b;
    }
    static const BufferSpec initialisation{-1, 0, 0, GMMVB_EHIP, "workspace initialisation"};
    for (const BufferSpec& b : plan)
        if ((b.flags & kZeroedLast) && !a.zero(*slots[b.id], b.bytes, false)) return &initialisation;
    return nullptr;
}

template <typename Allocator>
bool free_all(const BufferPlan& plan, BufferSlots slots, Scratch* group, Allocator& a) {
    for (const BufferSpec& b : plan) {
        void*& p = *slots[b.id];
        if (p && !(b.flags & kScratch)) a.release(p, (b.flags & kPinned) != 0);
        p = nullptr;
    }
    if (!group || --group->refs > 0) return false;
    for (void*& p : group->buf) {
        if (p) a.release(p, false);
        p = nullptr;
    }
    return true;
}

}
```

Baseline: 5.255 billion samples/s.

## Skip finish and settle-mask work for row tiles that stayed quiet two passes

The sweep kernel now counts, per 256-row tile, the rows that did not stay settled, and the proof kernel subtracts rows it returned to the settled state. A tile with zero loose rows that was also quiet on the previous pass exits early in rec_finish_kernel, writing only zeroed counts and partial sums, and settled_mask_kernel skips loading its lock and mask words. The goal is to avoid per-row finish work and memory reads for fully settled tiles. In exchange it adds cross-pass state that many code paths must invalidate, plus reuse of perm_tmp as scratch, which creates correctness risk if any invalidation is missed.

```diff
diff --git a/bayesml_amd/csrc/capi.hip b/bayesml_amd/csrc/capi.hip
--- a/bayesml_amd/csrc/capi.hip
+++ b/bayesml_amd/csrc/capi.hip
@@ -235,6 +235,7 @@
     ws->xc_src = nullptr;
     ws->xq_src = nullptr;
     ++ws->pivot_gen;
+    ws->quiet_valid = false;
     if (ws->lock_live) {
         ws->lock_live = false;
         ws->lock_reset = true;
@@ -328,6 +329,7 @@
     claim_scratch(ws);
     hipStream_t st = (hipStream_t)stream;
     ws->tmeta_valid = false;
+    ws->quiet_valid = false;
     const unsigned grid = (unsigned)((std::max<int64_t>(n_rows, ws->K) + 255) / 256);
     hipLaunchKernelGGL(debug_all_rows_kernel, dim3(grid), dim3(256), 0, st, ws->lists + (int64_t)k * ws->npad, ws->counts, ws->K, k,
                        n_rows);
@@ -356,6 +358,7 @@
     if (!ws) return fail(GMMVB_EINVAL, "null argument");
     ws->forget = true;
     ws->have_drift = false;
+    ws->quiet_valid = false;
     if (ws->lock_live) {
         ws->lock_live = false;
         ws->lock_reset = true;
@@ -420,6 +423,7 @@
             ws->lag.exits = 0.0;
             ws->lag.cols = -1.0;
             ws->lag.left = -1.0;
+            ws->lag_quiet = ws->lag_skipped = -1.0;
             ws->lag.proof = 0.0;
             ws->lag.moved = 0.0;
         } else {
@@ -427,6 +431,8 @@
             ws->lag.exits = (ws->exit_host && ws->gather_exit) ? (double)ws->exit_host[0] : 0.0;
             ws->lag.cols = (ws->exit_host && ws->pend_lazy) ? (double)ws->exit_host[1] : -1.0;
             ws->lag.left = (ws->exit_host && ws->pend_proj) ? (double)ws->exit_host[2] : -1.0;
+            ws->lag_quiet = (ws->exit_host && ws->pend_quiet) ? (double)(ws->exit_host[3] & 0xFFFFFFFFull) : -1.0;
+            ws->lag_skipped = (ws->exit_host && ws->pend_quiet) ? (double)(ws->exit_host[3] >> 32) : -1.0;
             ws->lag.settled = ws->ctr_host[4];
             ws->lag.listed = ws->ctr_host[5];
             ws->lag.accum = ws->ctr_host[6];
@@ -597,6 +603,7 @@
     if (rc) return rc;
     claim_scratch(ws);
     ws->bounds_rows = 0;
+    ws->quiet_valid = false;
     if (ws->lock_live) {
         ws->lock_live = false;
         ws->lock_reset = true;
diff --git a/bayesml_amd/csrc/capi_estep.hip b/bayesml_amd/csrc/capi_estep.hip
--- a/bayesml_amd/csrc/capi_estep.hip
+++ b/bayesml_amd/csrc/capi_estep.hip
@@ -17,11 +17,13 @@
     bool i8 = false;
     bool prunable = false;
     bool prev_lists = false, can_project = false, own_known = false, tmeta_was_valid = false;
+    bool quiet_was_valid = false;
     int mode = kPassDense;
     bool settle = false, proof_capable = false;
     double skip_margin = -1.0;
     bool counted = false, proof_ran = false, tmeta_kept = false, projected = false, filtered = false, emission_to_hmm = false,
          sorted_now = false;
+    bool quiet_swept = false;
     bool phase_closed = false;
     const char* name = "";
     int rpw = 0;
@@ -323,6 +325,9 @@
     unsigned char* lock = settle ? ws->lock : nullptr;
     unsigned long long* pmask = proof ? ws->rmask : nullptr;
     const int proof_all = ws->opt_proof_all ? 1 : 0, own_fresh = own_round ? 1 : 0;
+    int* tile_loose = can_project ? nullptr : ws->tile_loose();
+    unsigned long long* quiet_ctr = (tile_loose && ws->opt_debug) ? ws->exit_ctr + 3 : nullptr;
+    if (quiet_ctr) note_hip(ws, hipMemsetAsync(quiet_ctr, 0, sizeof(unsigned long long), st));
     if (can_project && ws->opt_project == 2) {
         note_hip(ws, hipMemsetAsync(ws->exit_ctr + 2, 0, sizeof(unsigned long long), st));
         hipError_t e = launch_rec_project(sel_grid, st, project_args(ws, n_rows, lock, pmask, proof_all, own_fresh));
@@ -335,13 +340,16 @@
             hipLaunchKernelGGL((rec_sweep_kernel<true, true, decltype(wc)::value>), dim3(sel_grid), dim3(kSelRows), 0, st, ws->ub32,
                                ws->lnrho, ws->npad, n_rows, ws->K, ws->drift, ws->cvec, ws->khat, rec, ws->masks, ws->blk,
                                ws->epart, ws->opart, lock, ws->dlock, ws->rthr, ws->lcomp, pmask, ws->rblk, proof_all, own_fresh,
-                               ws->tmeta, tmeta_was_valid ? 0 : 1, ws->exit_ctr + 1, ws->ppart);
+                               ws->tmeta, tmeta_was_valid ? 0 : 1, ws->exit_ctr + 1, ws->ppart, tile_loose, quiet_ctr);
         });
         tmeta_kept = true;
+        quiet_swept = tile_loose != nullptr;
     } else {
         hipLaunchKernelGGL(rec_sweep_kernel<true>, dim3(sel_grid), dim3(kSelRows), 0, st, ws->ub32, ws->lnrho, ws->npad, n_rows,
                            ws->K, ws->drift, ws->cvec, ws->khat, rec, ws->masks, ws->blk, ws->epart, ws->opart, lock, ws->dlock,
-                           ws->rthr, ws->lcomp, pmask, ws->rblk, proof_all, own_fresh, nullptr, 0, nullptr, ws->ppart);
+                           ws->rthr, ws->lcomp, pmask, ws->rblk, proof_all, own_fresh, nullptr, 0, nullptr, ws->ppart, tile_loose,
+                           quiet_ctr);
+        quiet_swept = tile_loose != nullptr;
     }
     return GMMVB_OK;
 }
@@ -363,7 +371,7 @@
     if (own_round) {
         span_begin(ws, kSpanSelect, st);
         hipLaunchKernelGGL(settled_mask_kernel, dim3(sel_grid), dim3(kSelRows), 0, st, ws->lock, ws->masks, ws->lcomp, ws->npad,
-                           n_rows, ws->K, ws->rmask, ws->rblk, ws->drift, ws->spart);
+                           n_rows, ws->K, ws->rmask, ws->rblk, ws->drift, ws->spart, quiet_was_valid ? ws->tile_quiet() : nullptr);
         scan_and_fill(ws, st, ws->rmask, ws->rblk, sel_grid, n_rows, ws->K, ws->spart);
         span_end(ws, st);
         span_begin(ws, kSpanProof, st);
@@ -390,7 +398,7 @@
         span_begin(ws, kSpanSelect, st);
         hipLaunchKernelGGL(rec_proof_decide_kernel, dim3(sel_grid), dim3(kSelRows), 0, st, rec, ws->rmask, ws->masks, ws->npad,
                            n_rows, ws->K, ws->cvec, ws->ub32, ws->lnrho, ws->lcomp, ws->dlock, ws->rthr, ws->blk, ws->epart,
-                           ws->ppart, own_round ? ws->spart : nullptr);
+                           ws->ppart, own_round ? ws->spart : nullptr, quiet_swept ? ws->tile_loose() : nullptr);
         proof_ran = true;
     }
     span_end(ws, st);
@@ -431,7 +439,9 @@
     hipLaunchKernelGGL(rec_finish_kernel, dim3(sel_grid), dim3(kSelRows), 0, st, rec, ws->lnrho, ws->npad, n_rows, ws->K,
                        ws->cvec, ws->lse, ws->khat, ws->masks, ws->blk, ws->apart, ws->mpart, ws->ub32,
                        settle ? ws->lock : nullptr, ws->dlock, skip_margin, settle ? ws->dmask : nullptr,
-                       settle ? ws->dblk : nullptr, ws->mmask, ws->mblk, ws->spart, ws->gpart, ws->qpart, ws->rthr, ws->lcomp);
+                       settle ? ws->dblk : nullptr, ws->mmask, ws->mblk, ws->spart, ws->gpart, ws->qpart, ws->rthr, ws->lcomp,
+                       quiet_swept ? ws->tile_loose() : nullptr, quiet_swept ? ws->tile_quiet() : nullptr, quiet_was_valid ? 1 : 0,
+                       (quiet_swept && ws->opt_debug) ? ws->exit_ctr + 3 : nullptr);
     if (!proof_ran) note_hip(ws, hipMemsetAsync(ws->ctr + 7, 0, sizeof(double), st));
     hipLaunchKernelGGL(sum_parts_kernel, dim3(proof_ran ? 8 : 7), dim3(1024), 0, st, ws->apart, ws->epart, ws->opart, ws->mpart,
                        ws->spart, ws->gpart, ws->qpart, ws->ppart, sel_grid, ws->ctr);
@@ -442,6 +452,7 @@
     ws->rec_valid = true;
     ws->rec_live = true;
     ws->evaluated = -1.0;
+    ws->quiet_valid = quiet_swept;
     if (settle) {
         ws->lock_live = true;
         ws->delta_pending = true;
@@ -453,6 +464,7 @@
     ws->tmeta_valid = tmeta_kept;
     ws->pend_lazy = tmeta_kept;
     ws->pend_proj = projected || filtered;
+    ws->pend_quiet = quiet_swept && ws->opt_debug;
     if (!phase_closed && phase_events(ws)) {
         note_hip(ws, hipEventRecord(ws->ev[1], st));
         ws->ev_e = true;
@@ -460,7 +472,7 @@
     if (counted) {
         hipError_t e = hipMemcpyAsync(ws->ctr_host, ws->ctr, 8 * sizeof(double), hipMemcpyDeviceToHost, st);
         if (e == hipSuccess && ws->exit_ctr && mode != kPassDense)
-            e = hipMemcpyAsync(ws->exit_host, ws->exit_ctr, 3 * sizeof(unsigned long long), hipMemcpyDeviceToHost, st);
+            e = hipMemcpyAsync(ws->exit_host, ws->exit_ctr, 4 * sizeof(unsigned long long), hipMemcpyDeviceToHost, st);
         if (e == hipSuccess) e = hipEventRecord(ws->ctr_ev, st);
         if (e != hipSuccess) return fail(GMMVB_EHIP, "E-step counters", e);
         ws->ctr_pending = true;
@@ -553,6 +565,7 @@
             if (e != hipSuccess) return fail(GMMVB_EHIP, "resetting the cache of single-component rows", e);
             ws->lock_live = false;
             ws->skip_used = false;
+            ws->quiet_valid = false;
         }
         ws->lock_reset = false;
         ws->delta_pending = false;
@@ -565,9 +578,11 @@
     if (ws->opt_debug) {
         const gmmvb_pass_counters& L = f.L;
         const double rows_l = f.rows_l();
-        std::fprintf(stderr, "[gmmvb] estep: mode=%d known=%d lag(mode=%d act=%.3g eval=%.3g over=%.3g settled=%.3g listed=%.3g) gamma=%.3f rec_valid=%d drift=%d settle=%d\n",
+        std::fprintf(stderr, "[gmmvb] estep: mode=%d known=%d lag(mode=%d act=%.3g eval=%.3g over=%.3g settled=%.3g listed=%.3g) gamma=%.3f rec_valid=%d drift=%d settle=%d quiet=%.0f/%lld skipped=%.0f\n",
                      plan.mode, (int)f.known, L.mode, L.act / rows_l, L.eval / rows_l, L.over / rows_l, L.settled / rows_l,
-                     L.listed / rows_l, ws->typical_gamma, (int)ws->rec_valid, (int)ws->have_drift, (int)plan.settle);
+                     L.listed / rows_l, ws->typical_gamma, (int)ws->rec_valid, (int)ws->have_drift, (int)plan.settle,
+                     ws->lag.valid ? ws->lag_quiet : -1.0, (long long)((n_rows + kSelRows - 1) / kSelRows),
+                     ws->lag.valid ? ws->lag_skipped : -1.0);
     }
     const bool wants_drift = gmmvb_wants_drift(ws, n_rows) != 0;
     ws->bound.choose(plan.mode, ws->img_i8b != nullptr, f.L, f.known, wants_drift && ws->have_drift, wants_drift, ws->pt, ws->T,
@@ -629,6 +644,8 @@
     ws->lse_stale = false;
     p.tmeta_was_valid = ws->tmeta_valid;
     ws->tmeta_valid = false;
+    p.quiet_was_valid = ws->quiet_valid && !plan.regroup && ws->tile_quiet() != nullptr;
+    ws->quiet_valid = false;
     if (p.mode == kPassDense) {
         rc = p.run_dense();
     } else {
diff --git a/bayesml_amd/csrc/capi_internal.h b/bayesml_amd/csrc/capi_internal.h
--- a/bayesml_amd/csrc/capi_internal.h
+++ b/bayesml_amd/csrc/capi_internal.h
@@ -85,6 +85,7 @@
 }
 
 static inline void yield_scratch(gmmvb_workspace* w) {
+    w->quiet_valid = false;
     w->lost_estep = w->e_state == 1;
     w->e_state = 0;
     w->active_lists = false;
diff --git a/bayesml_amd/csrc/capi_mstep.hip b/bayesml_amd/csrc/capi_mstep.hip
--- a/bayesml_amd/csrc/capi_mstep.hip
+++ b/bayesml_amd/csrc/capi_mstep.hip
@@ -16,6 +16,7 @@
     ws->e_rows = n_rows;
     ws->n_spans = 0;
     ws->bounds_rows = 0;
+    ws->quiet_valid = false;
     if (ws->lock_live) {
         ws->lock_live = false;
         ws->lock_reset = true;
diff --git a/bayesml_amd/csrc/records.h b/bayesml_amd/csrc/records.h
--- a/bayesml_amd/csrc/records.h
+++ b/bayesml_amd/csrc/records.h
@@ -237,7 +237,9 @@
                                                              float4* __restrict__ tmeta = nullptr ,
                                                              int tmeta_reset = 0 ,
                                                              unsigned long long* __restrict__ col_ctr = nullptr ,
-                                                             double* __restrict__ ppre = nullptr ) {
+                                                             double* __restrict__ ppre = nullptr ,
+                                                             int* __restrict__ tile_loose = nullptr ,
+                                                             unsigned long long* __restrict__ quiet_ctr = nullptr ) {
     static_assert(!LAZY || PREV, "the lazy sweep is a form of the PREV sweep");
     __shared__ int wcnt[4][256];
     __shared__ int pcnt[4][256];
@@ -246,7 +248,7 @@
     __shared__ double sc[256];
     __shared__ unsigned char sfirst[256];
     __shared__ float s_delta[256];
-    __shared__ int wsum[3][4];
+    __shared__ int wsum[4][4];
     __shared__ unsigned char s_force[LAZY ? 256 : 1];
     __shared__ float s_thr[LAZY ? 4 : 1];
     __shared__ unsigned long long s_open[LAZY ? 4 : 1];
@@ -593,6 +595,7 @@
         if (pmask) count_word(pm[w], w, wave, pcnt);
         plisted += __builtin_popcountll(pm[w]);
     }
+    const int loose_w = __builtin_popcountll(__builtin_amdgcn_ballot_w64(valid && !stays));
 #pragma unroll
     for (int o = 32; o > 0; o >>= 1) {
         listed += __shfl_xor(listed, o);
@@ -603,6 +606,7 @@
         wsum[0][wave] = listed;
         wsum[1][wave] = over_i;
         wsum[2][wave] = plisted;
+        wsum[3][wave] = loose_w;
     }
     if constexpr (LAZY) {
         if (lane == 0)
@@ -644,6 +648,11 @@
         epart[blockIdx.x] = (double)(wsum[0][0] + wsum[0][1] + wsum[0][2] + wsum[0][3]);
         opart[blockIdx.x] = (double)(wsum[1][0] + wsum[1][1] + wsum[1][2] + wsum[1][3]);
         if (ppre) ppre[blockIdx.x] = (double)(wsum[2][0] + wsum[2][1] + wsum[2][2] + wsum[2][3]);
+        if (tile_loose) {
+            const int loose = wsum[3][0] + wsum[3][1] + wsum[3][2] + wsum[3][3];
+            tile_loose[blockIdx.x] = loose;
+            if (quiet_ctr && loose == 0) atomicAdd(quiet_ctr, 1ull);
+        }
     }
 }
 
@@ -655,9 +664,10 @@
                                                                     float* __restrict__ dlock, float* __restrict__ rthr,
                                                                     int* __restrict__ blk_cnt, double* __restrict__ epart,
                                                                     double* __restrict__ ppart,
-                                                                    const double* __restrict__ own_part ) {
+                                                                    const double* __restrict__ own_part ,
+                                                                    int* __restrict__ tile_loose = nullptr ) {
     __shared__ int wcnt[4][256];
-    __shared__ int wsum[2][4];
+    __shared__ int wsum[3][4];
     const int tid = threadIdx.x, wave = tid >> 6;
     const int W = (K + 63) / 64;
     for (int k = tid & 63; k < K; k += 64) wcnt[wave][k] = 0;
@@ -665,6 +675,7 @@
     const bool valid = n < n_rows;
     unsigned long long mk[4] = {0ull, 0ull, 0ull, 0ull}, old[4] = {0ull, 0ull, 0ull, 0ull};
     int listed = 0, proved = 0;
+    bool back = false;
     const unsigned fl0 = valid ? rec.flags[n] : 0u;
     if (valid && ((fl0 & 16u) || fl0 == 8u)) {
         for (int w = 0; w < W; ++w) old[w] = mk[w] = masks[(int64_t)w * npad + n];
@@ -758,6 +769,7 @@
             }
             if (!any && l > -__builtin_huge_val()) {
                 rec.flags[n] = 4;
+                back = true;
                 dlock[n] = f32_up(dist_of(cvec[kset], l) * (1.0 + 1e-9));
             } else {
                 kept[kset >> 6] |= 1ull << (kset & 63);
@@ -790,6 +802,7 @@
         }
     }
     for (int w = 0; w < W; ++w) count_word(mk[w], w, wave, wcnt);
+    const int back_w = __builtin_popcountll(__builtin_amdgcn_ballot_w64(back));
 #pragma unroll
     for (int o = 32; o > 0; o >>= 1) {
         listed += __shfl_xor(listed, o);
@@ -798,6 +811,7 @@
     if ((tid & 63) == 0) {
         wsum[0][wave] = listed;
         wsum[1][wave] = proved;
+        wsum[2][wave] = back_w;
     }
     __syncthreads();
     const int joined = wsum[0][0] + wsum[0][1] + wsum[0][2] + wsum[0][3];
@@ -809,6 +823,8 @@
     if (tid == 0) {
         if (joined != 0) epart[blockIdx.x] += (double)joined;
         ppart[blockIdx.x] = (double)(wsum[1][0] + wsum[1][1] + wsum[1][2] + wsum[1][3]) + (own_part ? own_part[blockIdx.x] : 0.0);
+        const int returned = wsum[2][0] + wsum[2][1] + wsum[2][2] + wsum[2][3];
+        if (tile_loose && returned != 0) tile_loose[blockIdx.x] -= returned;
     }
 }
 
@@ -937,12 +953,31 @@
                                                               double* __restrict__ spart, double* __restrict__ gpart,
                                                               double* __restrict__ qpart ,
                                                               const float* __restrict__ rthr ,
-                                                              unsigned char* __restrict__ lcomp ) {
+                                                              unsigned char* __restrict__ lcomp ,
+                                                              const int* __restrict__ tile_loose = nullptr ,
+                                                              int* __restrict__ tile_quiet = nullptr ,
+                                                              int quiet_valid = 0 ,
+                                                              unsigned long long* __restrict__ quiet_ctr = nullptr ) {
     __shared__ int wcnt[4][256];
     __shared__ int dcnt[4][256];
     __shared__ int mcnt[4][256];
     __shared__ int wact[4], wmov[4], wset[4], wlist[4], wacc[4];
     const int tid = threadIdx.x, wave = tid >> 6;
+    const int loose = tile_loose ? tile_loose[blockIdx.x] : -1;
+    if (quiet_valid && loose == 0 && tile_quiet[blockIdx.x] == 1) {
+        for (int k = tid; k < K; k += kSelRows) {
+            blk_cnt[blk_at(k, blockIdx.x, K)] = 0;
+            if (dblk) dblk[blk_at(k, blockIdx.x, K)] = mblk[blk_at(k, blockIdx.x, K)] = 0;
+        }
+        if (tid == 0) {
+            const int64_t left = n_rows - (int64_t)blockIdx.x * kSelRows;
+            const double rows = (double)(left < kSelRows ? left : (int64_t)kSelRows);
+            apart[blockIdx.x] = spart[blockIdx.x] = rows;
+            mpart[blockIdx.x] = gpart[blockIdx.x] = qpart[blockIdx.x] = 0.0;
+            if (quiet_ctr) atomicAdd(quiet_ctr, 1ull << 32);
+        }
+        return;
+    }
     const int W = (K + 63) / 64;
     for (int k = tid & 63; k < K; k += 64) wcnt[wave][k] = dcnt[wave][k] = mcnt[wave][k] = 0;
     const int64_t n = (int64_t)blockIdx.x * kSelRows + tid;
@@ -1234,6 +1269,7 @@
         spart[blockIdx.x] = (double)(wset[0] + wset[1] + wset[2] + wset[3]);
         gpart[blockIdx.x] = (double)(wlist[0] + wlist[1] + wlist[2] + wlist[3]);
         qpart[blockIdx.x] = (double)(wacc[0] + wacc[1] + wacc[2] + wacc[3]);
+        if (tile_quiet) tile_quiet[blockIdx.x] = loose == 0 ? 1 : 0;
     }
 }
 
@@ -1274,7 +1310,8 @@
                                                                 int K, unsigned long long* __restrict__ masks,
                                                                 int* __restrict__ blk_cnt,
                                                                 const double* __restrict__ drift = nullptr ,
-                                                                double* __restrict__ listed_part = nullptr ) {
+                                                                double* __restrict__ listed_part = nullptr ,
+                                                                const int* __restrict__ tile_quiet = nullptr ) {
     __shared__ int wcnt[4][256];
     const int64_t n = (int64_t)blockIdx.x * kSelRows + threadIdx.x;
     const bool valid = n < n_rows;
@@ -1282,10 +1319,13 @@
     const int wave = threadIdx.x >> 6;
     for (int k = threadIdx.x & 63; k < K; k += 64) wcnt[wave][k] = 0;
     const int64_t nn = valid ? n : 0;
-    const unsigned lk = lock[nn];
     const int lc = (int)lcomp[nn];
+    unsigned lk = 1u;
     unsigned long long any = 0ull;
-    for (int w = 0; w < W; ++w) any |= emask[(int64_t)w * npad + nn];
+    if (!(tile_quiet && tile_quiet[blockIdx.x] == 1)) {
+        lk = lock[nn];
+        for (int w = 0; w < W; ++w) any |= emask[(int64_t)w * npad + nn];
+    }
     int kh = (valid && lk == 1u && any == 0ull) ? lc : -1;
     if (kh >= 0 && drift != nullptr && !own_first(drift[3 * K + kh], drift[K + kh])) kh = -1;
     for (int w = 0; w < W; ++w) {
diff --git a/bayesml_amd/csrc/workspace.h b/bayesml_amd/csrc/workspace.h
--- a/bayesml_amd/csrc/workspace.h
+++ b/bayesml_amd/csrc/workspace.h
@@ -128,6 +128,12 @@
     bool pend_proj = false;
     float4* tmeta = nullptr;
     bool tmeta_valid = false;
+    bool quiet_valid = false;
+    bool pend_quiet = false;
+    double lag_quiet = -1.0;
+    double lag_skipped = -1.0;
+    int* tile_loose() const { return (opt_quiet_tiles && perm_tmp && !(scratch && scratch->refs > 1)) ? perm_tmp : nullptr; }
+    int* tile_quiet() const { return tile_loose() ? perm_tmp + (npad + 255) / 256 : nullptr; }
     double* ppart = nullptr;
     void* xp = nullptr;
     int* perm = nullptr, *iperm = nullptr, *perm_tmp = nullptr;
diff --git a/bayesml_amd/csrc/workspace_plan.h b/bayesml_amd/csrc/workspace_plan.h
--- a/bayesml_amd/csrc/workspace_plan.h
+++ b/bayesml_amd/csrc/workspace_plan.h
@@ -38,6 +38,7 @@
     bool opt_carry_off = false;
     bool opt_hmm_mstep_dense = false;
     bool opt_calibrate = true;
+    bool opt_quiet_tiles = true;
     bool opt_debug = false;
 
     template <typename Lookup>
@@ -62,6 +63,7 @@
         o.opt_carry_off = dev("GMMVB_ESTEP_CARRY_OFF") != nullptr;
         o.opt_hmm_mstep_dense = dev("GMMVB_HMM_MSTEP_DENSE") != nullptr;
         o.opt_calibrate = not_zero(dev("GMMVB_POLICY_CALIBRATE"));
+        o.opt_quiet_tiles = not_zero(dev("GMMVB_QUIET_TILES"));
         o.opt_debug = lookup("GMMVB_DEBUG") && lookup("GMMVB_DEBUG")[0] == '2';
         return o;
     }
```

Result: faster. 5.585 billion samples/s (median of 6 runs) (+6.3%).
